# liuyuan-pal/Gen6D

Hardware: NVIDIA B200
Metric: poses/sec end-to-end (128^2 crop, 64 refs, 3 refine iters) (higher is better)
Workload: dtype f32

## Files before the change

gen6d_b200/_lib.py:

```python
import ctypes as C
import os
import re

HERE = os.path.dirname(os.path.abspath(__file__))
LIB_PATH = os.path.join(HERE, 'libgen6d_b200.so')
HEADER_PATH = os.path.join(os.path.dirname(HERE), 'include', 'gen6d_b200.h')

G6D_DET_MAX_SCALES = 8
PRO_NONE, PRO_AFFINE, PRO_AFFINE_RELU, PRO_CORR = 0, 1, 2, 3
ACT_NONE, ACT_RELU, ACT_LEAKY01 = 0, 1, 2
TC_TF32, TC_F16 = 0, 1


class ConvDesc(C.Structure):
    _fields_ = [(n, C.c_int) for n in ('B', 'D', 'H', 'W', 'Cin', 'in_cstride', 'in_coff', 'Cout', 'kd', 'kh', 'kw',
                                       'stride', 'pd', 'ph', 'pw', 'Do', 'Ho', 'Wo', 'out_cstride', 'out_coff',
                                       'prologue')] + [('group_rows', C.c_longlong), ('act', C.c_int), ('max_chain_k', C.c_int)]


class DetMaps(C.Structure):
    _fields_ = [('n_scales', C.c_int), ('rfn', C.c_int), ('hs', C.c_int), ('ws', C.c_int),
                ('map', (C.c_void_p * 3) * G6D_DET_MAX_SCALES),
                ('H', (C.c_int * 3) * G6D_DET_MAX_SCALES), ('W', (C.c_int * 3) * G6D_DET_MAX_SCALES),
                ('mu', C.c_float * 3), ('inv_sigma', C.c_float * 3), ('clip', C.c_float)]


class GlueCamera(C.Structure):
    _fields_ = [('K', C.c_double * 9), ('Kinv', C.c_double * 9), ('f', C.c_double), ('f_sq', C.c_double)]


class GlueRefs(C.Structure):
    _fields_ = [('poses', C.c_void_p), ('cen', C.c_void_p), ('f', C.c_void_p), ('dist', C.c_void_p), ('center', C.c_double * 3)]


class GlueViews(C.Structure):
    _fields_ = [('poses', C.c_void_p), ('R_look', C.c_void_p), ('RlookR', C.c_void_p), ('f', C.c_void_p), ('Kinv', C.c_void_p),
                ('src', C.c_void_p), ('rows', C.c_void_p), ('cols', C.c_void_p), ('even_idx', C.c_void_p), ('even_dirs', C.c_void_p),
                ('n_views', C.c_int), ('n_even', C.c_int), ('ref_num', C.c_int), ('size', C.c_int),
                ('norm_scale', C.c_double), ('norm_offset', C.c_float * 3), ('size_scale', C.c_float)]


P, I, L, F = C.c_void_p, C.c_int, C.c_longlong, C.c_float
_SIGNATURES = {
    'g6d_preprocess_u8': [P, P, L, I, I, P],
    'g6d_imagenet_norm': [P, P, L, I, I, P],
    'g6d_warp_perspective_u8': [P, I, P, I, I, P],
    'g6d_warp_affine_u8': [P, I, P, I, I, P],
    'g6d_glue_detection_jobs': [P, P, I, I, I, I, P, P],
    'g6d_glue_detection_jobs_host': [P, P, I, I, I, I, P],
    'g6d_glue_initial_poses': [P, P, P, C.POINTER(GlueRefs), P, I, P, P],
    'g6d_glue_initial_poses_host': [P, P, P, C.POINTER(GlueRefs), P, I, P],
    'g6d_glue_refine_problems': [C.POINTER(GlueViews), P, P, I, I, P, I, I, P, P, P, P, P, P, P, P],
    'g6d_glue_refine_problems_host': [C.POINTER(GlueViews), P, P, I, I, P, I, I, P, P, P, P, P, P, P],
    'g6d_glue_apply_refinements': [C.POINTER(GlueViews), P, P, P, P, I, P, P],
    'g6d_glue_apply_refinements_host': [C.POINTER(GlueViews), P, P, P, P, I, P],
    'g6d_track_smooth': [P, P, P, P, P, I, I, P, P, P, P, P, P],
    'g6d_track_smooth_host': [P, P, P, P, P, I, I, P, P, P, P, P],
    'g6d_nchw_to_nhwc': [P, P, I, I, I, I, I, P],
    'g6d_nhwc_to_nchw': [P, P, I, I, I, I, I, P],
    'g6d_resize_bilinear': [P, P, I, I, I, I, I, I, I, I, P],
    'g6d_resize_nearest': [P, P, I, I, I, I, I, I, P],
    'g6d_maxpool2x2': [P, P, I, I, I, I, P],
    'g6d_l2norm_channels': [P, P, L, I, F, P],
    'g6d_affine_act': [P, P, L, I, L, P, P, I, I, I, I, I, P],
    'g6d_avgpool_affine': [P, P, L, I, I, L, P, P, I, P],
    'g6d_add': [P, P, P, L, P],
    'g6d_instnorm_stats': [P, L, I, I, I, L, F, P, P, P, P],
    'g6d_instnorm_partial': [P, L, I, I, I, L, P, P],
    'g6d_instnorm_finalize': [P, L, I, L, F, P, P, P],
    'g6d_conv': [C.POINTER(ConvDesc), P, P, P, P, P, P, P, P],
    'g6d_conv_workspace_bytes': [C.POINTER(ConvDesc)],
    'g6d_vgg_first_block': [P, P, P, P, I, I, I, P],
    'g6d_pack_conv_weight': [P, P, I, I, I, I, P, P],
    'g6d_conv_tc_supported': [C.POINTER(ConvDesc), I],
    'g6d_conv_tc_debug': [C.POINTER(C.c_int)],
    'g6d_debug_umma_shift': [P, I, I, P],
    'g6d_conv_tc_workspace_bytes': [C.POINTER(ConvDesc), I],
    'g6d_conv_tc': [C.POINTER(ConvDesc), P, P, P, I, I, P, P, P, P, P, P, L, P],
    'g6d_conv_tc_stats_supported': [C.POINTER(ConvDesc), I, L],
    'g6d_pack_conv_weight_tc': [P, P, P, I, I, I, I, I, P, I, P],
    'g6d_split_operand': [P, P, P, L, I, P],
    'g6d_transpose2d': [P, P, I, I, P],
    'g6d_linear_smallm': [P, P, P, P, I, I, I, I, P],
    'g6d_det_score_fuse': [C.POINTER(DetMaps), I, P, P, P, P, P, P],
    'g6d_det_parse': [P, P, P, I, I, I, I, P, P, P],
    'g6d_det_corr_rowsum': [P, P, I, I, I, I, I, P],
    'g6d_sel_ref_sums': [P, I, I, I, P, P, P],
    'g6d_sel_corr_prologue': [P, P, P, I, I, I, F, P, P, P],
    'g6d_sel_corr_score': [P, P, I, I, I, P, P],
    'g6d_sel_corr_score3': [P, P, P, P, P, P, I, I, I, I, I, P, P, P, P],
    'g6d_sel_corr_score3_workspace_bytes': [I, I, I, I],
    'g6d_sel_vp_norm': [P, I, I, F, P, I, I, P],
    'g6d_sel_max_angle_add': [P, P, P, I, I, I, P],
    'g6d_attention': [P, P, P, P, I, I, I, P],
    'g6d_attention_headmajor': [P, P, P, P, I, I, I, P],
    'g6d_layernorm': [P, P, P, P, I, I, F, P],
    'g6d_sel_parse': [P, P, I, I, P, P, P],
    'g6d_ref_volume_fill': [P, P, P, P, P, P, I, I, I, I, I, I, I, I, P, P, P],
    'g6d_ref_pose_heads': [P, P, P, P, I, I, P],
    'g6d_pose_errors_workspace_bytes': [I, I],
    'g6d_pose_errors': [P, I, P, P, P, I, I, P, P, P],
}
_RESTYPE = {'g6d_pose_errors_workspace_bytes': L, 'g6d_sel_corr_score3_workspace_bytes': L, 'g6d_conv_workspace_bytes': L, 'g6d_conv_tc_workspace_bytes': L, 'g6d_launch_count': L, 'g6d_last_error': C.c_char_p}

_lib = None


class Gen6DLibraryError(RuntimeError):
    pass


def header_symbols():
    text = open(HEADER_PATH).read()
    text = re.sub(r'/\*.*?\*/', '', text, flags=re.S)
    return sorted(set(re.findall(r'\b(g6d_[a-z0-9_]+)\s*\(', text)))


def lib():
    global _lib
    if _lib is not None:
        return _lib
    if not os.path.exists(LIB_PATH):
        raise Gen6DLibraryError(
            f'{LIB_PATH} not found: build it with `python -m gen6d_b200.build` '
            '(there is no CPU or PyTorch fallback for the Gen6D hot path)')
    l = C.CDLL(LIB_PATH)
    for name, args in _SIGNATURES.items():
        fn = getattr(l, name)
        fn.argtypes = args
        fn.restype = _RESTYPE.get(name, I)
    l.g6d_last_error.restype = C.c_char_p
    l.g6d_last_error.argtypes = []
    l.g6d_version.restype = I
    l.g6d_launch_count.restype = L
    _lib = l
    return l


def check(rc, name):
    if rc != 0:
        msg = lib().g6d_last_error().decode(errors='replace')
        raise Gen6DLibraryError(f'{name} failed ({rc}): {msg}')


def launch_count():
    return int(lib().g6d_launch_count())
```

gen6d_b200/csrc/common.cuh:

```cuda
#pragma once
#include <cuda_runtime.h>
#include <stdint.h>
#include <stdio.h>
#include <stdarg.h>

#include "../../include/gen6d_b200.h"

namespace g6d {

void set_error(const char* fmt, ...);
void count_launch(int n = 1);

inline cudaStream_t as_stream(g6d_stream_t s) { return reinterpret_cast<cudaStream_t>(s); }

#define G6D_CHECK_LAUNCH(name)                                                        \
    do {                                                                              \
        cudaError_t e__ = cudaGetLastError();                                         \
        if (e__ != cudaSuccess) {                                                     \
            g6d::set_error("%s: launch failed: %s", name, cudaGetErrorString(e__));   \
            return G6D_ECUDA;                                                         \
        }                                                                             \
        g6d::count_launch();                                                          \
    } while (0)

#define G6D_REQUIRE(cond, ...)            \
    do {                                  \
        if (!(cond)) {                    \
            g6d::set_error(__VA_ARGS__);  \
            return G6D_EINVAL;            \
        }                                 \
    } while (0)

constexpr int kNumSMs = 148;

__device__ __forceinline__ float warp_sum(float v) {
#pragma unroll
    for (int o = 16; o > 0; o >>= 1) v += __shfl_xor_sync(0xffffffffu, v, o);
    return v;
}
__device__ __forceinline__ double warp_sum(double v) {
#pragma unroll
    for (int o = 16; o > 0; o >>= 1) v += __shfl_xor_sync(0xffffffffu, v, o);
    return v;
}
__device__ __forceinline__ float warp_max(float v) {
#pragma unroll
    for (int o = 16; o > 0; o >>= 1) v = fmaxf(v, __shfl_xor_sync(0xffffffffu, v, o));
    return v;
}

__device__ __forceinline__ float4 ldg_stream(const float4* p) {
    float4 r;
    asm volatile("ld.global.nc.L1::no_allocate.v4.f32 {%0,%1,%2,%3}, [%4];"
                 : "=f"(r.x), "=f"(r.y), "=f"(r.z), "=f"(r.w)
                 : "l"(p));
    return r;
}

inline int ceil_div(long long a, long long b) { return (int)((a + b - 1) / b); }

}
```

gen6d_b200/csrc/conv_ffma.cu:

```cuda
#include "common.cuh"

namespace g6d {

struct ConvP {
    const float* x; const float* w; const float* bias; const float* ps; const float* pb;
    float* y; float* ws;
    int B, D, H, W, Cin, ics, ico, Cout, ldw, kd, kh, kw, stride, pd, ph, pw, Do, Ho, Wo, ocs, oco, pro, act;
    long long group_rows;
    int M, K, ktiles, splits, kt_per_split;
};

constexpr int BM = 128, BK = 16, NT = 256;

__device__ __forceinline__ float act_apply(float v, int act) {
    if (act == G6D_ACT_RELU) return fmaxf(v, 0.f);
    if (act == G6D_ACT_LEAKY01) return v > 0.f ? v : 0.1f * v;
    return v;
}

template <int TN>
__global__ void __launch_bounds__(NT, 2) conv_ffma_kernel(const ConvP p) {
    constexpr int BN = 16 * TN;
    constexpr int HN = BN / 2;
    constexpr int B_F4 = (BK * BN / 4);
    constexpr int B_PER_T = (B_F4 + NT - 1) / NT;
    __shared__ __align__(16) float As[2][BK][BM + 4];
    __shared__ __align__(16) float Bs[2][BK][BN];

    const int t = threadIdx.x;
    const int tx = t & 15, ty = t >> 4;
    const int m_base = blockIdx.x * BM;
    const int n_base = blockIdx.y * BN;
    const int split = blockIdx.z;
    const int kt_begin = split * p.kt_per_split;
    const int kt_end = min(p.ktiles, kt_begin + p.kt_per_split);

    const int kq = t & 3;
    int rb[2], rz[2], ry[2], rx[2];
    bool rvalid[2];
#pragma unroll
    for (int i = 0; i < 2; ++i) {
        int m = m_base + (t >> 2) + 64 * i;
        rvalid[i] = m < p.M;
        int mm = rvalid[i] ? m : 0;
        int xo = mm % p.Wo; mm /= p.Wo;
        int yo = mm % p.Ho; mm /= p.Ho;
        int zo = mm % p.Do; mm /= p.Do;
        rb[i] = mm;
        rz[i] = zo * p.stride - p.pd;
        ry[i] = yo * p.stride - p.ph;
        rx[i] = xo * p.stride - p.pw;
    }

    float4 a_reg[2];
    float4 b_reg[B_PER_T];

    auto load_tile = [&](int kt) {
        const int k = kt * BK + kq * 4;
        const bool kvalid = k < p.K;
        int tap = 0, c = k;
        if (p.K != p.Cin) { tap = k / p.Cin; c = k - tap * p.Cin; }
        const int kx = tap % p.kw;
        const int tq = tap / p.kw;
        const int ky = tq % p.kh;
        const int kz = tq / p.kh;
#pragma unroll
        for (int i = 0; i < 2; ++i) {
            float4 v = make_float4(0.f, 0.f, 0.f, 0.f);
            const int zi = rz[i] + kz, yi = ry[i] + ky, xi = rx[i] + kx;
            const bool inb = rvalid[i] && kvalid && (unsigned)zi < (unsigned)p.D && (unsigned)yi < (unsigned)p.H &&
                             (unsigned)xi < (unsigned)p.W;
            if (inb) {
                const long long pos = ((long long)(rb[i] * p.D + zi) * p.H + yi) * p.W + xi;
                v = __ldg(reinterpret_cast<const float4*>(p.x + pos * p.ics + p.ico + c));
                if (p.pro != G6D_PRO_NONE) {
                    float4 s, b;
                    if (p.pro == G6D_PRO_CORR) {
                        const long long sp = ((long long)zi * p.H + yi) * p.W + xi;
                        s = __ldg(reinterpret_cast<const float4*>(p.ps + sp * p.Cin + c));
                        b = __ldg(reinterpret_cast<const float4*>(p.pb + c));
                    } else {
                        const long long g = rb[i] / p.group_rows;
                        s = __ldg(reinterpret_cast<const float4*>(p.ps + g * p.Cin + c));
                        b = __ldg(reinterpret_cast<const float4*>(p.pb + g * p.Cin + c));
                    }
                    v.x = fmaf(v.x, s.x, b.x); v.y = fmaf(v.y, s.y, b.y);
                    v.z = fmaf(v.z, s.z, b.z); v.w = fmaf(v.w, s.w, b.w);
                    if (p.pro == G6D_PRO_AFFINE_RELU) {
                        v.x = fmaxf(v.x, 0.f); v.y = fmaxf(v.y, 0.f); v.z = fmaxf(v.z, 0.f); v.w = fmaxf(v.w, 0.f);
                    }
                }
            }
            a_reg[i] = v;
        }
#pragma unroll
        for (int j = 0; j < B_PER_T; ++j) {
            const int f = t + j * NT;
            float4 v = make_float4(0.f, 0.f, 0.f, 0.f);
            if (f < B_F4) {
                const int kr = f / (BN / 4), nq = f % (BN / 4);
                const int kk = kt * BK + kr, n = n_base + nq * 4;
                if (kk < p.K && n < p.ldw) v = __ldg(reinterpret_cast<const float4*>(p.w + (long long)kk * p.ldw + n));
            }
            b_reg[j] = v;
        }
    };
    auto store_tile = [&](int buf) {
#pragma unroll
        for (int i = 0; i < 2; ++i) {
            const int r = (t >> 2) + 64 * i;
            As[buf][kq * 4 + 0][r] = a_reg[i].x;
            As[buf][kq * 4 + 1][r] = a_reg[i].y;
            As[buf][kq * 4 + 2][r] = a_reg[i].z;
            As[buf][kq * 4 + 3][r] = a_reg[i].w;
        }
#pragma unroll
        for (int j = 0; j < B_PER_T; ++j) {
            const int f = t + j * NT;
            if (f < B_F4) {
                const int kr = f / (BN / 4), nq = f % (BN / 4);
                *reinterpret_cast<float4*>(&Bs[buf][kr][nq * 4]) = b_reg[j];
            }
        }
    };

    float acc[8][TN];
#pragma unroll
    for (int i = 0; i < 8; ++i)
#pragma unroll
        for (int j = 0; j < TN; ++j) acc[i][j] = 0.f;

    if (kt_begin < kt_end) {
        load_tile(kt_begin);
        store_tile(0);
    }
    __syncthreads();
    int cur = 0;
// ... 131 lines not shown
            const int xi = 2 * xp - 1 + dx;
            float4 v = make_float4(0.f, 0.f, 0.f, 0.f);
            if ((unsigned)yi < (unsigned)H && (unsigned)xi < (unsigned)W)
                v = __ldg(reinterpret_cast<const float4*>(x + ((b * H + yi) * W + xi) * 4));
            win[dy][dx] = make_float3(v.x, v.y, v.z);
        }
    }
    float acc[4][16];
#pragma unroll
    for (int o = 0; o < 16; ++o) { const float bv = bs[q * 16 + o]; acc[0][o] = bv; acc[1][o] = bv; acc[2][o] = bv; acc[3][o] = bv; }
#pragma unroll
    for (int ky = 0; ky < 3; ++ky) {
#pragma unroll
        for (int kx = 0; kx < 3; ++kx) {
            const float* wr = ws + (ky * 3 + kx) * 4 * 64 + q * 16;
#pragma unroll
            for (int o4 = 0; o4 < 4; ++o4) {
                const float4 w0 = *reinterpret_cast<const float4*>(wr + o4 * 4);
                const float4 w1 = *reinterpret_cast<const float4*>(wr + 64 + o4 * 4);
                const float4 w2 = *reinterpret_cast<const float4*>(wr + 128 + o4 * 4);
#pragma unroll
                for (int px = 0; px < 4; ++px) {
                    const float3 v = win[(px >> 1) + ky][(px & 1) + kx];
                    float* a = acc[px] + o4 * 4;
                    a[0] = fmaf(v.x, w0.x, fmaf(v.y, w1.x, fmaf(v.z, w2.x, a[0])));
                    a[1] = fmaf(v.x, w0.y, fmaf(v.y, w1.y, fmaf(v.z, w2.y, a[1])));
                    a[2] = fmaf(v.x, w0.z, fmaf(v.y, w1.z, fmaf(v.z, w2.z, a[2])));
                    a[3] = fmaf(v.x, w0.w, fmaf(v.y, w1.w, fmaf(v.z, w2.w, a[3])));
                }
            }
        }
    }
    float4* yr = reinterpret_cast<float4*>(y + pp * 64 + q * 16);
#pragma unroll
    for (int o4 = 0; o4 < 4; ++o4) {
        float r[4];
#pragma unroll
        for (int e = 0; e < 4; ++e) {
            const int o = o4 * 4 + e;
            r[e] = fmaxf(fmaxf(fmaxf(acc[0][o], acc[1][o]), fmaxf(acc[2][o], acc[3][o])), 0.f);
        }
        __stcs(yr + o4, make_float4(r[0], r[1], r[2], r[3]));
    }
}

static int fill_params(const g6d_conv_desc* d, ConvP& p) {
    G6D_REQUIRE(d != nullptr, "g6d_conv: null desc");
    G6D_REQUIRE(d->B > 0 && d->D > 0 && d->H > 0 && d->W > 0 && d->Cin > 0 && d->Cout > 0, "g6d_conv: bad dims");
    G6D_REQUIRE(d->kd > 0 && d->kh > 0 && d->kw > 0 && d->stride > 0, "g6d_conv: bad kernel/stride");
    G6D_REQUIRE((d->Cin & 3) == 0 && (d->in_cstride & 3) == 0 && (d->in_coff & 3) == 0,
                "g6d_conv: Cin (%d), in_cstride (%d), in_coff (%d) must be multiples of 4", d->Cin, d->in_cstride,
                d->in_coff);
    G6D_REQUIRE(d->in_coff + d->Cin <= d->in_cstride, "g6d_conv: input channel slice out of row");
    G6D_REQUIRE(d->out_coff + d->Cout <= d->out_cstride, "g6d_conv: output channel slice out of row");
    const int Do = (d->D + 2 * d->pd - d->kd) / d->stride + 1;
    const int Ho = (d->H + 2 * d->ph - d->kh) / d->stride + 1;
    const int Wo = (d->W + 2 * d->pw - d->kw) / d->stride + 1;
    G6D_REQUIRE(Do == d->Do && Ho == d->Ho && Wo == d->Wo, "g6d_conv: output dims mismatch (%d,%d,%d) vs (%d,%d,%d)",
                d->Do, d->Ho, d->Wo, Do, Ho, Wo);
    G6D_REQUIRE(d->prologue >= 0 && d->prologue <= 3 && d->act >= 0 && d->act <= 2, "g6d_conv: bad prologue/act");
    if (d->prologue == G6D_PRO_AFFINE || d->prologue == G6D_PRO_AFFINE_RELU)
        G6D_REQUIRE(d->group_rows > 0, "g6d_conv: group_rows must be > 0 for affine prologue");
    const long long M = (long long)d->B * Do * Ho * Wo;
    const long long K = (long long)d->kd * d->kh * d->kw * d->Cin;
    G6D_REQUIRE(M < (1ll << 31) && K < (1ll << 31), "g6d_conv: problem too large");
    p.B = d->B; p.D = d->D; p.H = d->H; p.W = d->W; p.Cin = d->Cin; p.ics = d->in_cstride; p.ico = d->in_coff;
    p.Cout = d->Cout; p.ldw = (d->Cout + 3) & ~3; p.kd = d->kd; p.kh = d->kh; p.kw = d->kw; p.stride = d->stride;
    p.pd = d->pd; p.ph = d->ph; p.pw = d->pw; p.Do = Do; p.Ho = Ho; p.Wo = Wo; p.ocs = d->out_cstride;
    p.oco = d->out_coff; p.pro = d->prologue; p.act = d->act; p.group_rows = d->group_rows > 0 ? d->group_rows : 1;
    p.M = (int)M; p.K = (int)K; p.ktiles = (int)((K + BK - 1) / BK);
    const int bn = d->Cout > 64 ? 128 : (d->Cout > 32 ? 64 : 32);
    const long long ctas = (long long)ceil_div(M, BM) * ceil_div(d->Cout, bn);
    int splits = 1;
    if (ctas < kNumSMs && p.ktiles >= 16) {
        splits = (int)((2 * kNumSMs + ctas - 1) / ctas);
        splits = splits > p.ktiles / 8 ? p.ktiles / 8 : splits;
        splits = splits > 64 ? 64 : splits;
        splits = splits < 1 ? 1 : splits;
    }
    p.kt_per_split = (p.ktiles + splits - 1) / splits;
    p.splits = (p.ktiles + p.kt_per_split - 1) / p.kt_per_split;
    return G6D_OK;
}

}

using namespace g6d;

extern "C" long long g6d_conv_workspace_bytes(const g6d_conv_desc* desc) {
    ConvP p{};
    if (fill_params(desc, p) != G6D_OK) return -1;
    return p.splits > 1 ? (long long)p.splits * p.M * p.Cout * (long long)sizeof(float) : 0;
}

extern "C" int g6d_conv(const g6d_conv_desc* desc, const float* x, const float* w, const float* bias,
                        const float* pro_scale, const float* pro_shift, float* y, void* ws, g6d_stream_t stream) {
    ConvP p{};
    int rc = fill_params(desc, p);
    if (rc != G6D_OK) return rc;
    G6D_REQUIRE(x && w && y, "g6d_conv: null tensor pointer");
    if (p.pro != G6D_PRO_NONE) G6D_REQUIRE(pro_scale && pro_shift, "g6d_conv: prologue operands missing");
    if (p.splits > 1) G6D_REQUIRE(ws != nullptr, "g6d_conv: split-K workspace required (%d splits)", p.splits);
    p.x = x; p.w = w; p.bias = bias; p.ps = pro_scale; p.pb = pro_shift; p.y = y; p.ws = (float*)ws;
    cudaStream_t st = as_stream(stream);
    if (p.Cin == 4 && p.ics == 4 && p.ico == 0 && p.Cout == 64 && p.ocs == 64 && p.oco == 0 && p.kd == 1 && p.kh == 3 &&
        p.kw == 3 && p.stride == 1 && p.pd == 0 && p.ph == 1 && p.pw == 1 && p.D == 1 && p.pro == G6D_PRO_NONE) {
        conv3x3_c4_o64_kernel<<<ceil_div(p.M, 128), 128, 0, st>>>(x, w, bias, y, p.B, p.H, p.W, p.act);
        G6D_CHECK_LAUNCH("g6d_conv(first layer)");
        return G6D_OK;
    }
    const int bn = p.Cout > 64 ? 128 : (p.Cout > 32 ? 64 : 32);
    dim3 grid(ceil_div(p.M, BM), ceil_div(p.Cout, bn), p.splits);
    if (bn == 128) conv_ffma_kernel<8><<<grid, NT, 0, st>>>(p);
    else if (bn == 64) conv_ffma_kernel<4><<<grid, NT, 0, st>>>(p);
    else conv_ffma_kernel<2><<<grid, NT, 0, st>>>(p);
    G6D_CHECK_LAUNCH("g6d_conv");
    if (p.splits > 1) {
        const long long n = (long long)p.M * p.Cout;
        conv_splitk_reduce_kernel<<<ceil_div(n, 256), 256, 0, st>>>(p.ws, bias, y, p.M, p.Cout, p.splits, p.ocs, p.oco,
                                                                     p.act);
        G6D_CHECK_LAUNCH("g6d_conv(splitk reduce)");
    }
    return G6D_OK;
}

extern "C" int g6d_vgg_first_block(const float* x, const float* w, const float* bias, float* y, int B, int H, int W,
                                   g6d_stream_t stream) {
    G6D_REQUIRE(x && w && y && B > 0 && H >= 2 && W >= 2 && (H & 1) == 0 && (W & 1) == 0, "g6d_vgg_first_block: bad args (H, W even)");
    const long long threads = (long long)B * (H / 2) * (W / 2) * 4;
    conv3x3_c4_o64_relu_pool_kernel<<<ceil_div(threads, 128), 128, 0, as_stream(stream)>>>(x, w, bias, y, B, H, W);
    G6D_CHECK_LAUNCH("g6d_vgg_first_block");
    return G6D_OK;
}

__global__ void pack_conv_weight_kernel(const float* __restrict__ w, float* __restrict__ out, int Cout, int Cin,
                                        int Cin_pad, int taps, int ldw, const float* __restrict__ scale) {
    const long long i = (long long)blockIdx.x * blockDim.x + threadIdx.x;
    const long long total = (long long)taps * Cin_pad * ldw;
    if (i >= total) return;
    const int o = (int)(i % ldw);
    const long long k = i / ldw;
    const int c = (int)(k % Cin_pad);
    const int tap = (int)(k / Cin_pad);
    float v = 0.f;
    if (o < Cout && c < Cin) {
        v = w[((long long)o * Cin + c) * taps + tap];
        if (scale) v *= scale[o];
    }
    out[i] = v;
}

extern "C" int g6d_pack_conv_weight(const float* w, float* out, int Cout, int Cin, int Cin_pad, int taps,
                                    const float* cout_scale, g6d_stream_t stream) {
    G6D_REQUIRE(w && out && Cout > 0 && Cin > 0 && Cin_pad >= Cin && taps > 0, "g6d_pack_conv_weight: bad args");
    const int ldw = (Cout + 3) & ~3;
    const long long total = (long long)taps * Cin_pad * ldw;
    pack_conv_weight_kernel<<<ceil_div(total, 256), 256, 0, as_stream(stream)>>>(w, out, Cout, Cin, Cin_pad, taps, ldw,
                                                                                 cout_scale);
    G6D_CHECK_LAUNCH("g6d_pack_conv_weight");
// ... 68 lines not shown
```

gen6d_b200/csrc/conv_tc.cu:

```cuda
#include <stdlib.h>
#include <string.h>

#include <cuda_fp16.h>

#include "tc_common.cuh"

namespace g6d {

constexpr int TC_BM = 128;
constexpr int TC_PRODUCER_WARPS = 8;
constexpr int TC_THREADS = (TC_PRODUCER_WARPS + 2) * 32;
constexpr int TC_MAX_K_PER_CHAIN = 2048;

template <int KIND> struct KindCfg;
template <> struct KindCfg<G6D_TC_TF32> {
    static constexpr int BK = 32;
    static constexpr int NV = 1;
    static constexpr int RING = 3;
    static constexpr float CROSS = 1.f;
};
template <> struct KindCfg<G6D_TC_F16> {
    static constexpr int BK = 64;
    static constexpr int NV = 2;
    static constexpr int RING = 2;
    static constexpr float CROSS = 1.f / 2048.f;
};
constexpr float F16_LO_SCALE = 2048.f;
__host__ __device__ __forceinline__ int f16_k_source(int p) {
    const int c = p >> 3, i = p & 7;
    return i < 4 ? 4 * c + i : 32 + 4 * c + (i - 4);
}

struct ConvTcP {
    const float* x; const float* bias; const float* ps; const float* pb;
    float* y; float* ws;
    int B, D, H, W, Cin, ics, ico, Cout, kd, kh, kw, stride, pd, ph, pw, Do, Ho, Wo, ocs, oco, pro, act;
    long long group_rows;
    int M, K, kblocks, splits, kb_per_split;
    double* stats; long long stats_rows;
};

__device__ __forceinline__ uint32_t cvt_f16x2_sat(float e0, float e1) {
    uint32_t r;
    asm("cvt.rn.satfinite.f16x2.f32 %0, %1, %2;" : "=r"(r) : "f"(e1), "f"(e0));
    return r;
}
__device__ __forceinline__ void split_f16x2(float e0, float e1, uint32_t& hi, uint32_t& lo) {
    hi = cvt_f16x2_sat(e0, e1);
    const float2 hf = __half22float2(*reinterpret_cast<const __half2*>(&hi));
    lo = cvt_f16x2_sat((e0 - hf.x) * F16_LO_SCALE, (e1 - hf.y) * F16_LO_SCALE);
}
__device__ __forceinline__ void split_tf32x4(const float4 v, float4& hi, float4& lo) {
    hi.x = __uint_as_float((__float_as_uint(v.x) + 0x1000u) & 0xFFFFE000u);
    hi.y = __uint_as_float((__float_as_uint(v.y) + 0x1000u) & 0xFFFFE000u);
    hi.z = __uint_as_float((__float_as_uint(v.z) + 0x1000u) & 0xFFFFE000u);
    hi.w = __uint_as_float((__float_as_uint(v.w) + 0x1000u) & 0xFFFFE000u);
    lo.x = v.x - hi.x; lo.y = v.y - hi.y; lo.z = v.z - hi.z; lo.w = v.w - hi.w;
}
__device__ __forceinline__ void st_shared_v4(uint32_t addr, uint32_t a, uint32_t b, uint32_t c, uint32_t d) {
    asm volatile("st.shared.v4.b32 [%0], {%1,%2,%3,%4};" ::"r"(addr), "r"(a), "r"(b), "r"(c), "r"(d) : "memory");
}
template <int KIND>
__device__ __forceinline__ void split_store(uint32_t hi_addr, uint32_t lo_addr, const float4 (&v)[KindCfg<KIND>::NV]) {
    if constexpr (KIND == G6D_TC_TF32) {
        float4 hi, lo;
        split_tf32x4(v[0], hi, lo);
        st_shared_v4(hi_addr, __float_as_uint(hi.x), __float_as_uint(hi.y), __float_as_uint(hi.z), __float_as_uint(hi.w));
        st_shared_v4(lo_addr, __float_as_uint(lo.x), __float_as_uint(lo.y), __float_as_uint(lo.z), __float_as_uint(lo.w));
    } else {
        uint32_t h[4], l[4];
        split_f16x2(v[0].x, v[0].y, h[0], l[0]);
        split_f16x2(v[0].z, v[0].w, h[1], l[1]);
        split_f16x2(v[1].x, v[1].y, h[2], l[2]);
        split_f16x2(v[1].z, v[1].w, h[3], l[3]);
        st_shared_v4(hi_addr, h[0], h[1], h[2], h[3]);
        st_shared_v4(lo_addr, l[0], l[1], l[2], l[3]);
    }
}
__device__ __forceinline__ float4 affine4(float4 x, const float4 sc, const float4 sh, bool relu) {
    x.x = fmaf(x.x, sc.x, sh.x); x.y = fmaf(x.y, sc.y, sh.y); x.z = fmaf(x.z, sc.z, sh.z); x.w = fmaf(x.w, sc.w, sh.w);
    if (relu) { x.x = fmaxf(x.x, 0.f); x.y = fmaxf(x.y, 0.f); x.z = fmaxf(x.z, 0.f); x.w = fmaxf(x.w, 0.f); }
    return x;
}

template <int KIND>
__device__ __forceinline__ uint32_t umma_idesc(int M, int N) {
    constexpr uint32_t fmt = KIND == G6D_TC_TF32 ? 2u : 0u;
    return (1u << 4) | (fmt << 7) | (fmt << 10) | ((uint32_t)(N >> 3) << 17) | ((uint32_t)(M >> 4) << 24);
}
template <int KIND>
// ... 78 lines not shown
    const uint32_t base = (smem_u32(smem_raw) + 1023u) & ~1023u;
    uint8_t* base_ptr = smem_raw + (base - smem_u32(smem_raw));
    const uint32_t bar_base = base + STAGES * Cfg::STAGE_BYTES;
    auto a_hi = [&](int s) { return base + s * Cfg::STAGE_BYTES; };
    auto a_lo = [&](int s) { return base + s * Cfg::STAGE_BYTES + Cfg::A_BYTES; };
    auto b_hi = [&](int s) { return base + s * Cfg::STAGE_BYTES + 2 * Cfg::A_BYTES; };
    auto b_lo = [&](int s) { return base + s * Cfg::STAGE_BYTES + 2 * Cfg::A_BYTES + Cfg::B_BYTES; };
    auto full_a = [&](int s) { return bar_base + 8 * s; };
    auto full_b = [&](int s) { return bar_base + 8 * (STAGES + s); };
    auto empty = [&](int s) { return bar_base + 8 * (2 * STAGES + s); };
    auto tmem_full = [&](int b) { return bar_base + 8 * (3 * STAGES + b); };
    auto tmem_empty = [&](int b) { return bar_base + 8 * (3 * STAGES + 2 + b); };
    volatile uint32_t* tmem_slot = reinterpret_cast<volatile uint32_t*>(base_ptr + STAGES * Cfg::STAGE_BYTES + 8 * (3 * STAGES + 4));

    const int warp = threadIdx.x >> 5, lane = threadIdx.x & 31;
    if (warp == W_TMA && lane == 0) {
        for (int s = 0; s < STAGES; ++s) {
            mbar_init(full_a(s), NPW);
            mbar_init(full_b(s), 1);
            mbar_init(empty(s), 1);
        }
        for (int b = 0; b < 2; ++b) { mbar_init(tmem_full(b), 1); mbar_init(tmem_empty(b), 4); }
        fence_barrier_init();
        asm volatile("prefetch.tensormap [%0];" ::"l"(&map_hi) : "memory");
        asm volatile("prefetch.tensormap [%0];" ::"l"(&map_lo) : "memory");
    }
    if (warp == W_MMA) {
        asm volatile("tcgen05.alloc.cta_group::1.sync.aligned.shared::cta.b32 [%0], %1;"
                     ::"r"(smem_u32((const void*)tmem_slot)), "n"(Cfg::TMEM_COLS) : "memory");
        asm volatile("tcgen05.relinquish_alloc_permit.cta_group::1.sync.aligned;" ::: "memory");
    }
    tc_fence_before();
    __syncthreads();
    tc_fence_after();
    const uint32_t tmem_acc = *tmem_slot;

    auto decode = [&](int w, int& mt, int& nt, int& sp) {
        nt = w % wk.n_tiles; w /= wk.n_tiles;
        mt = w % wk.m_tiles;
        sp = w / wk.m_tiles;
    };

    if (warp < NPW) {
        const int chunk = threadIdx.x & 7;
        const int cofs = chunk * 4;
        const int r0 = threadIdx.x >> 3;
        int git = 0;
        for (int w = blockIdx.x; w < wk.total; w += gridDim.x) {
            int mt, nt, sp;
            decode(w, mt, nt, sp);
            const int m_base = mt * TC_BM;
            const int kb_begin = sp * p.kb_per_split;
            const int nkb = min(p.kblocks, kb_begin + p.kb_per_split) - kb_begin;
            int rb[ROWS], rsp[ROWS], rc[ROWS];
            unsigned rvmask = 0;
            const long long plane_sz = (long long)p.D * p.H * p.W;
#pragma unroll
            for (int j = 0; j < ROWS; ++j) {
                int m = m_base + r0 + RSTEP * j;
                const bool v = m < p.M;
                if (!v) m = 0;
                const int xo = m % p.Wo; m /= p.Wo;
                const int yo = m % p.Ho; m /= p.Ho;
                const int zo = m % p.Do; m /= p.Do;
                rb[j] = m;
                const int z = zo * p.stride - p.pd, y = yo * p.stride - p.ph, x = xo * p.stride - p.pw;
                rsp[j] = (z * p.H + y) * p.W + x;
                rc[j] = ((z + 8) << 24) | ((y + 8) << 12) | (x + 8);
                if (v) rvmask |= 1u << j;
            }
            int c0, kx, ky, kz;
            {
                const int k = kb_begin * BK;
                int tap = 0; c0 = k;
                if (p.K != p.Cin) { tap = k / p.Cin; c0 = k - tap * p.Cin; }
                kx = tap % p.kw; const int tq = tap / p.kw; ky = tq % p.kh; kz = tq / p.kh;
            }
            float4 v[RING][ROWS][NV];
            unsigned okm[RING]; int kc[RING]; int ksp[RING];
            auto issue_loads = [&](int q) {
                const int tap_sp = (kz * p.H + ky) * p.W + kx;
                okm[q] = 0; kc[q] = c0 + cofs; ksp[q] = tap_sp;
                const float* xb = p.x + p.ico + cofs + c0;
#pragma unroll
                for (int j = 0; j < ROWS; ++j) {
                    const int z = ((rc[j] >> 24) & 0xff) - 8 + kz, y = ((rc[j] >> 12) & 0xfff) - 8 + ky, x = (rc[j] & 0xfff) - 8 + kx;
                    const bool inb = ((rvmask >> j) & 1u) && (unsigned)z < (unsigned)p.D && (unsigned)y < (unsigned)p.H &&
                                     (unsigned)x < (unsigned)p.W;
#pragma unroll
                    for (int e = 0; e < NV; ++e) v[q][j][e] = make_float4(0.f, 0.f, 0.f, 0.f);
                    if (inb) {
                        const float4* src = reinterpret_cast<const float4*>(xb + ((long long)rb[j] * plane_sz + rsp[j] + tap_sp) * p.ics);
#pragma unroll
                        for (int e = 0; e < NV; ++e) v[q][j][e] = __ldg(src + e * 8);
                        okm[q] |= 1u << j;
                    }
                }
                c0 += BK;
                if (c0 == p.Cin) { c0 = 0; if (++kx == p.kw) { kx = 0; if (++ky == p.kh) { ky = 0; ++kz; } } }
            };
            auto process = [&](int q, int it) {
                const int g_it = git + it;
                const int s = g_it % STAGES;
                const uint32_t n_use = g_it / STAGES;
                if (p.pro != G6D_PRO_NONE) {
                    const bool relu = p.pro == G6D_PRO_AFFINE_RELU;
#pragma unroll
                    for (int j = 0; j < ROWS; ++j) {
                        if (okm[q] & (1u << j)) {
                            const float4* scp; const float4* shp;
                            if (p.pro == G6D_PRO_CORR) {
                                scp = reinterpret_cast<const float4*>(p.ps + (long long)(rsp[j] + ksp[q]) * p.Cin + kc[q]);
                                shp = reinterpret_cast<const float4*>(p.pb + kc[q]);
                            } else {
                                const long long g = rb[j] / (int)p.group_rows;
                                scp = reinterpret_cast<const float4*>(p.ps + g * p.Cin + kc[q]);
                                shp = reinterpret_cast<const float4*>(p.pb + g * p.Cin + kc[q]);
                            }
#pragma unroll
                            for (int e = 0; e < NV; ++e) v[q][j][e] = affine4(v[q][j][e], __ldg(scp + e * 8), __ldg(shp + e * 8), relu);
                        }
                    }
                }
                mbar_wait(empty(s), (n_use & 1) ^ 1, 1, g_it);
#pragma unroll
                for (int j = 0; j < ROWS; ++j) {
                    const int r = r0 + RSTEP * j;
                    const uint32_t so = r * 128 + ((chunk ^ (r & 7)) << 4);
                    split_store<KIND>(a_hi(s) + so, a_lo(s) + so, v[q][j]);
                }
                fence_proxy_async();
                __syncwarp();
                if (lane == 0) mbar_arrive(full_a(s));
            };
#pragma unroll
            for (int q = 0; q < RING - 1; ++q)
                if (q < nkb) issue_loads(q);
            for (int it = 0; it < nkb; it += RING) {
#pragma unroll
                for (int q = 0; q < RING; ++q) {
                    if (it + q < nkb) {
                        if (it + q + RING - 1 < nkb) issue_loads((q + RING - 1) % RING);
                        process(q, it + q);
                    }
                }
            }
            git += nkb;
        }
    } else if (warp == W_TMA) {
        if (lane == 0) {
            int git = 0;
            for (int w = blockIdx.x; w < wk.total; w += gridDim.x) {
                int mt, nt, sp;
                decode(w, mt, nt, sp);
                const int kb_begin = sp * p.kb_per_split;
                const int nkb = min(p.kblocks, kb_begin + p.kb_per_split) - kb_begin;
                for (int it = 0; it < min(nkb, PF); ++it) {
                    tma_prefetch_2d(&map_hi, (kb_begin + it) * BK, nt * BN);
                    tma_prefetch_2d(&map_lo, (kb_begin + it) * BK, nt * BN);
                }
                for (int it = 0; it < nkb; ++it, ++git) {
                    const int s = git % STAGES;
                    if (it + PF < nkb) {
                        tma_prefetch_2d(&map_hi, (kb_begin + it + PF) * BK, nt * BN);
                        tma_prefetch_2d(&map_lo, (kb_begin + it + PF) * BK, nt * BN);
                    }
                    mbar_wait(empty(s), ((git / STAGES) & 1) ^ 1, 3, git);
                    mbar_expect_tx(full_b(s), 2 * Cfg::B_BYTES);
                    const int k = (kb_begin + it) * BK;
                    tma_load_2d(b_hi(s), &map_hi, full_b(s), k, nt * BN);
                    tma_load_2d(b_lo(s), &map_lo, full_b(s), k, nt * BN);
// ... 177 lines not shown
}

static void launch_reduce(const float* ws, const float* bias, float* y, int M, int Cout, int splits, int ocs, int oco, int act,
                          double* stats, long long stats_rows, cudaStream_t st) {
    if (stats) {
        dim3 grid(ceil_div(M, 32), ceil_div(Cout, 64));
        conv_tc_reduce_stats_kernel<<<grid, 256, 0, st>>>(ws, bias, y, M, Cout, splits, ocs, oco, act, stats, stats_rows);
    } else {
        const long long n = (long long)M * Cout;
        conv_tc_reduce_kernel<<<ceil_div(n, 256), 256, 0, st>>>(ws, bias, y, M, Cout, splits, ocs, oco, act);
    }
}

typedef CUresult (*EncodeTiledFn)(CUtensorMap*, CUtensorMapDataType, cuuint32_t, void*, const cuuint64_t*,
                                  const cuuint64_t*, const cuuint32_t*, const cuuint32_t*, CUtensorMapInterleave,
                                  CUtensorMapSwizzle, CUtensorMapL2promotion, CUtensorMapFloatOOBfill);

static EncodeTiledFn get_encode_fn() {
    static EncodeTiledFn fn = nullptr;
    static bool tried = false;
    if (!tried) {
        tried = true;
        void* sym = nullptr;
        cudaDriverEntryPointQueryResult qres;
        if (cudaGetDriverEntryPoint("cuTensorMapEncodeTiled", &sym, cudaEnableDefault, &qres) == cudaSuccess &&
            qres == cudaDriverEntryPointSuccess)
            fn = reinterpret_cast<EncodeTiledFn>(sym);
    }
    return fn;
}

static int kind_bk(int kind) { return kind == G6D_TC_F16 ? 64 : 32; }
static int kind_esize(int kind) { return kind == G6D_TC_F16 ? 2 : 4; }

static int make_weight_map(CUtensorMap* map, const void* w, int rows, int K, int bn, int kind) {
    EncodeTiledFn enc = get_encode_fn();
    if (!enc) { set_error("g6d_conv_tc: cuTensorMapEncodeTiled unavailable"); return G6D_ECUDA; }
    cuuint64_t dims[2] = {(cuuint64_t)K, (cuuint64_t)rows};
    cuuint64_t strides[1] = {(cuuint64_t)K * kind_esize(kind)};
    cuuint32_t box[2] = {(cuuint32_t)kind_bk(kind), (cuuint32_t)bn};
    cuuint32_t estr[2] = {1, 1};
    CUresult r = enc(map, kind == G6D_TC_F16 ? CU_TENSOR_MAP_DATA_TYPE_FLOAT16 : CU_TENSOR_MAP_DATA_TYPE_FLOAT32, 2,
                     const_cast<void*>(w), dims, strides, box, estr,
                     CU_TENSOR_MAP_INTERLEAVE_NONE, CU_TENSOR_MAP_SWIZZLE_128B, CU_TENSOR_MAP_L2_PROMOTION_L2_256B,
                     CU_TENSOR_MAP_FLOAT_OOB_FILL_NONE);
    if (r != CUDA_SUCCESS) { set_error("g6d_conv_tc: cuTensorMapEncodeTiled failed (%d)", (int)r); return G6D_ECUDA; }
    return G6D_OK;
}

static int tc_block_n(int Cout) { return Cout > 64 ? 128 : (Cout > 32 ? 64 : 32); }

static bool tc2_dims_ok(const g6d_conv_desc* d) {
    return d->D + d->pd + 8 < 256 && d->H + d->ph + 8 < 4096 && d->W + d->pw + 8 < 4096 &&
           (long long)d->D * d->H * d->W < (1ll << 30) && d->group_rows < (1ll << 31);
}

static int fill_tc_params(const g6d_conv_desc* d, int kind, ConvTcP& p) {
    G6D_REQUIRE(d != nullptr, "g6d_conv_tc: null desc");
    G6D_REQUIRE(kind == G6D_TC_TF32 || kind == G6D_TC_F16, "g6d_conv_tc: bad operand kind %d", kind);
    G6D_REQUIRE(d->B > 0 && d->D > 0 && d->H > 0 && d->W > 0 && d->Cin > 0 && d->Cout > 0, "g6d_conv_tc: bad dims");
    G6D_REQUIRE(d->kd > 0 && d->kh > 0 && d->kw > 0 && d->stride > 0, "g6d_conv_tc: bad kernel/stride");
    const int bk = kind_bk(kind);
    G6D_REQUIRE((d->Cin % bk) == 0, "g6d_conv_tc: Cin (%d) must be a multiple of %d", d->Cin, bk);
    G6D_REQUIRE((d->in_cstride & 3) == 0 && (d->in_coff & 3) == 0, "g6d_conv_tc: in_cstride/in_coff must be multiples of 4");
    G6D_REQUIRE(d->in_coff + d->Cin <= d->in_cstride, "g6d_conv_tc: input channel slice out of row");
    G6D_REQUIRE(d->out_coff + d->Cout <= d->out_cstride, "g6d_conv_tc: output channel slice out of row");
    G6D_REQUIRE(tc2_dims_ok(d), "g6d_conv_tc: spatial extent too large for the tensor-core kernel");
    const int Do = (d->D + 2 * d->pd - d->kd) / d->stride + 1;
    const int Ho = (d->H + 2 * d->ph - d->kh) / d->stride + 1;
    const int Wo = (d->W + 2 * d->pw - d->kw) / d->stride + 1;
    G6D_REQUIRE(Do == d->Do && Ho == d->Ho && Wo == d->Wo, "g6d_conv_tc: output dims mismatch");
    G6D_REQUIRE(d->prologue >= 0 && d->prologue <= 3 && d->act >= 0 && d->act <= 2, "g6d_conv_tc: bad prologue/act");
    const long long M = (long long)d->B * Do * Ho * Wo;
    const long long K = (long long)d->kd * d->kh * d->kw * d->Cin;
    G6D_REQUIRE(M < (1ll << 31) && K < (1ll << 31), "g6d_conv_tc: problem too large");
    p.B = d->B; p.D = d->D; p.H = d->H; p.W = d->W; p.Cin = d->Cin; p.ics = d->in_cstride; p.ico = d->in_coff;
    p.Cout = d->Cout; p.kd = d->kd; p.kh = d->kh; p.kw = d->kw; p.stride = d->stride; p.pd = d->pd; p.ph = d->ph;
    p.pw = d->pw; p.Do = Do; p.Ho = Ho; p.Wo = Wo; p.ocs = d->out_cstride; p.oco = d->out_coff; p.pro = d->prologue;
    p.act = d->act; p.group_rows = d->group_rows > 0 ? d->group_rows : 1;
    p.M = (int)M; p.K = (int)K; p.kblocks = (int)(K / bk);
    const int bn = tc_block_n(d->Cout);
    const long long ctas = (long long)ceil_div(M, TC_BM) * ceil_div(d->Cout, bn);
    const int min_kb = 256 / bk;
    int splits = 1;
    if (ctas < kNumSMs && p.kblocks >= 2 * min_kb) {
        splits = (int)(kNumSMs / ctas);
        splits = splits > p.kblocks / min_kb ? p.kblocks / min_kb : splits;
        splits = splits < 1 ? 1 : splits;
    }
    const int nmain = bn == 32 ? Tc2Cfg<32>::NMAIN : (bn == 64 ? Tc2Cfg<64>::NMAIN : Tc2Cfg<128>::NMAIN);
    const int chain = d->max_chain_k > 0 ? d->max_chain_k * nmain : (K > 8192 ? TC_MAX_K_PER_CHAIN : 0);
    const int max_kb = chain > bk ? chain / bk : 1;
    const int min_splits = chain > 0 ? (p.kblocks + max_kb - 1) / max_kb : 1;
    splits = splits < min_splits ? min_splits : splits;
    splits = splits > 64 ? 64 : splits;
    p.kb_per_split = (p.kblocks + splits - 1) / splits;
    p.splits = (p.kblocks + p.kb_per_split - 1) / p.kb_per_split;
    return G6D_OK;
}

template <int BN, int KIND, int NPW = 8>
static int launch_tc2(const ConvTcP& p, const CUtensorMap& mh, const CUtensorMap& ml, cudaStream_t st) {
    using Cfg = Tc2Cfg<BN>;
    static bool configured = false;
    if (!configured) {
        cudaError_t e = cudaFuncSetAttribute(conv_tc2_kernel<BN, KIND, NPW>, cudaFuncAttributeMaxDynamicSharedMemorySize, Cfg::SMEM_BYTES);
        if (e != cudaSuccess) { set_error("g6d_conv_tc: cannot opt in to %d B of shared memory: %s", Cfg::SMEM_BYTES, cudaGetErrorString(e)); return G6D_ECUDA; }
        configured = true;
    }
    Tc2Work wk;
    wk.m_tiles = ceil_div(p.M, TC_BM); wk.n_tiles = ceil_div(p.Cout, BN);
    const long long total = (long long)wk.m_tiles * wk.n_tiles * p.splits;
    wk.total = (int)total;
    const int grid = total < kNumSMs ? (int)total : kNumSMs;
    conv_tc2_kernel<BN, KIND, NPW><<<grid, tc2_threads(NPW), Cfg::SMEM_BYTES, st>>>(p, wk, mh, ml);
    G6D_CHECK_LAUNCH("g6d_conv_tc");
    return G6D_OK;
}

__global__ void split_tf32_kernel(const float* __restrict__ in, float* __restrict__ hi, float* __restrict__ lo, long long n) {
    const long long i = (long long)blockIdx.x * blockDim.x + threadIdx.x;
    if (i >= n) return;
    const float v = in[i];
    const float h = to_tf32(v);
    hi[i] = h;
    lo[i] = to_tf32(v - h);
}
__device__ __forceinline__ void split_f16_scalar(float v, __half& h, __half& l) {
    uint32_t hh, ll;
    split_f16x2(v, 0.f, hh, ll);
    h = __ushort_as_half((unsigned short)(hh & 0xffffu));
    l = __ushort_as_half((unsigned short)(ll & 0xffffu));
}
__global__ void split_f16_kernel(const float* __restrict__ in, __half* __restrict__ hi, __half* __restrict__ lo, long long n) {
    const long long i = (long long)blockIdx.x * blockDim.x + threadIdx.x;
    if (i >= n) return;
    split_f16_scalar(in[(i & ~63ll) + f16_k_source((int)(i & 63))], hi[i], lo[i]);
}

template <int KIND>
__global__ void pack_conv_weight_tc_kernel(const float* __restrict__ w, void* __restrict__ hi, void* __restrict__ lo,
                                           int Cout, int Cin, int Cin_pad, int taps, int rows_pad,
                                           const float* __restrict__ scale) {
    const long long i = (long long)blockIdx.x * blockDim.x + threadIdx.x;
    const long long K = (long long)taps * Cin_pad;
    if (i >= K * rows_pad) return;
    const int o = (int)(i / K);
    const long long k = i % K;
    const int tap = (int)(k / Cin_pad);
    int c = (int)(k % Cin_pad);
    if constexpr (KIND == G6D_TC_F16) c = (c & ~63) + f16_k_source(c & 63);
    float v = 0.f;
    if (o < Cout && c < Cin) {
        v = w[((long long)o * Cin + c) * taps + tap];
        if (scale) v *= scale[o];
    }
    if constexpr (KIND == G6D_TC_TF32) {
        const float h = to_tf32(v);
        static_cast<float*>(hi)[i] = h;
        static_cast<float*>(lo)[i] = to_tf32(v - h);
    } else {
        split_f16_scalar(v, static_cast<__half*>(hi)[i], static_cast<__half*>(lo)[i]);
    }
}

struct ConvFlatP {
    const float* x; const float* bias; const float* ps; const float* pb; float* y; float* ws;
    int B, D, H, W, Cin, ics, ico, Cout, kd, kh, kw, pd, ph, pw, Do, Ho, Wo, ocs, oco, pro, act;
    long long group_rows;
    int Wp, tiles_per_plane, mode, nseg, taps_per_seg, seg_rows, rows_pad, ntab, cblocks;
    int a_stages, b_stages, splits, cb_per_split, M;
    double* stats; long long stats_rows;
};

template <int BN> struct FlatCfg {
    static constexpr int NMAIN = BN == 32 ? 7 : (BN == 256 ? 1 : 3);
    static constexpr int TMEM_COLS = (NMAIN + 1) * BN;
};

template <int BN, int KIND>
__global__ void __launch_bounds__(TC_THREADS, 1)
conv_tcflat_kernel(const ConvFlatP p, const __grid_constant__ CUtensorMap map_hi, const __grid_constant__ CUtensorMap map_lo) {
    using KC = KindCfg<KIND>;
    constexpr int NMAIN = FlatCfg<BN>::NMAIN;
    constexpr int TMEM_COLS = FlatCfg<BN>::TMEM_COLS;
    constexpr int B_BYTES = BN * 128;
    constexpr int BK = KC::BK, NV = KC::NV;
    extern __shared__ uint8_t smem_raw[];
    const uint32_t base = (smem_u32(smem_raw) + 1023u) & ~1023u;
    uint8_t* base_ptr = smem_raw + (base - smem_u32(smem_raw));
    const int A_TILE = p.rows_pad * 128;
    const uint32_t a_base = base;
    const uint32_t b_base = base + p.a_stages * 2 * A_TILE;
    const uint32_t bar_base = b_base + p.b_stages * 2 * B_BYTES;
    auto a_hi = [&](int s) { return a_base + s * 2 * A_TILE; };
    auto a_lo = [&](int s) { return a_base + s * 2 * A_TILE + A_TILE; };
    auto b_hi = [&](int s) { return b_base + s * 2 * B_BYTES; };
    auto b_lo = [&](int s) { return b_base + s * 2 * B_BYTES + B_BYTES; };
    auto a_full = [&](int s) { return bar_base + 8 * s; };
    auto a_empty = [&](int s) { return bar_base + 8 * (4 + s); };
    auto b_full = [&](int s) { return bar_base + 8 * (8 + s); };
    auto b_empty = [&](int s) { return bar_base + 8 * (12 + s); };
    const uint32_t tmem_full = bar_base + 8 * 16;
    const uint32_t bar_off = (bar_base - base);
    volatile uint32_t* tmem_slot = reinterpret_cast<volatile uint32_t*>(base_ptr + bar_off + 8 * 17);
    int* rowtab = reinterpret_cast<int*>(base_ptr + bar_off + 256);

    const int warp = threadIdx.x >> 5, lane = threadIdx.x & 31;
    int tile = blockIdx.x;
    const int t_in_plane = tile % p.tiles_per_plane; tile /= p.tiles_per_plane;
    const int zo = tile % p.Do;
    const int b = tile / p.Do;
    const int f0 = t_in_plane * TC_BM;
    const int n_base = blockIdx.y * BN;
    const int split = blockIdx.z;
    const int cb_begin = split * p.cb_per_split;
    const int cb_end = min(p.cblocks, cb_begin + p.cb_per_split);
    const int nunits = (cb_end - cb_begin) * p.nseg;

    for (int e = threadIdx.x; e < p.ntab * p.seg_rows; e += blockDim.x) {
        const int tb = e / p.seg_rows, i = e % p.seg_rows;
        const int g = f0 + (p.mode == 1 ? tb * p.Wp : 0) + i;
        const int yy = g / p.Wp - p.ph, xx = g % p.Wp - p.pw;
        rowtab[e] = ((unsigned)yy < (unsigned)p.H && (unsigned)xx < (unsigned)p.W) ? yy * p.W + xx : -1;
    }
    if (warp == TC_PRODUCER_WARPS && lane == 0) {
        for (int s = 0; s < 4; ++s) {
            mbar_init(a_full(s), TC_PRODUCER_WARPS);
            mbar_init(a_empty(s), 1);
            mbar_init(b_full(s), 1);
            mbar_init(b_empty(s), 1);
        }
        mbar_init(tmem_full, 1);
        fence_barrier_init();
        asm volatile("prefetch.tensormap [%0];" ::"l"(&map_hi) : "memory");
        asm volatile("prefetch.tensormap [%0];" ::"l"(&map_lo) : "memory");
    }
    if (warp == TC_PRODUCER_WARPS + 1) {
        asm volatile("tcgen05.alloc.cta_group::1.sync.aligned.shared::cta.b32 [%0], %1;"
                     ::"r"(smem_u32((const void*)tmem_slot)), "n"(TMEM_COLS) : "memory");
        asm volatile("tcgen05.relinquish_alloc_permit.cta_group::1.sync.aligned;" ::: "memory");
    }
    tc_fence_before();
    __syncthreads();
    tc_fence_after();
    const uint32_t tmem_acc = *tmem_slot;

    if (warp < TC_PRODUCER_WARPS) {
        const int chunk = threadIdx.x & 7;
        const int cofs = chunk * 4;
        const int r0 = threadIdx.x >> 3;
        const long long plane = (long long)p.H * p.W;
        const long long gi = (long long)b / p.group_rows;
        const bool relu = p.pro == G6D_PRO_AFFINE_RELU;
        constexpr int NB = 3;
        const int trips = (p.seg_rows + 127) / 128;
        const int total = nunits * trips;
        float4 v[NB][4][NV]; int off[NB][4];
        auto unit_of = [&](int tt, int& u, int& rbase, int& cb, int& kz, int& tb) {
            u = tt / trips; rbase = (tt - u * trips) * 128;
            cb = cb_begin + u / p.nseg;
            const int seg = u % p.nseg;
            kz = p.mode == 1 ? seg / p.kh : seg;
            tb = p.mode == 1 ? seg % p.kh : 0;
        };
        auto issue = [&](int tt, int q) {
            int u, rbase, cb, kz, tb;
            unit_of(tt, u, rbase, cb, kz, tb);
            const int zz = zo + kz - p.pd;
            const bool zok = (unsigned)zz < (unsigned)p.D;
            const float* xplane = p.x + ((long long)b * p.D + (zok ? zz : 0)) * plane * p.ics + p.ico + cb * BK + cofs;
            const int* tab = rowtab + tb * p.seg_rows;
#pragma unroll
            for (int j = 0; j < 4; ++j) {
                const int r = rbase + r0 + 32 * j;
                off[q][j] = (r < p.seg_rows && zok) ? tab[r] : -1;
#pragma unroll
                for (int e = 0; e < NV; ++e) v[q][j][e] = make_float4(0.f, 0.f, 0.f, 0.f);
                if (off[q][j] >= 0) {
                    const float4* src = reinterpret_cast<const float4*>(xplane + (long long)off[q][j] * p.ics);
#pragma unroll
                    for (int e = 0; e < NV; ++e) v[q][j][e] = __ldg(src + e * 8);
                }
            }
        };
        auto store = [&](int tt, int q) {
            int u, rbase, cb, kz, tb;
            unit_of(tt, u, rbase, cb, kz, tb);
            const int s = u % p.a_stages;
            const int zz = zo + kz - p.pd;
            const int c = cb * BK + cofs;
            if (rbase == 0) mbar_wait(a_empty(s), ((u / p.a_stages) & 1) ^ 1, 1, u);
#pragma unroll
            for (int j = 0; j < 4; ++j) {
                const int r = rbase + r0 + 32 * j;
                if (r >= p.rows_pad) continue;
                if (p.pro != G6D_PRO_NONE && off[q][j] >= 0) {
                    const float4* scp; const float4* shp;
                    if (p.pro == G6D_PRO_CORR) {
                        const long long sp = (long long)zz * plane + off[q][j];
                        scp = reinterpret_cast<const float4*>(p.ps + sp * p.Cin + c);
                        shp = reinterpret_cast<const float4*>(p.pb + c);
                    } else {
                        scp = reinterpret_cast<const float4*>(p.ps + gi * p.Cin + c);
                        shp = reinterpret_cast<const float4*>(p.pb + gi * p.Cin + c);
                    }
#pragma unroll
                    for (int e = 0; e < NV; ++e) v[q][j][e] = affine4(v[q][j][e], __ldg(scp + e * 8), __ldg(shp + e * 8), relu);
                }
                const uint32_t so = r * 128 + ((chunk ^ (r & 7)) << 4);
                split_store<KIND>(a_hi(s) + so, a_lo(s) + so, v[q][j]);
            }
            if (rbase + 128 >= p.seg_rows) {
                fence_proxy_async();
                __syncwarp();
                if (lane == 0) mbar_arrive(a_full(s));
            }
        };
#pragma unroll
        for (int q = 0; q < NB - 1; ++q)
            if (q < total) issue(q, q);
        for (int tt = 0; tt < total; tt += NB) {
#pragma unroll
            for (int q = 0; q < NB; ++q) {
                if (tt + q < total) {
                    if (tt + q + NB - 1 < total) issue(tt + q + NB - 1, (q + NB - 1) % NB);
                    store(tt + q, q);
                }
            }
        }

        mbar_wait(tmem_full, 0, 2, nunits);
        tc_fence_after();
        const int quad = warp & 3;
        const int row = quad * 32 + lane;
        const int f = f0 + row;
        const int yo = f / p.Wp, xo = f % p.Wp;
        const bool valid = yo < p.Ho && xo < p.Wo;
        const long long m = (((long long)b * p.Do + zo) * p.Ho + yo) * p.Wo + xo;
        constexpr int HALF = BN / 2;
        const int col0 = (warp >> 2) * HALF;
        const bool partial = p.splits > 1;
        const bool vec_ok = partial ? (p.Cout & 3) == 0
                                    : ((p.ocs & 3) == 0 && (p.oco & 3) == 0 && (reinterpret_cast<uintptr_t>(p.y) & 15) == 0 &&
                                       (!p.bias || (reinterpret_cast<uintptr_t>(p.bias) & 15) == 0));
        const int total_mm = nunits * p.taps_per_seg;
        const int n_acc = total_mm < NMAIN ? total_mm : NMAIN;
#pragma unroll
        for (int cc = 0; cc < HALF; cc += 16) {
            float accv[16];
            const uint32_t taddr = tmem_acc + ((uint32_t)(quad * 32) << 16) + (uint32_t)(col0 + cc);
            {
                uint32_t r[16];
                G6D_TMEM_LD16(r, taddr + (uint32_t)(NMAIN * BN));
                asm volatile("tcgen05.wait::ld.sync.aligned;" ::: "memory");
// ... 59 lines not shown
                    const int k = (seg * p.taps_per_seg + t) * p.Cin + cb * BK;
                    tma_load_2d(b_hi(s), &map_hi, b_full(s), k, n_base);
                    tma_load_2d(b_lo(s), &map_lo, b_full(s), k, n_base);
                }
            }
        }
    } else {
        if (elect_one_sync()) {
            const uint32_t idesc = umma_idesc<KIND>(TC_BM, BN);
            int bi = 0;
            for (int u = 0; u < nunits; ++u) {
                const int sa = u % p.a_stages;
                mbar_wait(a_full(sa), (u / p.a_stages) & 1, 4, u);
                tc_fence_after();
                for (int t = 0; t < p.taps_per_seg; ++t, ++bi) {
                    const int sb = bi % p.b_stages;
                    mbar_wait(b_full(sb), (bi / p.b_stages) & 1, 5, bi);
                    tc_fence_after();
                    const int shift = p.mode == 1 ? t : (t / p.kw) * p.Wp + (t % p.kw);
                    const uint64_t dah = umma_desc_sw128(a_hi(sa) + shift * 128), dal = umma_desc_sw128(a_lo(sa) + shift * 128);
                    const uint64_t dbh = umma_desc_sw128(b_hi(sb)), dbl = umma_desc_sw128(b_lo(sb));
                    const uint32_t main_acc = tmem_acc + (uint32_t)((bi % NMAIN) * BN);
                    const uint32_t cross_acc = tmem_acc + (uint32_t)(NMAIN * BN);
#pragma unroll
                    for (int ks = 0; ks < 4; ++ks) {
                        const uint64_t adv = (uint64_t)((ks * 32) >> 4);
                        umma<KIND>(cross_acc, dal + adv, dbh + adv, idesc, (bi > 0 || ks > 0) ? 1u : 0u);
                        umma<KIND>(cross_acc, dah + adv, dbl + adv, idesc, 1u);
                        umma<KIND>(main_acc, dah + adv, dbh + adv, idesc, (bi >= NMAIN || ks > 0) ? 1u : 0u);
                    }
                    umma_commit(b_empty(sb));
                }
                umma_commit(a_empty(sa));
            }
            umma_commit(tmem_full);
        }
    }
    __syncthreads();
    if (warp == TC_PRODUCER_WARPS + 1) {
        tc_fence_after();
        asm volatile("tcgen05.dealloc.cta_group::1.sync.aligned.b32 %0, %1;" ::"r"(tmem_acc), "n"(TMEM_COLS) : "memory");
    }
}

static int flat_level() {
    static int v = -1;
    if (v < 0) { const char* e = getenv("G6D_CONV_FLAT"); v = (e && e[0] >= '0' && e[0] <= '2') ? e[0] - '0' : 1; }
    return v;
}
static bool flat_disabled() { return flat_level() == 0; }

static int fill_flat_params(const g6d_conv_desc* d, int kind, ConvFlatP& p, int* smem_bytes) {
    const int bk = kind_bk(kind);
    if (!d || d->stride != 1 || (d->Cin % bk) != 0 || d->Cout < 16 || (d->in_cstride & 3) || (d->in_coff & 3)) return -1;
    const int Do = d->D + 2 * d->pd - d->kd + 1, Ho = d->H + 2 * d->ph - d->kh + 1, Wo = d->W + 2 * d->pw - d->kw + 1;
    if (Do != d->Do || Ho != d->Ho || Wo != d->Wo || Do < 1 || Ho < 1 || Wo < 1) return -1;
    if (d->kd * d->kh * d->kw == 1) return -1;
    const int bn = tc_block_n(d->Cout);
    const int Wp = d->W + 2 * d->pw;
    const int flat_rows = TC_BM + (d->kh - 1) * Wp + d->kw - 1;
    const int row_rows = TC_BM + d->kw - 1;
    const int budget = 220 * 1024;
    const int b_stage = 2 * bn * 128;
    {
        const long long tiles = ((long long)Ho * Wp + TC_BM - 1) / TC_BM;
        if ((long long)Ho * Wo * 100 < tiles * TC_BM * 60) return -1;
    }
    auto a_stage = [](int rows) { return 2 * ((rows + 7) / 8 * 8) * 128; };
    int mode, rows, ntab;
    if (2 * a_stage(flat_rows) + 3 * b_stage + 4 * flat_rows + 2048 <= budget) { mode = 0; rows = flat_rows; ntab = 1; }
    else if (d->kw > 1 && flat_level() >= 2) { mode = 1; rows = row_rows; ntab = d->kh; }
    else return -1;
    p.B = d->B; p.D = d->D; p.H = d->H; p.W = d->W; p.Cin = d->Cin; p.ics = d->in_cstride; p.ico = d->in_coff;
    p.Cout = d->Cout; p.kd = d->kd; p.kh = d->kh; p.kw = d->kw; p.pd = d->pd; p.ph = d->ph; p.pw = d->pw;
    p.Do = Do; p.Ho = Ho; p.Wo = Wo; p.ocs = d->out_cstride; p.oco = d->out_coff; p.pro = d->prologue; p.act = d->act;
    p.group_rows = d->group_rows > 0 ? d->group_rows : 1;
    p.Wp = Wp; p.tiles_per_plane = (Ho * Wp + TC_BM - 1) / TC_BM; p.mode = mode;
    p.nseg = mode == 0 ? d->kd : d->kd * d->kh; p.taps_per_seg = mode == 0 ? d->kh * d->kw : d->kw;
    p.seg_rows = rows; p.rows_pad = (rows + 7) / 8 * 8; p.ntab = ntab; p.cblocks = d->Cin / bk;
    const long long M = (long long)d->B * Do * Ho * Wo;
    if (M >= (1ll << 31)) return -1;
    p.M = (int)M;
    const int tab_bytes = 4 * ntab * rows;
    int a_st = 2, b_st = 3;
    int used = a_st * a_stage(rows) + b_st * b_stage + tab_bytes + 2048;
    while (b_st < 4 && used + b_stage <= budget) { ++b_st; used += b_stage; }
    while (a_st < 4 && used + a_stage(rows) <= budget) { ++a_st; used += a_stage(rows); }
    if (used > budget) return -1;
    p.a_stages = a_st; p.b_stages = b_st;
    *smem_bytes = a_st * a_stage(rows) + b_st * b_stage + 256 + tab_bytes + 1024 + 64;
    const long long ctas = (long long)d->B * Do * p.tiles_per_plane * ((d->Cout + bn - 1) / bn);
    const long long K = (long long)d->Cin * d->kd * d->kh * d->kw;
    int splits = 1;
    if (ctas < kNumSMs && p.cblocks >= 2) splits = (int)((kNumSMs + ctas - 1) / ctas);
    const int nmain = bn == 32 ? FlatCfg<32>::NMAIN : (bn == 64 ? FlatCfg<64>::NMAIN : FlatCfg<128>::NMAIN);
    const long long chain = d->max_chain_k > 0 ? (long long)d->max_chain_k * nmain : (K > 8192 ? TC_MAX_K_PER_CHAIN : 0);
    if (chain > 0) { const int ms = (int)((K + chain - 1) / chain); splits = splits < ms ? ms : splits; }
    splits = splits > p.cblocks ? p.cblocks : splits;
    splits = splits < 1 ? 1 : splits;
    p.cb_per_split = (p.cblocks + splits - 1) / splits;
    p.splits = (p.cblocks + p.cb_per_split - 1) / p.cb_per_split;
    return 0;
}

template <int BN, int KIND>
static int launch_flat(const ConvFlatP& p, int smem, const CUtensorMap& mh, const CUtensorMap& ml, cudaStream_t st) {
    static bool configured = false;
    if (!configured) {
        cudaError_t e = cudaFuncSetAttribute(conv_tcflat_kernel<BN, KIND>, cudaFuncAttributeMaxDynamicSharedMemorySize, 227 * 1024);
        if (e != cudaSuccess) { set_error("g6d_conv_tc(flat): cannot opt in to shared memory: %s", cudaGetErrorString(e)); return G6D_ECUDA; }
        configured = true;
    }
    dim3 grid((unsigned)((long long)p.B * p.Do * p.tiles_per_plane), ceil_div(p.Cout, BN), p.splits);
    conv_tcflat_kernel<BN, KIND><<<grid, TC_THREADS, smem, st>>>(p, mh, ml);
    G6D_CHECK_LAUNCH("g6d_conv_tc(flat)");
    return G6D_OK;
}

template <int KIND>
static int dispatch_flat(int bn, const ConvFlatP& p, int smem, const CUtensorMap& mh, const CUtensorMap& ml, cudaStream_t st) {
    if (bn == 128) return launch_flat<128, KIND>(p, smem, mh, ml, st);
    if (bn == 64) return launch_flat<64, KIND>(p, smem, mh, ml, st);
    return launch_flat<32, KIND>(p, smem, mh, ml, st);
}
template <int KIND>
static int dispatch_tc2(int bn, const ConvTcP& p, const CUtensorMap& mh, const CUtensorMap& ml, cudaStream_t st) {
    if (bn == 128) return launch_tc2<128, KIND>(p, mh, ml, st);
    if (bn == 64) return launch_tc2<64, KIND>(p, mh, ml, st);
    return launch_tc2<32, KIND>(p, mh, ml, st);
}

}

using namespace g6d;

extern "C" int g6d_conv_tc_debug(int* host_out8) {
    G6D_REQUIRE(host_out8 != nullptr, "g6d_conv_tc_debug: null");
    cudaError_t e = cudaDeviceSynchronize();
    if (e != cudaSuccess) { set_error("g6d_conv_tc_debug: sync: %s", cudaGetErrorString(e)); return G6D_ECUDA; }
    e = cudaMemcpyFromSymbol(host_out8, g_tc_timeout, sizeof(int) * 8);
    if (e != cudaSuccess) { set_error("g6d_conv_tc_debug: %s", cudaGetErrorString(e)); return G6D_ECUDA; }
    int zeros[8] = {0, 0, 0, 0, 0, 0, 0, 0};
    cudaMemcpyToSymbol(g_tc_timeout, zeros, sizeof(zeros));
    return G6D_OK;
}

extern "C" int g6d_conv_tc_supported(const g6d_conv_desc* d, int kind) {
    if (!d || (kind != G6D_TC_TF32 && kind != G6D_TC_F16)) return 0;
    return (d->Cin % kind_bk(kind)) == 0 && d->Cout >= 16 && (d->in_cstride & 3) == 0 && (d->in_coff & 3) == 0 &&
           tc2_dims_ok(d) ? 1 : 0;
}

extern "C" long long g6d_conv_tc_workspace_bytes(const g6d_conv_desc* desc, int kind) {
    {
        ConvFlatP fp{}; int smem = 0;
        if (!flat_disabled() && (kind == G6D_TC_TF32 || kind == G6D_TC_F16) && fill_flat_params(desc, kind, fp, &smem) == 0)
            return fp.splits > 1 ? (long long)fp.splits * fp.M * fp.Cout * (long long)sizeof(float) : 0;
    }
    ConvTcP p{};
    if (fill_tc_params(desc, kind, p) != G6D_OK) return -1;
    return p.splits > 1 ? (long long)p.splits * p.M * p.Cout * (long long)sizeof(float) : 0;
}

static bool stats_ok_tc2(long long stats_rows, long long M) { return stats_rows > 0 && stats_rows % 32 == 0 && M % stats_rows == 0; }
static bool stats_ok_flat(const ConvFlatP& fp, long long stats_rows) {
    return stats_rows > 0 && stats_rows % 32 == 0 && stats_rows % ((long long)fp.Ho * fp.Wo) == 0 && (long long)fp.M % stats_rows == 0;
}

extern "C" int g6d_conv_tc_stats_supported(const g6d_conv_desc* desc, int kind, long long stats_rows) {
    if (!g6d_conv_tc_supported(desc, kind)) return 0;
    ConvFlatP fp{}; int smem = 0;
    if (!flat_disabled() && fill_flat_params(desc, kind, fp, &smem) == 0) return stats_ok_flat(fp, stats_rows) ? 1 : 0;
    const long long M = (long long)desc->B * desc->Do * desc->Ho * desc->Wo;
    return stats_ok_tc2(stats_rows, M) ? 1 : 0;
}

extern "C" int g6d_conv_tc(const g6d_conv_desc* desc, const float* x, const void* w_hi, const void* w_lo, int w_rows,
                           int kind, const float* bias, const float* pro_scale, const float* pro_shift, float* y,
                           void* ws, double* stats, long long stats_rows, g6d_stream_t stream) {
    G6D_REQUIRE(kind == G6D_TC_TF32 || kind == G6D_TC_F16, "g6d_conv_tc: bad operand kind %d", kind);
    if (stats) {
        G6D_REQUIRE(g6d_conv_tc_stats_supported(desc, kind, stats_rows), "g6d_conv_tc: fused statistics need groups of whole 32-row slices / planes (stats_rows %lld)", stats_rows);
        const long long M = (long long)desc->B * desc->Do * desc->Ho * desc->Wo;
        cudaError_t e = cudaMemsetAsync(stats, 0, sizeof(double) * 2 * (M / stats_rows) * desc->Cout, as_stream(stream));
        if (e != cudaSuccess) { set_error("g6d_conv_tc: memset: %s", cudaGetErrorString(e)); return G6D_ECUDA; }
    }
    {
        ConvFlatP fp{}; int smem = 0;
        if (!flat_disabled() && fill_flat_params(desc, kind, fp, &smem) == 0) {
            G6D_REQUIRE(x && w_hi && w_lo && y, "g6d_conv_tc: null tensor pointer");
            G6D_REQUIRE(w_rows >= fp.Cout, "g6d_conv_tc: weight rows (%d) < Cout (%d)", w_rows, fp.Cout);
            if (fp.pro != G6D_PRO_NONE) G6D_REQUIRE(pro_scale && pro_shift, "g6d_conv_tc: prologue operands missing");
            if (fp.splits > 1) G6D_REQUIRE(ws != nullptr, "g6d_conv_tc: split workspace required (%d splits)", fp.splits);
            fp.x = x; fp.bias = bias; fp.ps = pro_scale; fp.pb = pro_shift; fp.y = y; fp.ws = (float*)ws;
            fp.stats = stats; fp.stats_rows = stats ? stats_rows : 1;
            const int bn = tc_block_n(fp.Cout);
            const int K = fp.kd * fp.kh * fp.kw * fp.Cin;
            CUtensorMap mh, ml;
            int rc2;
            if ((rc2 = make_weight_map(&mh, w_hi, w_rows, K, bn, kind)) != G6D_OK) return rc2;
            if ((rc2 = make_weight_map(&ml, w_lo, w_rows, K, bn, kind)) != G6D_OK) return rc2;
            cudaStream_t st = as_stream(stream);
// ... 126 lines not shown
```

gen6d_b200/csrc/selector.cu:

```cuda
#include <stdlib.h>

#include "common.cuh"

namespace g6d {

template <int C>
__global__ void __launch_bounds__(256) sel_corr_score_kernel(const float* __restrict__ ref,
                                                             const float* __restrict__ q, int S, int P,
                                                             float* __restrict__ score) {
    constexpr int V = C / 128;
    extern __shared__ float t_sh[];
    const int warp = threadIdx.x >> 5, lane = threadIdx.x & 31;
    const int nwarp = blockDim.x >> 5;
    __shared__ float s_red[8];
    for (int s = blockIdx.x; s < S; s += gridDim.x) {
        const float4* rs = reinterpret_cast<const float4*>(ref + (long long)s * P * C);
        float mx = -INFINITY;
        for (int p = warp; p < P; p += nwarp) {
            const float4* rp = rs + (long long)p * (C / 4);
            const float4* qp = reinterpret_cast<const float4*>(q + (long long)p * C);
            float4 rv[V];
#pragma unroll
            for (int i = 0; i < V; ++i) rv[i] = ldg_stream(rp + lane + 32 * i);
            float t = 0.f;
#pragma unroll
            for (int i = 0; i < V; ++i) {
                const float4 qv = __ldg(qp + lane + 32 * i);
                t = fmaf(rv[i].x, qv.x, fmaf(rv[i].y, qv.y, fmaf(rv[i].z, qv.z, fmaf(rv[i].w, qv.w, t))));
            }
            t = warp_sum(t);
            if (lane == 0) t_sh[p] = t;
            mx = fmaxf(mx, t);
        }
        if (lane == 0) s_red[warp] = mx;
        __syncthreads();
        float m = s_red[0];
        for (int w = 1; w < nwarp; ++w) m = fmaxf(m, s_red[w]);
        __syncthreads();
        float acc = 0.f;
        for (int p = threadIdx.x; p < P; p += blockDim.x) { const float t = t_sh[p]; acc += t * (t / m); }
        acc = warp_sum(acc);
        if (lane == 0) s_red[warp] = acc;
        __syncthreads();
        if (threadIdx.x == 0) {
            float a = 0.f;
            for (int w = 0; w < nwarp; ++w) a += s_red[w];
            score[s] = a;
        }
        __syncthreads();
    }
}

struct ScoreLevels {
    const float* ref[3];
    const float* q[3];
    int P[3];
    int S;
    long long row_end[3];
};

template <int C>
__device__ __forceinline__ float row_dot(const float4* __restrict__ rp, const float4* __restrict__ qp, int lane) {
    constexpr int V = C / 128;
    float4 rv[V];
#pragma unroll
    for (int i = 0; i < V; ++i) rv[i] = ldg_stream(rp + lane + 32 * i);
    float t = 0.f;
#pragma unroll
    for (int i = 0; i < V; ++i) {
        const float4 qv = __ldg(qp + lane + 32 * i);
        t = fmaf(rv[i].x, qv.x, fmaf(rv[i].y, qv.y, fmaf(rv[i].z, qv.z, fmaf(rv[i].w, qv.w, t))));
    }
    return t;
}

template <int C, bool FUSED>
__global__ void __launch_bounds__(256, 6) sel_corr_dots_kernel(const ScoreLevels L, float* __restrict__ t_out,
                                                            int* __restrict__ done, float* __restrict__ score,
                                                            long long chunk) {
    const int lane = threadIdx.x & 31, wib = threadIdx.x >> 5;
    const long long rows = L.row_end[2];
    auto locate = [&](long long row, const float4*& rp, const float4*& qp, int& item, int& P, long long& first) {
        const bool l0 = row < L.row_end[0], l1 = row < L.row_end[1];
        const long long lbase = l0 ? 0 : (l1 ? L.row_end[0] : L.row_end[1]);
        const long long local = row - lbase;
        P = l0 ? L.P[0] : (l1 ? L.P[1] : L.P[2]);
        const float* ref = l0 ? L.ref[0] : (l1 ? L.ref[1] : L.ref[2]);
        const float* q = l0 ? L.q[0] : (l1 ? L.q[1] : L.q[2]);
        const int sl = (int)(local / P);
        const int p = (int)(local - (long long)sl * P);
        item = (l0 ? 0 : (l1 ? 1 : 2)) * L.S + sl;
        first = lbase + (long long)sl * P;
        rp = reinterpret_cast<const float4*>(ref + local * C);
        qp = reinterpret_cast<const float4*>(q + (long long)p * C);
    };
    long long begin, end, stride;
    if (FUSED) {
        begin = (long long)blockIdx.x * chunk;
        end = min(rows, begin + chunk);
        stride = 16;
    } else {
        begin = 0; end = rows;
        stride = (((long long)gridDim.x * blockDim.x) >> 5) * 2;
    }
    const long long w0 = FUSED ? wib : (((long long)blockIdx.x * blockDim.x + threadIdx.x) >> 5);
    for (long long row = begin + w0 * 2; row < end; row += stride) {
        const float4 *r0, *q0, *r1, *q1;
        int item, P;
        long long first;
        locate(row, r0, q0, item, P, first);
        const bool two = row + 1 < end;
        locate(two ? row + 1 : row, r1, q1, item, P, first);
        float t0 = row_dot<C>(r0, q0, lane);
        float t1 = row_dot<C>(r1, q1, lane);
        t0 = warp_sum(t0);
        t1 = warp_sum(t1);
        if (lane == 0) {
            t_out[row] = t0;
            if (two) t_out[row + 1] = t1;
        }
    }
    if (!FUSED) return;
    if (lane == 0) __threadfence();
    __syncthreads();
    int n = 0;
    for (long long r = begin; r < end; ++n) {
        const float4 *rp, *qp;
        int item, P;
        long long first;
        locate(r, rp, qp, item, P, first);
        const long long next = min(end, first + P);
        if ((n & 7) == wib) {
            int last = 0;
            if (lane == 0) last = atomicAdd(done + item, (int)(next - r)) + (int)(next - r) == P;
            last = __shfl_sync(0xffffffffu, last, 0);
            if (last) {
                if (lane == 0) done[item] = 0;
                __threadfence();
                const float* tp = t_out + first;
                float m = -INFINITY;
                for (int p = lane; p < P; p += 32) m = fmaxf(m, __ldcg(tp + p));
                m = warp_max(m);
                float acc = 0.f;
                for (int p = lane; p < P; p += 32) { const float v = __ldcg(tp + p); acc += v * (v / m); }
                acc = warp_sum(acc);
                if (lane == 0) score[item] = acc;
            }
        }
        r = next;
    }
}

__global__ void sel_corr_finish_kernel(const ScoreLevels L, const float* __restrict__ t, float* __restrict__ score) {
    const int lane = threadIdx.x & 31;
    const int item = (int)(((long long)blockIdx.x * blockDim.x + threadIdx.x) >> 5);
    if (item >= 3 * L.S) return;
    const int l = item / L.S, s = item % L.S;
    const int P = l == 0 ? L.P[0] : (l == 1 ? L.P[1] : L.P[2]);
    const float* tp = t + (l == 0 ? 0 : (l == 1 ? L.row_end[0] : L.row_end[1])) + (long long)s * P;
    float m = -INFINITY;
    for (int p = lane; p < P; p += 32) m = fmaxf(m, tp[p]);
    m = warp_max(m);
    float acc = 0.f;
    for (int p = lane; p < P; p += 32) { const float v = tp[p]; acc += v * (v / m); }
    acc = warp_sum(acc);
    if (lane == 0) score[item] = acc;
}

__global__ void sel_ref_sums_kernel(const float* __restrict__ ref, int S, long long PC, int s_chunk,
                                    double* __restrict__ sum1, double* __restrict__ sum2) {
    const long long i = (long long)blockIdx.x * blockDim.x + threadIdx.x;
    if (i >= PC) return;
    const int s0 = blockIdx.y * s_chunk, s1 = min(S, s0 + s_chunk);
    double a = 0.0, b = 0.0;
    for (int s = s0; s < s1; ++s) {
        const double v = (double)ref[(long long)s * PC + i];
        a += v; b += v * v;
    }
    atomicAdd(sum1 + i, a);
    atomicAdd(sum2 + i, b);
}

__global__ void sel_corr_prologue_kernel(const float* __restrict__ q, const double* __restrict__ sum1,
                                         const double* __restrict__ sum2, int S, int P, int C, float eps,
                                         float* __restrict__ scale, float* __restrict__ shift) {
    const int c = blockIdx.x * 32 + (threadIdx.x & 31);
    const int row = threadIdx.x >> 5, nrow = blockDim.x >> 5;
    __shared__ double sm[8][32], sv[8][32];
    __shared__ float s_rstd[32];
    double m = 0.0, e2 = 0.0;
    if (c < C) {
        for (int p = row; p < P; p += nrow) {
            const double qv = (double)q[(long long)p * C + c];
            m += qv * sum1[(long long)p * C + c];
            e2 += qv * qv * sum2[(long long)p * C + c];
        }
    }
    sm[row][threadIdx.x & 31] = m; sv[row][threadIdx.x & 31] = e2;
    __syncthreads();
    if (row == 0 && c < C) {
        for (int r = 1; r < nrow; ++r) { m += sm[r][threadIdx.x]; e2 += sv[r][threadIdx.x]; }
        const double n = (double)S * (double)P;
        const double mean = m / n;
        double var = e2 / n - mean * mean;
        var = var < 0.0 ? 0.0 : var;
        const double rstd = 1.0 / sqrt(var + (double)eps);
        s_rstd[threadIdx.x] = (float)rstd;
        shift[c] = (float)(-mean * rstd);
    }
    __syncthreads();
    if (c < C) {
        const float r = s_rstd[threadIdx.x & 31];
        for (int p = row; p < P; p += nrow) scale[(long long)p * C + c] = q[(long long)p * C + c] * r;
    }
}

__global__ void sel_vp_norm_kernel(const float* __restrict__ score, int n, float eps, float* __restrict__ feats,
                                   int cstride, int coff) {
    const int l = blockIdx.x;
    const float* s = score + (long long)l * n;
    __shared__ double r1[32], r2[32];
    double a = 0.0, b = 0.0;
    for (int i = threadIdx.x; i < n; i += blockDim.x) { const double v = s[i]; a += v; b += v * v; }
    a = warp_sum(a); b = warp_sum(b);
    if ((threadIdx.x & 31) == 0) { r1[threadIdx.x >> 5] = a; r2[threadIdx.x >> 5] = b; }
    __syncthreads();
    a = 0.0; b = 0.0;
    for (int w = 0; w < (int)(blockDim.x >> 5); ++w) { a += r1[w]; b += r2[w]; }
    const double mean = a / n;
    double var = b / n - mean * mean;
    var = var < 0.0 ? 0.0 : var;
    const float rstd = (float)(1.0 / sqrt(var + (double)eps));
    const float fm = (float)mean;
    for (int i = threadIdx.x; i < n; i += blockDim.x) feats[(long long)i * cstride + coff + l] = (s[i] - fm) * rstd;
    if (l == 0)
        for (int c = coff + (int)gridDim.x; c < cstride; ++c)
            for (int i = threadIdx.x; i < n; i += blockDim.x) feats[(long long)i * cstride + c] = 0.f;
}

__global__ void sel_max_angle_add_kernel(const float* __restrict__ x, const float* __restrict__ embed,
                                         float* __restrict__ out, int rfn, int an, int C) {
    const long long i = (long long)blockIdx.x * blockDim.x + threadIdx.x;
    if (i >= (long long)rfn * C) return;
    const int c = (int)(i % C);
    const int r = (int)(i / C);
    float m = -INFINITY;
    for (int a = 0; a < an; ++a) m = fmaxf(m, x[((long long)r * an + a) * C + c]);
    out[i] = m + embed[i];
}

__global__ void attention_kernel(const float* __restrict__ q, const float* __restrict__ k, const float* __restrict__ v,
                                 float* __restrict__ out, int n, int C, int heads) {
    extern __shared__ float sh[];
    const int i = blockIdx.x, h = blockIdx.y;
    const int D = C / heads;
    float* prob = sh;
    float* qv = sh + n;
    for (int d = threadIdx.x; d < D; d += blockDim.x) qv[d] = q[(long long)i * C + d * heads + h];
    __syncthreads();
    const float inv = rsqrtf((float)D);
    for (int j = threadIdx.x; j < n; j += blockDim.x) {
        float s = 0.f;
        for (int d = 0; d < D; ++d) s = fmaf(qv[d], k[(long long)j * C + d * heads + h], s);
        prob[j] = s * inv;
    }
    __syncthreads();
    __shared__ float red[32];
    float m = -INFINITY;
    for (int j = threadIdx.x; j < n; j += blockDim.x) m = fmaxf(m, prob[j]);
    m = warp_max(m);
    if ((threadIdx.x & 31) == 0) red[threadIdx.x >> 5] = m;
    __syncthreads();
    m = red[0];
    for (int w = 1; w < (int)(blockDim.x >> 5); ++w) m = fmaxf(m, red[w]);
    __syncthreads();
    float sum = 0.f;
    for (int j = threadIdx.x; j < n; j += blockDim.x) { const float e = expf(prob[j] - m); prob[j] = e; sum += e; }
    sum = warp_sum(sum);
    if ((threadIdx.x & 31) == 0) red[threadIdx.x >> 5] = sum;
    __syncthreads();
    sum = 0.f;
    for (int w = 0; w < (int)(blockDim.x >> 5); ++w) sum += red[w];
    for (int d = threadIdx.x; d < D; d += blockDim.x) {
        float acc = 0.f;
        for (int j = 0; j < n; ++j) acc = fmaf(prob[j], v[(long long)j * C + d * heads + h], acc);
        out[(long long)i * C + d * heads + h] = acc / sum;
    }
}

constexpr int ATT_TQ = 8, ATT_TK = 32, ATT_D = 64;
__global__ void __launch_bounds__(128) attention_hm_kernel(const float* __restrict__ q, const float* __restrict__ k,
                                                           const float* __restrict__ v, float* __restrict__ out, int n, int C) {
    extern __shared__ float sh[];
    const int npad = (n + 31) & ~31;
    float* qs = sh;
    float* kt = qs + ATT_TQ * ATT_D;
    float* sc = kt + ATT_TK * (ATT_D + 1);
    __shared__ float s_sum[ATT_TQ];
    const int t = threadIdx.x, lane = t & 31, warp = t >> 5;
    const int i0 = blockIdx.x * ATT_TQ, h = blockIdx.y;
    const float inv = rsqrtf((float)ATT_D);
    for (int e = t; e < ATT_TQ * ATT_D; e += 128) {
        const int qi = e / ATT_D, d = e % ATT_D;
        qs[e] = i0 + qi < n ? q[(long long)(i0 + qi) * C + h * ATT_D + d] : 0.f;
    }
    for (int j0 = 0; j0 < n; j0 += ATT_TK) {
        __syncthreads();
        for (int e = t; e < ATT_TK * ATT_D / 4; e += 128) {
            const int jj = e >> 4, d4 = e & 15;
            float4 kv = make_float4(0.f, 0.f, 0.f, 0.f);
            if (j0 + jj < n) kv = __ldg(reinterpret_cast<const float4*>(k + (long long)(j0 + jj) * C + h * ATT_D) + d4);
            float* dst = kt + jj * (ATT_D + 1) + d4 * 4;
            dst[0] = kv.x; dst[1] = kv.y; dst[2] = kv.z; dst[3] = kv.w;
        }
        __syncthreads();
#pragma unroll
        for (int r = 0; r < 2; ++r) {
            const int qi = warp + 4 * r;
            const float* qr = qs + qi * ATT_D;
            const float* kr = kt + lane * (ATT_D + 1);
            float a = 0.f;
#pragma unroll 16
            for (int d = 0; d < ATT_D; ++d) a = fmaf(qr[d], kr[d], a);
            sc[qi * npad + j0 + lane] = a * inv;
        }
    }
    __syncthreads();
#pragma unroll
    for (int r = 0; r < 2; ++r) {
        const int qi = warp + 4 * r;
        float* row = sc + qi * npad;
        float m = -INFINITY;
        for (int j = lane; j < n; j += 32) m = fmaxf(m, row[j]);
        m = warp_max(m);
        float sum = 0.f;
        for (int j = lane; j < n; j += 32) { const float e = expf(row[j] - m); row[j] = e; sum += e; }
        sum = warp_sum(sum);
        if (lane == 0) s_sum[qi] = sum;
    }
    const int d = t & 63, qh = t >> 6;
    float acc[4] = {0.f, 0.f, 0.f, 0.f};
    for (int j0 = 0; j0 < n; j0 += ATT_TK) {
        __syncthreads();
        for (int e = t; e < ATT_TK * ATT_D / 4; e += 128) {
            const int jj = e >> 4, d4 = e & 15;
            float4 vv = make_float4(0.f, 0.f, 0.f, 0.f);
            if (j0 + jj < n) vv = __ldg(reinterpret_cast<const float4*>(v + (long long)(j0 + jj) * C + h * ATT_D) + d4);
            float* dst = kt + jj * (ATT_D + 1) + d4 * 4;
            dst[0] = vv.x; dst[1] = vv.y; dst[2] = vv.z; dst[3] = vv.w;
        }
        __syncthreads();
        const int jn = min(ATT_TK, n - j0);
        for (int jj = 0; jj < jn; ++jj) {
// ... 7 lines not shown
        const int qi = qh + 2 * r;
        if (i0 + qi < n) out[(long long)(i0 + qi) * C + h * ATT_D + d] = acc[r] / s_sum[qi];
    }
}

__global__ void layernorm_kernel(const float* __restrict__ x, const float* __restrict__ gamma,
                                 const float* __restrict__ beta, float* __restrict__ out, int rows, int C, float eps) {
    const int row = blockIdx.x * (blockDim.x >> 5) + (threadIdx.x >> 5);
    if (row >= rows) return;
    const int lane = threadIdx.x & 31;
    const float* xr = x + (long long)row * C;
    float s = 0.f;
    for (int c = lane; c < C; c += 32) s += xr[c];
    const float mean = warp_sum(s) / (float)C;
    float v = 0.f;
    for (int c = lane; c < C; c += 32) { const float d = xr[c] - mean; v = fmaf(d, d, v); }
    const float rstd = rsqrtf(warp_sum(v) / (float)C + eps);
    for (int c = lane; c < C; c += 32) out[(long long)row * C + c] = (xr[c] - mean) * rstd * gamma[c] + beta[c];
}

__global__ void sel_parse_kernel(const float* __restrict__ logits, const float* __restrict__ angles, int rfn,
                                 long long* __restrict__ out_idx, float* __restrict__ out) {
    const int qi = blockIdx.x;
    if (threadIdx.x != 0) return;
    const float* l = logits + (long long)qi * rfn;
    int best = 0;
    float bv = l[0];
    for (int r = 1; r < rfn; ++r)
        if (l[r] > bv || (l[r] != l[r] && bv == bv)) { bv = l[r]; best = r; }
    out_idx[qi] = best;
    out[qi * 2 + 0] = angles[(long long)qi * rfn + best];
    out[qi * 2 + 1] = bv;
}

}

using namespace g6d;

extern "C" int g6d_sel_corr_score(const float* ref, const float* q, int S, int P, int C, float* score,
                                  g6d_stream_t stream) {
    G6D_REQUIRE(ref && q && score && S > 0 && P > 0, "g6d_sel_corr_score: bad args");
    G6D_REQUIRE(C == 512 || C == 256 || C == 128, "g6d_sel_corr_score: C must be 128, 256 or 512 (got %d)", C);
    G6D_REQUIRE(P <= 8192, "g6d_sel_corr_score: P too large");
    const int grid = S < 8 * kNumSMs ? S : 8 * kNumSMs;
    const size_t smem = sizeof(float) * P;
    cudaStream_t st = as_stream(stream);
    if (C == 512) sel_corr_score_kernel<512><<<grid, 256, smem, st>>>(ref, q, S, P, score);
    else if (C == 256) sel_corr_score_kernel<256><<<grid, 256, smem, st>>>(ref, q, S, P, score);
    else sel_corr_score_kernel<128><<<grid, 256, smem, st>>>(ref, q, S, P, score);
    G6D_CHECK_LAUNCH("g6d_sel_corr_score");
    return G6D_OK;
}

extern "C" long long g6d_sel_corr_score3_workspace_bytes(int S, int P0, int P1, int P2) {
    if (S <= 0 || P0 <= 0 || P1 <= 0 || P2 <= 0) { set_error("g6d_sel_corr_score3_workspace_bytes: bad args"); return -1; }
    const long long rows = (long long)S * ((long long)P0 + P1 + P2);
    return ((rows + 3) / 4) * 4 * (long long)sizeof(float);
}

extern "C" int g6d_sel_corr_score3(const float* ref0, const float* ref1, const float* ref2, const float* q0,
                                   const float* q1, const float* q2, int S, int P0, int P1, int P2, int C, float* score,
                                   float* ws, int* counters, g6d_stream_t stream) {
    G6D_REQUIRE(ref0 && ref1 && ref2 && q0 && q1 && q2 && score && ws && S > 0 && P0 > 0 && P1 > 0 && P2 > 0,
                "g6d_sel_corr_score3: bad args");
    G6D_REQUIRE(C == 512, "g6d_sel_corr_score3: C must be 512 (got %d)", C);
    ScoreLevels L;
    L.ref[0] = ref0; L.ref[1] = ref1; L.ref[2] = ref2; L.q[0] = q0; L.q[1] = q1; L.q[2] = q2;
    L.P[0] = P0; L.P[1] = P1; L.P[2] = P2; L.S = S;
    L.row_end[0] = (long long)S * P0; L.row_end[1] = L.row_end[0] + (long long)S * P1;
    L.row_end[2] = L.row_end[1] + (long long)S * P2;
    cudaStream_t st = as_stream(stream);
    static int fused = -1;
    if (fused < 0) { const char* e = getenv("G6D_S2_FUSED"); fused = (e && e[0] == '0') ? 0 : 1; }
    static int occ[2] = {0, 0};
    if (occ[fused] == 0) {
        int n = 0;
        cudaError_t e = fused ? cudaOccupancyMaxActiveBlocksPerMultiprocessor(&n, sel_corr_dots_kernel<512, true>, 256, 0)
                              : cudaOccupancyMaxActiveBlocksPerMultiprocessor(&n, sel_corr_dots_kernel<512, false>, 256, 0);
        occ[fused] = (e == cudaSuccess && n > 0) ? n : 4;
    }
    const long long pairs = (L.row_end[2] + 1) / 2;
    long long grid = (pairs + 7) / 8;
    const long long full = (long long)occ[fused] * kNumSMs;
    if (grid > full) grid = full;
    if (fused && counters) {
        int* done = counters;
        long long chunk = (L.row_end[2] + grid - 1) / grid;
        chunk += chunk & 1;
        grid = (L.row_end[2] + chunk - 1) / chunk;
        sel_corr_dots_kernel<512, true><<<(unsigned)grid, 256, 0, st>>>(L, ws, done, score, chunk);
        G6D_CHECK_LAUNCH("g6d_sel_corr_score3");
        return G6D_OK;
    }
    sel_corr_dots_kernel<512, false><<<(unsigned)grid, 256, 0, st>>>(L, ws, nullptr, nullptr, 0);
    G6D_CHECK_LAUNCH("g6d_sel_corr_score3(dots)");
    sel_corr_finish_kernel<<<ceil_div(3ll * S * 32, 256), 256, 0, st>>>(L, ws, score);
    G6D_CHECK_LAUNCH("g6d_sel_corr_score3(finish)");
    return G6D_OK;
}

extern "C" int g6d_sel_ref_sums(const float* ref, int S, int P, int C, double* sum1, double* sum2,
                                g6d_stream_t stream) {
    G6D_REQUIRE(ref && sum1 && sum2 && S > 0 && P > 0 && C > 0, "g6d_sel_ref_sums: bad args");
    const long long PC = (long long)P * C;
    cudaStream_t st = as_stream(stream);
    cudaError_t e = cudaMemsetAsync(sum1, 0, sizeof(double) * PC, st);
    if (e == cudaSuccess) e = cudaMemsetAsync(sum2, 0, sizeof(double) * PC, st);
    if (e != cudaSuccess) { set_error("g6d_sel_ref_sums: memset failed: %s", cudaGetErrorString(e)); return G6D_ECUDA; }
    const int s_chunk = 16;
    dim3 grid(ceil_div(PC, 256), ceil_div(S, s_chunk));
    sel_ref_sums_kernel<<<grid, 256, 0, st>>>(ref, S, PC, s_chunk, sum1, sum2);
    G6D_CHECK_LAUNCH("g6d_sel_ref_sums");
    return G6D_OK;
}

extern "C" int g6d_sel_corr_prologue(const float* q, const double* sum1, const double* sum2, int S, int P, int C,
                                     float eps, float* scale, float* shift, g6d_stream_t stream) {
    G6D_REQUIRE(q && sum1 && sum2 && scale && shift && S > 0 && P > 0 && C > 0, "g6d_sel_corr_prologue: bad args");
    sel_corr_prologue_kernel<<<ceil_div(C, 32), 256, 0, as_stream(stream)>>>(q, sum1, sum2, S, P, C, eps, scale, shift);
    G6D_CHECK_LAUNCH("g6d_sel_corr_prologue");
    return G6D_OK;
}

extern "C" int g6d_sel_vp_norm(const float* score, int L, int n, float eps, float* feats, int cstride, int coff,
                               g6d_stream_t stream) {
    G6D_REQUIRE(score && feats && L > 0 && n > 0 && coff + L <= cstride, "g6d_sel_vp_norm: bad args");
    sel_vp_norm_kernel<<<L, 256, 0, as_stream(stream)>>>(score, n, eps, feats, cstride, coff);
    G6D_CHECK_LAUNCH("g6d_sel_vp_norm");
    return G6D_OK;
}

extern "C" int g6d_sel_max_angle_add(const float* x, const float* embed, float* out, int rfn, int an, int C,
                                     g6d_stream_t stream) {
    G6D_REQUIRE(x && embed && out && rfn > 0 && an > 0 && C > 0, "g6d_sel_max_angle_add: bad args");
    sel_max_angle_add_kernel<<<ceil_div((long long)rfn * C, 256), 256, 0, as_stream(stream)>>>(x, embed, out, rfn, an, C);
    G6D_CHECK_LAUNCH("g6d_sel_max_angle_add");
    return G6D_OK;
}

extern "C" int g6d_attention(const float* q, const float* k, const float* v, float* out, int n, int C, int heads,
                             g6d_stream_t stream) {
    G6D_REQUIRE(q && k && v && out && n > 0 && n <= 8192 && heads > 0 && C % heads == 0, "g6d_attention: bad args");
    const size_t smem = sizeof(float) * (n + C / heads);
    attention_kernel<<<dim3(n, heads), 64, smem, as_stream(stream)>>>(q, k, v, out, n, C, heads);
    G6D_CHECK_LAUNCH("g6d_attention");
    return G6D_OK;
}

extern "C" int g6d_attention_headmajor(const float* q, const float* k, const float* v, float* out, int n, int C, int heads,
                                       g6d_stream_t stream) {
    G6D_REQUIRE(q && k && v && out && n > 0 && n <= 2048 && heads > 0 && C == heads * ATT_D && (C & 3) == 0,
                "g6d_attention_headmajor: bad args (n <= 2048, C = heads * 64)");
    const int npad = (n + 31) & ~31;
    const size_t smem = sizeof(float) * (ATT_TQ * ATT_D + ATT_TK * (ATT_D + 1) + (size_t)ATT_TQ * npad);
    static bool configured = false;
    if (!configured) {
        cudaError_t e = cudaFuncSetAttribute(attention_hm_kernel, cudaFuncAttributeMaxDynamicSharedMemorySize, 96 * 1024);
        if (e != cudaSuccess) { set_error("g6d_attention_headmajor: %s", cudaGetErrorString(e)); return G6D_ECUDA; }
        configured = true;
    }
    attention_hm_kernel<<<dim3(ceil_div(n, ATT_TQ), heads), 128, smem, as_stream(stream)>>>(q, k, v, out, n, C);
    G6D_CHECK_LAUNCH("g6d_attention_headmajor");
    return G6D_OK;
}

extern "C" int g6d_layernorm(const float* x, const float* gamma, const float* beta, float* out, int rows, int C,
                             float eps, g6d_stream_t stream) {
    G6D_REQUIRE(x && gamma && beta && out && rows > 0 && C > 0, "g6d_layernorm: bad args");
    layernorm_kernel<<<ceil_div(rows, 4), 128, 0, as_stream(stream)>>>(x, gamma, beta, out, rows, C, eps);
    G6D_CHECK_LAUNCH("g6d_layernorm");
    return G6D_OK;
}

extern "C" int g6d_sel_parse(const float* logits, const float* angles, int qn, int rfn, long long* out_idx, float* out,
                             g6d_stream_t stream) {
    G6D_REQUIRE(logits && angles && out_idx && out && qn > 0 && rfn > 0, "g6d_sel_parse: bad args");
    sel_parse_kernel<<<qn, 32, 0, as_stream(stream)>>>(logits, angles, rfn, out_idx, out);
    G6D_CHECK_LAUNCH("g6d_sel_parse");
    return G6D_OK;
}
```

gen6d_b200/network/selector.py:

```python
import numpy as np
import torch

from .. import ops
from .backbone import pack_vgg, vgg_v1
from .base import Branches, PackedModule, linear_as_conv
from .params import SEL_TOWER_POST, SEL_TOWERS, VGG11BNParams, selector_modules

IN_EPS = 1e-5


class LocalComm:
    rank, world, capturable = 0, 1, True

    def all_reduce_sum(self, t):
        return t

    def all_gather_cat(self, t, dim=0):
        return t

    def shard_range(self, n):
        return 0, n


FEAT_PAD = 516
# ... 42 lines not shown
        p['score_predict'] = [linear_as_conv(self.score_predict[i].weight, self.score_predict[i].bias) for i in (0, 2)]
        w0 = self.angle_predict[0].weight.reshape(512, 515, an)
        w0p = torch.zeros(512, an, FEAT_PAD, device=w0.device, dtype=torch.float32)
        w0p[:, :, :515] = w0.permute(0, 2, 1)
        p['angle_predict'] = [linear_as_conv(w0p.reshape(512, an * FEAT_PAD, 1), self.angle_predict[0].bias)] + \
                             [linear_as_conv(self.angle_predict[i].weight, self.angle_predict[i].bias) for i in (2, 4)]
        p['vpe'] = [linear_as_conv(self.view_point_encoder[i].weight, self.view_point_encoder[i].bias) for i in (0, 2, 4)]
        return p

    def _feats(self, imgs_norm4):
        return [ops.l2norm_channels(f) for f in vgg_v1(self.packed()['vgg'], imgs_norm4)]

    @staticmethod
    def viewpoints(ref_poses, object_center, object_vert):
        ref_poses = torch.as_tensor(ref_poses, dtype=torch.float32).cpu()
        center = torch.as_tensor(object_center, dtype=torch.float32).cpu()
        vert = torch.as_tensor(object_vert, dtype=torch.float32).cpu()
        cam = (-ref_poses[:, :3, :3].permute(0, 2, 1) @ ref_poses[:, :3, 3:])[..., 0] - center[None]
        fwd = cam[0]
        y = torch.linalg.cross(vert, fwd)
        x = torch.linalg.cross(y, vert)
        nrm = lambda v: v / torch.clamp(torch.linalg.norm(v), min=1e-12)
        R = torch.stack([nrm(x), nrm(y), nrm(vert)], 0)
        cam = cam @ R.T
        return cam / torch.clamp(torch.linalg.norm(cam, dim=1, keepdim=True), min=1e-12)

    def _load_nhwc(self, ref_norm4, rfn, an, ref_poses, object_center, object_vert, chunk=64):
        p = self.packed()
        self.rfn_total = rfn
        r0, r1 = self.comm.shard_range(rfn)
        assert ref_norm4.shape[0] == (r1 - r0) * an
        vp_all = self.viewpoints(ref_poses, object_center, object_vert)
        rfn = r1 - r0
        S = rfn * an
        levels = [[], [], []]
        for s0 in range(0, S, chunk):
            for l, f in enumerate(self._feats(ref_norm4[s0:s0 + chunk])):
                levels[l].append(f)
        self.ref_feats_cache = [torch.cat(lv, 0) if len(lv) > 1 else lv[0] for lv in levels]
        sums = [ops.sel_ref_sums(f.reshape(S, -1, f.shape[-1])) for f in self.ref_feats_cache]
        self.ref_sums = [(self.comm.all_reduce_sum(a), self.comm.all_reduce_sum(b)) for a, b in sums]
        self.ref_shape = (rfn, an)
        vp = torch.zeros(rfn, 4, dtype=torch.float32)
        vp[:, :3] = vp_all[r0:r1]
        x = vp.to(self.device).reshape(rfn, 1, 1, 4)
        for i, pc in enumerate(p['vpe']):
            x = ops.conv(x, pc, act=ops.ACT_RELU if i < 2 else ops.ACT_NONE)
        self.ref_pose_embed = x.reshape(rfn, 512)
        self.bump_generation()

    def comm_stats(self):
        return dict(getattr(self.comm, 'calls', {}))

    def _s2_counters(self):
        n = 3 * self.ref_shape[0] * self.ref_shape[1]
        c = self.__dict__.get('_s2_done')
        if c is None or c.numel() != n or c.device != self.device:
            c = torch.zeros(n, device=self.device, dtype=torch.int32)
            self.__dict__['_s2_done'] = c
        return c

    def _finalize(self, ws, rows_total):
        return ops.instnorm_finalize(self.comm.all_reduce_sum(ws), rows_total, IN_EPS)

    def _tower(self, level, ref, scale, shift, cat_buf, S):
        convs = self.packed()['towers'][level]
        x, pro, ps, pb = ref, ops.PRO_CORR, scale, shift
        for i, (pc, post) in enumerate(convs):
            last = i + 1 == len(convs)
            if last:
                ops.conv(x, pc, prologue=pro, pro_scale=ps, pro_shift=pb, group_rows=S, out=cat_buf, out_coff=256 * level)
                break
            rows = x.shape[0] * x.shape[1] * x.shape[2]
            y, ws = ops.conv(x, pc, prologue=pro, pro_scale=ps, pro_shift=pb, group_rows=S, stats_rows=rows)
            ps, pb = self._finalize(ws, rows // self.ref_shape[0] * self.rfn_total)
            pro = ops.PRO_AFFINE_RELU if 'r' in post else ops.PRO_AFFINE
            x = ops.maxpool2x2(y) if 'p' in post else y

    def _towers_sharded(self, q_feats, cat_buf, S, S_total):
        towers = self.packed()['towers']
        nbr = 3 if self.comm.capturable else 1
        state, keep = [], []
        for l, (q, ref, (s1, s2)) in enumerate(zip(q_feats, self.ref_feats_cache, self.ref_sums)):
            h, w, c = q.shape
            scale, shift = ops.sel_corr_prologue(q.reshape(h * w, c), s1, s2, S_total, IN_EPS)
            state.append({'x': ref, 'pro': ops.PRO_CORR, 'ps': scale, 'pb': shift, 'i': 0})
        for _ in range(max(len(t) for t in towers)):
            br = Branches(nbr)
            pend = []
            for l, st in enumerate(state):
                convs = towers[l]
                if st['i'] >= len(convs):
                    continue
                pc, post = convs[st['i']]
                last = st['i'] + 1 == len(convs)

                def step(l=l, st=st, pc=pc, last=last):
                    if last:
                        ops.conv(st['x'], pc, prologue=st['pro'], pro_scale=st['ps'], pro_shift=st['pb'], group_rows=S,
                                 out=cat_buf, out_coff=256 * l)
                        return None
                    rows = st['x'].shape[0] * st['x'].shape[1] * st['x'].shape[2]
                    return ops.conv(st['x'], pc, prologue=st['pro'], pro_scale=st['ps'], pro_shift=st['pb'], group_rows=S,
                                    stats_rows=rows) + (rows,)
                res = br.run(l, step)
                st['i'] += 1
                if res is not None:
                    pend.append((st, post, res))
            br.join()
            if not pend:
                continue
            flat = torch.cat([ws.reshape(-1) for _, _, (_, ws, _) in pend]) if len(pend) > 1 else pend[0][2][1].reshape(-1)
            flat = self.comm.all_reduce_sum(flat)
            o = 0
            for st, post, (y, ws, rows) in pend:
                n = ws.numel()
                ps, pb = ops.instnorm_finalize(flat[o:o + n].reshape(ws.shape), rows // self.ref_shape[0] * self.rfn_total, IN_EPS)
                o += n
                keep.append((y, ws))
                st['ps'], st['pb'] = ps, pb
                st['pro'] = ops.PRO_AFFINE_RELU if 'r' in post else ops.PRO_AFFINE
                st['x'] = ops.maxpool2x2(y) if 'p' in post else y

    def _select_one(self, q_feats):
        p = self.packed()
        rfn, an = self.ref_shape
        S = rfn * an
        S_total = self.rfn_total * an
        dev = self.device
        cat_buf = torch.empty(S, 4, 4, 768, device=dev, dtype=torch.float32)
        feats = torch.empty(S, FEAT_PAD, device=dev, dtype=torch.float32)
        scores = ops.sel_corr_score3([r.reshape(S, -1, r.shape[-1]) for r in self.ref_feats_cache],
                                     [q.reshape(-1, q.shape[-1]) for q in q_feats], counters=self._s2_counters())
        if self.comm.world == 1:
            br = Branches(3)
            keep = []

            def one_level(l, q, ref, s1, s2):
                h, w, c = q.shape
                scale, shift = ops.sel_corr_prologue(q.reshape(h * w, c), s1, s2, S_total, IN_EPS)
                keep.append((scale, shift))
                self._tower(l, ref, scale, shift, cat_buf, S)

            for l, (q, ref, (s1, s2)) in enumerate(zip(q_feats, self.ref_feats_cache, self.ref_sums)):
                br.run(l, lambda l=l, q=q, ref=ref, s1=s1, s2=s2: one_level(l, q, ref, s1, s2))
            br.join()
        else:
            self._towers_sharded(q_feats, cat_buf, S, S_total)
        y, ws = ops.conv(cat_buf, p['cf0'], stats_rows=S * 16)
        ps, pb = self._finalize(ws, S_total * 16)
        y = ops.avgpool_affine(y.reshape(S * 16, 512), 16, ps, pb, rows_per_group=S * 16, act=ops.ACT_RELU)
        ops.conv(y.reshape(S, 1, 1, 512), p['cf3'], out=feats.reshape(S, 1, 1, FEAT_PAD), out_coff=0)
        if self.comm.world == 1:
            ops.sel_vp_norm(scores, feats, 512, IN_EPS)
        else:
            all_scores = self.comm.all_gather_cat(scores, dim=1).contiguous()
            tmp = torch.empty(S_total, 4, device=dev, dtype=torch.float32)
            ops.sel_vp_norm(all_scores, tmp, 0, IN_EPS)
            r0, _ = self.comm.shard_range(self.rfn_total)
            feats[:, 512:516] = tmp[r0 * an:r0 * an + S]
        x = ops.conv(feats.reshape(S, 1, 1, FEAT_PAD), p['sp0'], act=ops.ACT_RELU)
        x = ops.conv(x, p['sp2']).reshape(rfn, an, 512)
        sf = ops.sel_max_angle_add(x, self.ref_pose_embed)
        sf = self.comm.all_gather_cat(sf, dim=0).contiguous()
        rfn_local, rfn = rfn, self.rfn_total
        for att, (m0, m3) in zip(p['atts'], p['mlps']):
            x4 = sf.reshape(rfn, 1, 1, 512)
            qv = ops.conv(x4, att['conv_query']).reshape(rfn, 512)
            kv = ops.conv(x4, att['conv_key']).reshape(rfn, 512)
            vv = ops.conv(x4, att['conv_feats']).reshape(rfn, 512)
            msg = ops.attention(qv, kv, vv, heads=8, head_major=True)
            msg = ops.conv(msg.reshape(rfn, 1, 1, 512), att['conv_merge']).reshape(rfn, 512)
            msg = ops.layernorm(msg, att['ln_w'], att['ln_b'], 1e-5)
            y = ops.conv(torch.cat([sf, msg], 1).reshape(rfn, 1, 1, 1024), m0)
            ps, pb = ops.instnorm_stats(y, rows_per_group=rfn, eps=IN_EPS)
            y = ops.conv(y, m3, prologue=ops.PRO_AFFINE_RELU, pro_scale=ps, pro_shift=pb, group_rows=rfn)
            ps, pb = ops.instnorm_stats(y, rows_per_group=rfn, eps=IN_EPS)
            y = ops.affine_act(y.reshape(rfn, 512), ps, pb, rows_per_group=rfn, act=ops.ACT_RELU)
            sf = ops.add(y, sf)
        x = ops.conv(sf.reshape(rfn, 1, 1, 512), p['score_predict'][0], act=ops.ACT_RELU)
        logits = ops.conv(x, p['score_predict'][1]).reshape(rfn)
        x = feats.reshape(rfn_local, 1, 1, an * FEAT_PAD)
        for i, pc in enumerate(p['angle_predict']):
            x = ops.conv(x, pc, act=ops.ACT_RELU if i < 2 else ops.ACT_NONE)
        angles = self.comm.all_gather_cat(x.reshape(rfn_local), dim=0)
        return logits, angles, scores

    def _select_nhwc(self, que_norm4):
        if self.ref_feats_cache is None:
            raise RuntimeError('ViewpointSelector: load_ref_imgs / extract_ref_feats must be called first')
        feats = self._feats(que_norm4)
        logits, angles, taps = [], [], []
        for qi in range(que_norm4.shape[0]):
            lg, ang, sc = self._select_one([f[qi] for f in feats])
            logits.append(lg)
            angles.append(ang)
            taps.append(sc)
        return torch.stack(logits, 0), torch.stack(angles, 0), torch.stack(taps, 0)

    def _select_u8(self, u8):
        logits, angles, _ = self._select_nhwc(ops.preprocess_u8(u8, out_c=4, imagenet_norm=True))
        idx, out = ops.sel_parse(logits, angles)
        return idx, out, logits

    def extract_ref_feats(self, ref_imgs, ref_poses, object_center, object_vert, is_train=False):
        if is_train:
            raise NotImplementedError('inference-only build: random forward-view selection is a training feature')
        with torch.no_grad():
            an, rfn, _, h, w = ref_imgs.shape
            r0, r1 = self.comm.shard_range(rfn)
            x = ref_imgs[:, r0:r1].permute(1, 0, 2, 3, 4).reshape((r1 - r0) * an, 3, h, w).float().contiguous()
            x = ops.imagenet_norm(ops.nchw_to_nhwc(x), out_c=4)
            self._load_nhwc(x, rfn, an, ref_poses, object_center, object_vert)

    def compute_view_point_feats(self, que_imgs):
        with torch.no_grad():
            x = ops.imagenet_norm(ops.nchw_to_nhwc(que_imgs.float().contiguous()), out_c=4)
            logits, angles, _ = self._select_nhwc(x)
        return logits, angles

    def forward(self, data):
        self.extract_ref_feats(data['ref_imgs'], data['ref_imgs_info']['poses'], data['object_center'],
                               data['object_vert'], 'eval' not in data)
        logits, angles = self.compute_view_point_feats(data['que_imgs_info']['imgs'])
        return {'ref_vp_logits': logits, 'angles_pr': angles}

    def load_ref_imgs(self, ref_imgs, ref_poses, object_center, object_vert):
        with torch.no_grad():
            an, rfn, h, w, _ = ref_imgs.shape
            r0, r1 = self.comm.shard_range(rfn)
            u8 = torch.from_numpy(np.ascontiguousarray(ref_imgs[:, r0:r1].transpose(1, 0, 2, 3, 4))).to(self.device)
            u8 = u8.reshape((r1 - r0) * an, h, w, 3)
            x = ops.preprocess_u8(u8, out_c=4, imagenet_norm=True)
            self._load_nhwc(x, rfn, an, ref_poses.astype(np.float32), object_center.astype(np.float32),
                            object_vert.astype(np.float32))

    def _select_warped(self, size):
        def fn(jobs):
            crop = ops.warp_affine_u8(jobs, jobs.numel() // ops.WARP_JOB_BYTES, size, size)
            return (crop,) + tuple(self._select_u8(crop))
        return fn

    def select_from_frame(self, frame_dev, M, size):
        from .. import geometry as G
        fn = self._select_warped(size)
        with torch.no_grad():
            jobs = self._to_dev(G.pack_warp_jobs([frame_dev], [G.affine_dst_to_src(M)]))
            if self.comm.capturable:
                crop, idx, out, logits = self.stages.run(f'select_warp{size}', fn, [jobs])
            else:
                crop, idx, out, logits = fn(jobs)
# ... 25 lines not shown
```

gen6d_b200/ops.py:

```python
import ctypes as C
import os
from dataclasses import dataclass
from typing import Optional

import torch

from . import _lib
from ._lib import ACT_LEAKY01, ACT_NONE, ACT_RELU, PRO_AFFINE, PRO_AFFINE_RELU, PRO_CORR, PRO_NONE


WARP_JOB_BYTES = 88


def _stream():
    return C.c_void_p(torch.cuda.current_stream().cuda_stream)


def _p(t, dtype=torch.float32):
    if t is None:
        return None
    if not (t.is_cuda and t.dtype == dtype and t.is_contiguous()):
        raise ValueError(f'expected a contiguous CUDA {dtype} tensor, got {t.dtype} {t.device} '
                         f'contiguous={t.is_contiguous()} shape={tuple(t.shape)}')
    return C.c_void_p(t.data_ptr())
# ... 245 lines not shown


def _tc_dtype(kind):
    return torch.float16 if kind == _lib.TC_F16 else torch.float32


def pack_conv(weight, bias=None, stride=1, pad=None, cin_pad=None, cout_scale=None, bias_override=None):
    cout, cin = weight.shape[:2]
    ks = tuple(weight.shape[2:])
    k3 = (1,) * (3 - len(ks)) + ks
    if pad is None:
        pad = tuple(kk // 2 for kk in k3)
    elif isinstance(pad, int):
        pad = tuple(pad if kk > 1 else 0 for kk in k3)
    else:
        pad = (0,) * (3 - len(pad)) + tuple(pad)
    cin_pad = cin_pad or ((cin + 3) // 4 * 4)
    taps = k3[0] * k3[1] * k3[2]
    ldw = (cout + 3) // 4 * 4
    w = weight.detach().to(torch.float32).contiguous()
    out = torch.empty(taps * cin_pad, ldw, device=w.device, dtype=torch.float32)
    _call('g6d_pack_conv_weight', _p(w), _p(out), cout, cin, cin_pad, taps,
          _p(cout_scale.contiguous()) if cout_scale is not None else None, _stream())
    b = bias_override if bias_override is not None else bias
    b = b.detach().to(torch.float32).contiguous() if b is not None else None
    pc = PackedConv(out, b, cin_pad, cout, k3, stride, pad)
    kind = tc_kind_for(cin_pad)
    if kind is not None and cout >= 16:
        rows = (cout + 7) // 8 * 8
        pc.kind = kind
        pc.w_hi = torch.empty(rows, taps * cin_pad, device=w.device, dtype=_tc_dtype(kind))
        pc.w_lo = torch.empty_like(pc.w_hi)
        _call('g6d_pack_conv_weight_tc', _p(w), _p(pc.w_hi, pc.w_hi.dtype), _p(pc.w_lo, pc.w_lo.dtype), cout, cin, cin_pad,
              taps, rows, _p(cout_scale.contiguous()) if cout_scale is not None else None, kind, _stream())
    return pc


def split_operand(x, kind=None):
    kind = tc_kind_for(x.shape[-1]) if kind is None else kind
    hi = torch.empty(x.shape, device=x.device, dtype=_tc_dtype(kind))
    lo = torch.empty_like(hi)
    _call('g6d_split_operand', _p(x), _p(hi, hi.dtype), _p(lo, lo.dtype), x.numel(), kind, _stream())
    return hi, lo, kind


def transpose_to_packed(x2d):
    rows, cols = x2d.shape
    out = torch.empty(cols, (rows + 3) // 4 * 4, device=x2d.device, dtype=torch.float32)
    _call('g6d_transpose2d', _p(x2d), _p(out), rows, cols, _stream())
    return out


def conv(x, pc, prologue=PRO_NONE, pro_scale=None, pro_shift=None, group_rows=1, act=ACT_NONE,
         in_coff=0, out=None, out_coff=0, stats_rows=None):
    four = x.dim() == 4
    if four:
        B, H, W, cs = x.shape
        D = 1
    else:
        B, D, H, W, cs = x.shape
    kd, kh, kw = pc.k
    pd, ph, pw = pc.pad
    s = pc.stride
    Do, Ho, Wo = (D + 2 * pd - kd) // s + 1, (H + 2 * ph - kh) // s + 1, (W + 2 * pw - kw) // s + 1
    if out is None:
        shape = (B, Ho, Wo, pc.cout) if four else (B, Do, Ho, Wo, pc.cout)
        out = torch.empty(shape, device=x.device, dtype=torch.float32)
    d = _lib.ConvDesc(B=B, D=D, H=H, W=W, Cin=pc.cin, in_cstride=cs, in_coff=in_coff, Cout=pc.cout, kd=kd, kh=kh,
                      kw=kw, stride=s, pd=pd, ph=ph, pw=pw, Do=Do, Ho=Ho, Wo=Wo, out_cstride=out.shape[-1],
                      out_coff=out_coff, prologue=prologue, group_rows=group_rows, act=act, max_chain_k=pc.max_chain_k)
    work = 2.0 * B * Do * Ho * Wo * pc.cout * kd * kh * kw * pc.cin
    M = B * Do * Ho * Wo
    stats = None
    if pc.w_hi is not None and conv_path() == 'tc' and _lib.lib().g6d_conv_tc_supported(C.byref(d), pc.kind):
        nbytes = _lib.lib().g6d_conv_tc_workspace_bytes(C.byref(d), pc.kind)
        if nbytes < 0:
            _lib.check(-1, 'g6d_conv_tc_workspace_bytes')
        ws = torch.empty(nbytes // 4, device=x.device, dtype=torch.float32) if nbytes > 0 else None
        fuse = (stats_rows is not None and fused_stats_enabled() and
                _lib.lib().g6d_conv_tc_stats_supported(C.byref(d), pc.kind, stats_rows))
        if fuse:
            stats = torch.empty(M // stats_rows, pc.cout, 2, device=x.device, dtype=torch.float64)
        _call('g6d_conv_tc', C.byref(d), _p(x), _p(pc.w_hi, pc.w_hi.dtype), _p(pc.w_lo, pc.w_lo.dtype), pc.w_hi.shape[0],
              pc.kind, _p(pc.bias), _p(pro_scale), _p(pro_shift), _p(out), _p(ws), _p(stats, torch.float64), stats_rows or 0,
              _stream(), work=work,
              tag=f'M={M} N={pc.cout} K={kd * kh * kw * pc.cin} k={kd}x{kh}x{kw} s={s} pro={prologue}')
    else:
        if pc.w is None:
            raise _lib.Gen6DLibraryError('this operand was packed for the tensor-core path only and the problem is not supported there')
        nbytes = _lib.lib().g6d_conv_workspace_bytes(C.byref(d))
        if nbytes < 0:
            _lib.check(-1, 'g6d_conv_workspace_bytes')
        ws = torch.empty(nbytes // 4, device=x.device, dtype=torch.float32) if nbytes > 0 else None
        _call('g6d_conv', C.byref(d), _p(x), _p(pc.w), _p(pc.bias), _p(pro_scale), _p(pro_shift), _p(out), _p(ws), _stream(),
              work=work)
    if stats_rows is None:
        return out
    if stats is None:
        stats = instnorm_partial(out, rows_per_group=stats_rows, channels=pc.cout, coff=out_coff)
    return out, stats


def fused_stats_enabled():
    return os.environ.get('G6D_FUSED_STATS', '1') != '0'


def vgg_first_block(x, pc):
    B, H, W, _ = x.shape
    out = torch.empty(B, H // 2, W // 2, 64, device=x.device, dtype=torch.float32)
    _call('g6d_vgg_first_block', _p(x), _p(pc.w), _p(pc.bias), _p(out), B, H, W, _stream())
    return out


def linear_smallm(x, w, bias, act=ACT_NONE):
    M, K = x.shape
    N = w.shape[0]
    out = torch.empty(M, N, device=x.device, dtype=torch.float32)
    _call('g6d_linear_smallm', _p(x), _p(w), _p(bias), _p(out), M, N, K, act, _stream())
    return out


def det_score_fuse(maps, sizes, rfn, hs, ws, stats, clip, w1, b1, w2, b2, qn):
    m = _lib.DetMaps()
    m.n_scales, m.rfn, m.hs, m.ws = len(maps), rfn, hs, ws
    for s, lv in enumerate(maps):
        for l, t in enumerate(lv):
            m.map[s][l] = _p(t).value
            m.H[s][l], m.W[s][l] = sizes[s][l]
    for l in range(3):
        m.mu[l] = float(stats[l][0])
        m.inv_sigma[l] = 1.0 / float(stats[l][1])
    m.clip = float(clip)
    out = torch.empty(qn, hs, ws, 64, device=w1.device, dtype=torch.float32)
    _call('g6d_det_score_fuse', C.byref(m), qn, _p(w1), _p(b1), _p(w2), _p(b2), _p(out), _stream())
    return out


def det_corr_rowsum(partial, k, rfn):
    qn, Hp, W, _ = partial.shape
    H = Hp - (k - 1)
    out = torch.empty(qn, H, W, rfn, device=partial.device, dtype=torch.float32)
    _call('g6d_det_corr_rowsum', _p(partial), _p(out), qn, H, W, k, rfn, _stream())
    return out


def det_parse(scores, scales, offsets, pool_ratio=8):
    qn, hs, ws, _ = scores.shape
    out = torch.empty(qn, 4, device=scores.device, dtype=torch.float32)
    idx = torch.empty(qn, device=scores.device, dtype=torch.int64)
    _call('g6d_det_parse', _p(scores), _p(scales), _p(offsets), qn, hs, ws, pool_ratio, _p(out),
          _p(idx, torch.int64), _stream())
    return out, idx


def sel_ref_sums(ref):
    S, Pn, Cc = ref.shape
    s1 = torch.empty(Pn, Cc, device=ref.device, dtype=torch.float64)
    s2 = torch.empty_like(s1)
    _call('g6d_sel_ref_sums', _p(ref), S, Pn, Cc, _p(s1, torch.float64), _p(s2, torch.float64), _stream())
    return s1, s2


def sel_corr_prologue(q, s1, s2, S, eps=1e-5):
    Pn, Cc = q.shape
    scale = torch.empty(Pn, Cc, device=q.device, dtype=torch.float32)
    shift = torch.empty(Cc, device=q.device, dtype=torch.float32)
    _call('g6d_sel_corr_prologue', _p(q), _p(s1, torch.float64), _p(s2, torch.float64), S, Pn, Cc, eps, _p(scale),
          _p(shift), _stream())
    return scale, shift


def sel_corr_score(ref, q, out=None):
    S, Pn, Cc = ref.shape
    if out is None:
        out = torch.empty(S, device=ref.device, dtype=torch.float32)
    _call('g6d_sel_corr_score', _p(ref), _p(q), S, Pn, Cc, _p(out), _stream(),
          work=4.0 * (S * Pn * Cc + Pn * Cc + S))
    return out


def sel_corr_score3(refs, qs, counters=None):
    S, Cc = refs[0].shape[0], refs[0].shape[2]
    Ps = [r.shape[1] for r in refs]
    out = torch.empty(3, S, device=refs[0].device, dtype=torch.float32)
    ws = torch.empty(_lib.lib().g6d_sel_corr_score3_workspace_bytes(S, *Ps) // 4, device=refs[0].device, dtype=torch.float32)
    _call('g6d_sel_corr_score3', _p(refs[0]), _p(refs[1]), _p(refs[2]), _p(qs[0]), _p(qs[1]), _p(qs[2]), S, Ps[0], Ps[1],
          Ps[2], Cc, _p(out), _p(ws), _p(counters, torch.int32), _stream(), work=4.0 * (S * sum(Ps) * Cc + sum(Ps) * Cc + 3 * S))
    return out


def sel_vp_norm(score, feats, coff, eps=1e-5):
    Ln, n = score.shape
    _call('g6d_sel_vp_norm', _p(score), Ln, n, eps, _p(feats), feats.shape[-1], coff, _stream())


def sel_max_angle_add(x, embed):
    rfn, an, Cc = x.shape
    out = torch.empty(rfn, Cc, device=x.device, dtype=torch.float32)
    _call('g6d_sel_max_angle_add', _p(x), _p(embed), _p(out), rfn, an, Cc, _stream())
    return out


def attention(q, k, v, heads, head_major=False):
    n, Cc = q.shape
    out = torch.empty_like(q)
    _call('g6d_attention_headmajor' if head_major else 'g6d_attention', _p(q), _p(k), _p(v), _p(out), n, Cc, heads, _stream())
    return out


def layernorm(x, gamma, beta, eps=1e-5):
    rows, Cc = x.shape
    out = torch.empty_like(x)
    _call('g6d_layernorm', _p(x), _p(gamma), _p(beta), _p(out), rows, Cc, eps, _stream())
    return out


def sel_parse(logits, angles):
    qn, rfn = logits.shape
    idx = torch.empty(qn, device=logits.device, dtype=torch.int64)
    out = torch.empty(qn, 2, device=logits.device, dtype=torch.float32)
    _call('g6d_sel_parse', _p(logits), _p(angles), qn, rfn, _p(idx, torch.int64), _p(out), _stream())
    return idx, out


def ref_volume_fill(ref_feats, que_feats, ref_Ks, ref_poses, que_Ks, que_poses, sn, img_h, img_w):
    Q, R, fh, fw, Cc = ref_feats.shape
    mean_in = torch.empty(Q, sn, sn, sn, 2 * Cc, device=ref_feats.device, dtype=torch.float32)
    stdv = torch.empty(Q, sn, sn, sn, Cc, device=ref_feats.device, dtype=torch.float32)
    _call('g6d_ref_volume_fill', _p(ref_feats), _p(que_feats), _p(ref_Ks), _p(ref_poses), _p(que_Ks), _p(que_poses),
          Q, R, fh, fw, Cc, sn, img_h, img_w, _p(mean_in), _p(stdv), _stream(),
          work=4.0 * Q * ((R + 1) * fh * fw * Cc + 3 * Cc * sn ** 3))
    return mean_in, stdv


def ref_pose_heads(x, w, b):
    M, K = x.shape
    out = torch.empty(M, 7, device=x.device, dtype=torch.float32)
    _call('g6d_ref_pose_heads', _p(x), _p(w), _p(b), _p(out), M, K, _stream())
    return out
```

include/gen6d_b200.h:

```cpp
#ifndef GEN6D_B200_H
#define GEN6D_B200_H

#include <stdint.h>

#ifdef __cplusplus
extern "C" {
#endif

#define G6D_OK 0
#define G6D_EINVAL (-1)
#define G6D_ECUDA (-2)

typedef void* g6d_stream_t;

const char* g6d_last_error(void);
int g6d_version(void);
long long g6d_launch_count(void);

int g6d_preprocess_u8(const uint8_t* img, float* out, long long n_pixels, int out_c, int imagenet_norm,
                      g6d_stream_t stream);
typedef struct g6d_warp_job {
    const uint8_t* src;
    int rows, cols;
    double M[9];
// ... 37 lines not shown
                           const g6d_glue_camera* cams, int qn, double* poses, g6d_stream_t stream);
int g6d_glue_initial_poses_host(const float* det_out, const long long* sel_idx, const float* sel_out, const g6d_glue_refs* refs,
                                const g6d_glue_camera* cams, int qn, double* poses);
int g6d_glue_refine_problems(const g6d_glue_views* views, const g6d_glue_camera* cams, const uint8_t* frames, int rows, int cols,
                             const double* poses, int poses_are_f32, int qn, g6d_warp_job* jobs, float* que_K, float* que_pose,
                             float* rect, float* ref_Ks, float* ref_poses, int* ref_rows, g6d_stream_t stream);
int g6d_glue_refine_problems_host(const g6d_glue_views* views, const g6d_glue_camera* cams, const uint8_t* frames, int rows,
                                  int cols, const double* poses, int poses_are_f32, int qn, g6d_warp_job* jobs, float* que_K,
                                  float* que_pose, float* rect, float* ref_Ks, float* ref_poses, int* ref_rows);
int g6d_glue_apply_refinements(const g6d_glue_views* views, const float* que_pose, const float* que_K, const float* rect,
                               const float* net_out, int qn, double* poses, g6d_stream_t stream);
int g6d_glue_apply_refinements_host(const g6d_glue_views* views, const float* que_pose, const float* que_K, const float* rect,
                                    const float* net_out, int qn, double* poses);

int g6d_track_smooth(const float* bbox, const double* poses, const g6d_glue_camera* cams, const double* weights, const double* wsum,
                     int lanes, int num, float* hist, int* count, float* corners, double* wpts, double* smoothed, g6d_stream_t stream);
int g6d_track_smooth_host(const float* bbox, const double* poses, const g6d_glue_camera* cams, const double* weights, const double* wsum,
                          int lanes, int num, float* hist, int* count, float* corners, double* wpts, double* smoothed);
int g6d_imagenet_norm(const float* in, float* out, long long n_pixels, int in_c, int out_c, g6d_stream_t stream);
int g6d_nchw_to_nhwc(const float* in, float* out, int N, int C, int H, int W, int out_c, g6d_stream_t stream);
int g6d_nhwc_to_nchw(const float* in, float* out, int N, int C, int H, int W, int in_c, g6d_stream_t stream);
int g6d_resize_bilinear(const float* in, float* out, int N, int Hi, int Wi, int Ho, int Wo, int C,
                        int out_cstride, int out_coff, g6d_stream_t stream);
int g6d_resize_nearest(const float* in, float* out, int N, int Hi, int Wi, int Ho, int Wo, int C, g6d_stream_t stream);
int g6d_maxpool2x2(const float* in, float* out, int N, int H, int W, int C, g6d_stream_t stream);
int g6d_l2norm_channels(const float* in, float* out, long long rows, int C, float eps, g6d_stream_t stream);
int g6d_affine_act(const float* in, float* out, long long rows, int C, long long rows_per_group,
                   const float* scale, const float* shift, int act,
                   int in_cstride, int in_coff, int out_cstride, int out_coff, g6d_stream_t stream);
int g6d_avgpool_affine(const float* in, float* out, long long n_out, int spatial, int C, long long rows_per_group,
                       const float* scale, const float* shift, int act, g6d_stream_t stream);
int g6d_add(const float* a, const float* b, float* out, long long n, g6d_stream_t stream);

int g6d_instnorm_stats(const float* x, long long rows, int C, int cstride, int coff, long long rows_per_group,
                       float eps, float* scale, float* shift, double* ws, g6d_stream_t stream);

int g6d_instnorm_partial(const float* x, long long rows, int C, int cstride, int coff, long long rows_per_group,
                         double* ws, g6d_stream_t stream);
int g6d_instnorm_finalize(const double* ws, long long groups, int C, long long count, float eps, float* scale,
                          float* shift, g6d_stream_t stream);

typedef struct g6d_conv_desc {
    int B, D, H, W, Cin;
    int in_cstride, in_coff;
    int Cout, kd, kh, kw;
    int stride;
    int pd, ph, pw;
    int Do, Ho, Wo;
    int out_cstride, out_coff;
    int prologue;
    long long group_rows;
    int act;
    int max_chain_k;
} g6d_conv_desc;

#define G6D_PRO_NONE 0
#define G6D_PRO_AFFINE 1
#define G6D_PRO_AFFINE_RELU 2
#define G6D_PRO_CORR 3
#define G6D_ACT_NONE 0
#define G6D_ACT_RELU 1
#define G6D_ACT_LEAKY01 2

int g6d_conv(const g6d_conv_desc* desc, const float* x, const float* w, const float* bias,
             const float* pro_scale, const float* pro_shift, float* y, void* ws, g6d_stream_t stream);
long long g6d_conv_workspace_bytes(const g6d_conv_desc* desc);
int g6d_vgg_first_block(const float* x, const float* w, const float* bias, float* y, int B, int H, int W,
                        g6d_stream_t stream);
int g6d_pack_conv_weight(const float* w, float* out, int Cout, int Cin, int Cin_pad, int taps,
                         const float* cout_scale, g6d_stream_t stream);
#define G6D_TC_TF32 0
#define G6D_TC_F16 1
int g6d_conv_tc_supported(const g6d_conv_desc* desc, int kind);
int g6d_debug_umma_shift(float* out, int shift, int mode, g6d_stream_t stream);
int g6d_conv_tc_debug(int* host_out8);
long long g6d_conv_tc_workspace_bytes(const g6d_conv_desc* desc, int kind);
int g6d_conv_tc_stats_supported(const g6d_conv_desc* desc, int kind, long long stats_rows);
int g6d_conv_tc(const g6d_conv_desc* desc, const float* x, const void* w_hi, const void* w_lo, int w_rows, int kind,
                const float* bias, const float* pro_scale, const float* pro_shift, float* y, void* ws,
                double* stats, long long stats_rows, g6d_stream_t stream);
int g6d_pack_conv_weight_tc(const float* w, void* out_hi, void* out_lo, int Cout, int Cin, int Cin_pad, int taps,
                            int rows_pad, const float* cout_scale, int kind, g6d_stream_t stream);
int g6d_split_operand(const float* in, void* hi, void* lo, long long n, int kind, g6d_stream_t stream);
int g6d_transpose2d(const float* in, float* out, int rows, int cols, g6d_stream_t stream);
int g6d_linear_smallm(const float* x, const float* w, const float* bias, float* y, int M, int N, int K, int act,
                      g6d_stream_t stream);

#define G6D_DET_MAX_SCALES 8
typedef struct g6d_det_maps {
    int n_scales;
    int rfn, hs, ws;
    const float* map[G6D_DET_MAX_SCALES][3];
    int H[G6D_DET_MAX_SCALES][3];
    int W[G6D_DET_MAX_SCALES][3];
    float mu[3], inv_sigma[3], clip;
} g6d_det_maps;
int g6d_det_score_fuse(const g6d_det_maps* host_maps, int qn, const float* w1, const float* b1,
                       const float* w2, const float* b2, float* out, g6d_stream_t stream);
int g6d_det_corr_rowsum(const float* partial, float* out, int qn, int H, int W, int k, int rfn, g6d_stream_t stream);
int g6d_det_parse(const float* scores, const float* scales, const float* offsets, int qn, int hs, int ws,
                  int pool_ratio, float* out, long long* out_idx, g6d_stream_t stream);

int g6d_sel_ref_sums(const float* ref, int S, int P, int C, double* sum1, double* sum2, g6d_stream_t stream);
int g6d_sel_corr_prologue(const float* q, const double* sum1, const double* sum2, int S, int P, int C, float eps,
                          float* scale, float* shift, g6d_stream_t stream);
int g6d_sel_corr_score(const float* ref, const float* q, int S, int P, int C, float* score, g6d_stream_t stream);
long long g6d_sel_corr_score3_workspace_bytes(int S, int P0, int P1, int P2);
int g6d_sel_corr_score3(const float* ref0, const float* ref1, const float* ref2, const float* q0, const float* q1,
                        const float* q2, int S, int P0, int P1, int P2, int C, float* score, float* ws, int* counters,
                        g6d_stream_t stream);
int g6d_sel_vp_norm(const float* score, int L, int n, float eps, float* feats, int cstride, int coff,
                    g6d_stream_t stream);
int g6d_sel_max_angle_add(const float* x, const float* embed, float* out, int rfn, int an, int C, g6d_stream_t stream);
int g6d_attention(const float* q, const float* k, const float* v, float* out, int n, int C, int heads,
                  g6d_stream_t stream);
int g6d_attention_headmajor(const float* q, const float* k, const float* v, float* out, int n, int C, int heads,
                            g6d_stream_t stream);
int g6d_layernorm(const float* x, const float* gamma, const float* beta, float* out, int rows, int C, float eps,
                  g6d_stream_t stream);
int g6d_sel_parse(const float* logits, const float* angles, int qn, int rfn, long long* out_idx, float* out,
                  g6d_stream_t stream);

int g6d_ref_volume_fill(const float* ref_feats, const float* que_feats, const float* ref_Ks,
                        const float* ref_poses, const float* que_Ks, const float* que_poses, int Q, int R,
                        int fh, int fw, int C, int sn, int img_h, int img_w, float* mean_in, float* stdv,
                        g6d_stream_t stream);
int g6d_ref_pose_heads(const float* x, const float* w, const float* b, float* out, int M, int K, g6d_stream_t stream);

long long g6d_pose_errors_workspace_bytes(int n_pts, int n_poses);
int g6d_pose_errors(const float* pts, int n_pts, const float* poses_pr, const float* poses_gt, const float* Ks,
                    int n_poses, int symmetric, float* out, void* ws, g6d_stream_t stream);

#ifdef __cplusplus
}
#endif
#endif
```

Before: 170.6.

## Batch viewpoint selection across query images instead of a per-query loop

Replaces the per-query Python loop in viewpoint selection with one batched pass. Convolutions gain an in_items field so a shared input can be broadcast across a larger batch with per-group prologue operands. The correlation, vp-norm, max-angle and attention kernels gain a group dimension. This cuts kernel launches and host overhead per query, at the cost of more index arithmetic and packed group deltas in the tensor-core gather.

```diff
diff --git a/gen6d_b200/_lib.py b/gen6d_b200/_lib.py
--- a/gen6d_b200/_lib.py
+++ b/gen6d_b200/_lib.py
@@ -15,7 +15,8 @@
 class ConvDesc(C.Structure):
     _fields_ = [(n, C.c_int) for n in ('B', 'D', 'H', 'W', 'Cin', 'in_cstride', 'in_coff', 'Cout', 'kd', 'kh', 'kw',
                                        'stride', 'pd', 'ph', 'pw', 'Do', 'Ho', 'Wo', 'out_cstride', 'out_coff',
-                                       'prologue')] + [('group_rows', C.c_longlong), ('act', C.c_int), ('max_chain_k', C.c_int)]
+                                       'prologue')] + [('group_rows', C.c_longlong), ('act', C.c_int), ('max_chain_k', C.c_int),
+                                                           ('in_items', C.c_int)]
 
 
 class DetMaps(C.Structure):
@@ -86,14 +87,14 @@
     'g6d_det_parse': [P, P, P, I, I, I, I, P, P, P],
     'g6d_det_corr_rowsum': [P, P, I, I, I, I, I, P],
     'g6d_sel_ref_sums': [P, I, I, I, P, P, P],
-    'g6d_sel_corr_prologue': [P, P, P, I, I, I, F, P, P, P],
+    'g6d_sel_corr_prologue': [P, P, P, I, I, I, I, F, P, P, P],
     'g6d_sel_corr_score': [P, P, I, I, I, P, P],
-    'g6d_sel_corr_score3': [P, P, P, P, P, P, I, I, I, I, I, P, P, P, P],
-    'g6d_sel_corr_score3_workspace_bytes': [I, I, I, I],
-    'g6d_sel_vp_norm': [P, I, I, F, P, I, I, P],
-    'g6d_sel_max_angle_add': [P, P, P, I, I, I, P],
-    'g6d_attention': [P, P, P, P, I, I, I, P],
-    'g6d_attention_headmajor': [P, P, P, P, I, I, I, P],
+    'g6d_sel_corr_score3': [P, P, P, P, P, P, I, I, I, I, I, I, P, P, P, P],
+    'g6d_sel_corr_score3_workspace_bytes': [I, I, I, I, I],
+    'g6d_sel_vp_norm': [P, I, I, I, F, P, I, I, P],
+    'g6d_sel_max_angle_add': [P, P, P, I, I, I, I, P],
+    'g6d_attention': [P, P, P, P, I, I, I, I, P],
+    'g6d_attention_headmajor': [P, P, P, P, I, I, I, I, P],
     'g6d_layernorm': [P, P, P, P, I, I, F, P],
     'g6d_sel_parse': [P, P, I, I, P, P, P],
     'g6d_ref_volume_fill': [P, P, P, P, P, P, I, I, I, I, I, I, I, I, P, P, P],
diff --git a/gen6d_b200/csrc/common.cuh b/gen6d_b200/csrc/common.cuh
--- a/gen6d_b200/csrc/common.cuh
+++ b/gen6d_b200/csrc/common.cuh
@@ -59,4 +59,13 @@
 
 inline int ceil_div(long long a, long long b) { return (int)((a + b - 1) / b); }
 
+inline bool in_items_ok(const g6d_conv_desc* d) { return d->in_items == 0 || (d->in_items > 0 && d->B % d->in_items == 0); }
+inline bool pro_operands_fit(const g6d_conv_desc* d) {
+    if (d->prologue == G6D_PRO_NONE) return true;
+    const long long gr = d->group_rows > 0 ? d->group_rows : 1;
+    const long long groups = (d->B + gr - 1) / gr;
+    const long long per = d->prologue == G6D_PRO_CORR ? (long long)d->D * d->H * d->W : 1;
+    return groups * per * d->Cin < (1ll << 31);
 }
+
+}
diff --git a/gen6d_b200/csrc/conv_ffma.cu b/gen6d_b200/csrc/conv_ffma.cu
--- a/gen6d_b200/csrc/conv_ffma.cu
+++ b/gen6d_b200/csrc/conv_ffma.cu
@@ -7,6 +7,7 @@
     float* y; float* ws;
     int B, D, H, W, Cin, ics, ico, Cout, ldw, kd, kh, kw, stride, pd, ph, pw, Do, Ho, Wo, ocs, oco, pro, act;
     long long group_rows;
+    int in_items;
     int M, K, ktiles, splits, kt_per_split;
 };
 
@@ -36,7 +37,7 @@
     const int kt_end = min(p.ktiles, kt_begin + p.kt_per_split);
 
     const int kq = t & 3;
-    int rb[2], rz[2], ry[2], rx[2];
+    int rb[2], rg[2], rz[2], ry[2], rx[2];
     bool rvalid[2];
 #pragma unroll
     for (int i = 0; i < 2; ++i) {
@@ -46,7 +47,8 @@
         int xo = mm % p.Wo; mm /= p.Wo;
         int yo = mm % p.Ho; mm /= p.Ho;
         int zo = mm % p.Do; mm /= p.Do;
-        rb[i] = mm;
+        rb[i] = p.in_items == p.B ? mm : mm % p.in_items;
+        rg[i] = p.pro == G6D_PRO_NONE ? 0 : (int)(mm / p.group_rows);
         rz[i] = zo * p.stride - p.pd;
         ry[i] = yo * p.stride - p.ph;
         rx[i] = xo * p.stride - p.pw;
@@ -75,14 +77,13 @@
                 v = __ldg(reinterpret_cast<const float4*>(p.x + pos * p.ics + p.ico + c));
                 if (p.pro != G6D_PRO_NONE) {
                     float4 s, b;
+                    const int gc = rg[i] * p.Cin + c;
                     if (p.pro == G6D_PRO_CORR) {
-                        const long long sp = ((long long)zi * p.H + yi) * p.W + xi;
-                        s = __ldg(reinterpret_cast<const float4*>(p.ps + sp * p.Cin + c));
-                        b = __ldg(reinterpret_cast<const float4*>(p.pb + c));
+                        s = __ldg(reinterpret_cast<const float4*>(p.ps + (((rg[i] * p.D + zi) * p.H + yi) * p.W + xi) * p.Cin + c));
+                        b = __ldg(reinterpret_cast<const float4*>(p.pb + gc));
                     } else {
-                        const long long g = rb[i] / p.group_rows;
-                        s = __ldg(reinterpret_cast<const float4*>(p.ps + g * p.Cin + c));
-                        b = __ldg(reinterpret_cast<const float4*>(p.pb + g * p.Cin + c));
+                        s = __ldg(reinterpret_cast<const float4*>(p.ps + gc));
+                        b = __ldg(reinterpret_cast<const float4*>(p.pb + gc));
                     }
                     v.x = fmaf(v.x, s.x, b.x); v.y = fmaf(v.y, s.y, b.y);
                     v.z = fmaf(v.z, s.z, b.z); v.w = fmaf(v.w, s.w, b.w);
@@ -320,6 +321,8 @@
                 "g6d_conv: Cin (%d), in_cstride (%d), in_coff (%d) must be multiples of 4", d->Cin, d->in_cstride,
                 d->in_coff);
     G6D_REQUIRE(d->in_coff + d->Cin <= d->in_cstride, "g6d_conv: input channel slice out of row");
+    G6D_REQUIRE(in_items_ok(d), "g6d_conv: in_items (%d) must be 0 or divide B (%d)", d->in_items, d->B);
+    G6D_REQUIRE(pro_operands_fit(d), "g6d_conv: prologue operands too large");
     G6D_REQUIRE(d->out_coff + d->Cout <= d->out_cstride, "g6d_conv: output channel slice out of row");
     const int Do = (d->D + 2 * d->pd - d->kd) / d->stride + 1;
     const int Ho = (d->H + 2 * d->ph - d->kh) / d->stride + 1;
@@ -336,6 +339,7 @@
     p.Cout = d->Cout; p.ldw = (d->Cout + 3) & ~3; p.kd = d->kd; p.kh = d->kh; p.kw = d->kw; p.stride = d->stride;
     p.pd = d->pd; p.ph = d->ph; p.pw = d->pw; p.Do = Do; p.Ho = Ho; p.Wo = Wo; p.ocs = d->out_cstride;
     p.oco = d->out_coff; p.pro = d->prologue; p.act = d->act; p.group_rows = d->group_rows > 0 ? d->group_rows : 1;
+    p.in_items = d->in_items > 0 ? d->in_items : d->B;
     p.M = (int)M; p.K = (int)K; p.ktiles = (int)((K + BK - 1) / BK);
     const int bn = d->Cout > 64 ? 128 : (d->Cout > 32 ? 64 : 32);
     const long long ctas = (long long)ceil_div(M, BM) * ceil_div(d->Cout, bn);
@@ -372,7 +376,8 @@
     p.x = x; p.w = w; p.bias = bias; p.ps = pro_scale; p.pb = pro_shift; p.y = y; p.ws = (float*)ws;
     cudaStream_t st = as_stream(stream);
     if (p.Cin == 4 && p.ics == 4 && p.ico == 0 && p.Cout == 64 && p.ocs == 64 && p.oco == 0 && p.kd == 1 && p.kh == 3 &&
-        p.kw == 3 && p.stride == 1 && p.pd == 0 && p.ph == 1 && p.pw == 1 && p.D == 1 && p.pro == G6D_PRO_NONE) {
+        p.kw == 3 && p.stride == 1 && p.pd == 0 && p.ph == 1 && p.pw == 1 && p.D == 1 && p.pro == G6D_PRO_NONE &&
+        p.in_items == p.B) {
         conv3x3_c4_o64_kernel<<<ceil_div(p.M, 128), 128, 0, st>>>(x, w, bias, y, p.B, p.H, p.W, p.act);
         G6D_CHECK_LAUNCH("g6d_conv(first layer)");
         return G6D_OK;
diff --git a/gen6d_b200/csrc/conv_tc.cu b/gen6d_b200/csrc/conv_tc.cu
--- a/gen6d_b200/csrc/conv_tc.cu
+++ b/gen6d_b200/csrc/conv_tc.cu
@@ -36,6 +36,7 @@
     float* y; float* ws;
     int B, D, H, W, Cin, ics, ico, Cout, kd, kh, kw, stride, pd, ph, pw, Do, Ho, Wo, ocs, oco, pro, act;
     long long group_rows;
+    int in_items;
     int M, K, kblocks, splits, kb_per_split;
     double* stats; long long stats_rows;
 };
@@ -220,8 +221,9 @@
             const int m_base = mt * TC_BM;
             const int kb_begin = sp * p.kb_per_split;
             const int nkb = min(p.kblocks, kb_begin + p.kb_per_split) - kb_begin;
-            int rb[ROWS], rsp[ROWS], rc[ROWS];
-            unsigned rvmask = 0;
+            static_assert(ROWS <= 4 && RSTEP * (ROWS - 1) < 128, "group deltas must fit 7 bits each");
+            int rin[ROWS], rc[ROWS];
+            int g0 = 0; unsigned gd = 0;
             const long long plane_sz = (long long)p.D * p.H * p.W;
 #pragma unroll
             for (int j = 0; j < ROWS; ++j) {
@@ -231,11 +233,13 @@
                 const int xo = m % p.Wo; m /= p.Wo;
                 const int yo = m % p.Ho; m /= p.Ho;
                 const int zo = m % p.Do; m /= p.Do;
-                rb[j] = m;
+                const int item = p.in_items == p.B ? m : m % p.in_items;
+                const int g = m / (int)p.group_rows;
+                if (j == 0) g0 = g;
+                if (v) gd |= ((unsigned)(g - g0) | 0x80u) << (8 * j);
                 const int z = zo * p.stride - p.pd, y = yo * p.stride - p.ph, x = xo * p.stride - p.pw;
-                rsp[j] = (z * p.H + y) * p.W + x;
+                rin[j] = item * (int)plane_sz + (z * p.H + y) * p.W + x;
                 rc[j] = ((z + 8) << 24) | ((y + 8) << 12) | (x + 8);
-                if (v) rvmask |= 1u << j;
             }
             int c0, kx, ky, kz;
             {
@@ -253,12 +257,12 @@
 #pragma unroll
                 for (int j = 0; j < ROWS; ++j) {
                     const int z = ((rc[j] >> 24) & 0xff) - 8 + kz, y = ((rc[j] >> 12) & 0xfff) - 8 + ky, x = (rc[j] & 0xfff) - 8 + kx;
-                    const bool inb = ((rvmask >> j) & 1u) && (unsigned)z < (unsigned)p.D && (unsigned)y < (unsigned)p.H &&
+                    const bool inb = ((gd >> (8 * j + 7)) & 1u) && (unsigned)z < (unsigned)p.D && (unsigned)y < (unsigned)p.H &&
                                      (unsigned)x < (unsigned)p.W;
 #pragma unroll
                     for (int e = 0; e < NV; ++e) v[q][j][e] = make_float4(0.f, 0.f, 0.f, 0.f);
                     if (inb) {
-                        const float4* src = reinterpret_cast<const float4*>(xb + ((long long)rb[j] * plane_sz + rsp[j] + tap_sp) * p.ics);
+                        const float4* src = reinterpret_cast<const float4*>(xb + (long long)(rin[j] + tap_sp) * p.ics);
 #pragma unroll
                         for (int e = 0; e < NV; ++e) v[q][j][e] = __ldg(src + e * 8);
                         okm[q] |= 1u << j;
@@ -277,14 +281,15 @@
                     for (int j = 0; j < ROWS; ++j) {
                         if (okm[q] & (1u << j)) {
                             const float4* scp; const float4* shp;
+                            const int gc = (g0 + (int)((gd >> (8 * j)) & 0x7fu)) * p.Cin;
+                            const int sh = gc + kc[q];
                             if (p.pro == G6D_PRO_CORR) {
-                                scp = reinterpret_cast<const float4*>(p.ps + (long long)(rsp[j] + ksp[q]) * p.Cin + kc[q]);
-                                shp = reinterpret_cast<const float4*>(p.pb + kc[q]);
+                                const int rsp = ((((rc[j] >> 24) & 0xff) - 8) * p.H + ((rc[j] >> 12) & 0xfff) - 8) * p.W + (rc[j] & 0xfff) - 8;
+                                scp = reinterpret_cast<const float4*>(p.ps + (gc * (int)plane_sz + (rsp + ksp[q]) * p.Cin + kc[q]));
                             } else {
-                                const long long g = rb[j] / (int)p.group_rows;
-                                scp = reinterpret_cast<const float4*>(p.ps + g * p.Cin + kc[q]);
-                                shp = reinterpret_cast<const float4*>(p.pb + g * p.Cin + kc[q]);
+                                scp = reinterpret_cast<const float4*>(p.ps + sh);
                             }
+                            shp = reinterpret_cast<const float4*>(p.pb + sh);
 #pragma unroll
                             for (int e = 0; e < NV; ++e) v[q][j][e] = affine4(v[q][j][e], __ldg(scp + e * 8), __ldg(shp + e * 8), relu);
                         }
@@ -568,7 +573,8 @@
 
 static bool tc2_dims_ok(const g6d_conv_desc* d) {
     return d->D + d->pd + 8 < 256 && d->H + d->ph + 8 < 4096 && d->W + d->pw + 8 < 4096 &&
-           (long long)d->D * d->H * d->W < (1ll << 30) && d->group_rows < (1ll << 31);
+           (long long)d->D * d->H * d->W < (1ll << 30) && d->group_rows < (1ll << 31) &&
+           (long long)(d->in_items > 0 ? d->in_items : d->B) * d->D * d->H * d->W < (1ll << 31);
 }
 
 static int fill_tc_params(const g6d_conv_desc* d, int kind, ConvTcP& p) {
@@ -581,6 +587,8 @@
     G6D_REQUIRE((d->in_cstride & 3) == 0 && (d->in_coff & 3) == 0, "g6d_conv_tc: in_cstride/in_coff must be multiples of 4");
     G6D_REQUIRE(d->in_coff + d->Cin <= d->in_cstride, "g6d_conv_tc: input channel slice out of row");
     G6D_REQUIRE(d->out_coff + d->Cout <= d->out_cstride, "g6d_conv_tc: output channel slice out of row");
+    G6D_REQUIRE(in_items_ok(d), "g6d_conv_tc: in_items (%d) must be 0 or divide B (%d)", d->in_items, d->B);
+    G6D_REQUIRE(pro_operands_fit(d), "g6d_conv_tc: prologue operands too large");
     G6D_REQUIRE(tc2_dims_ok(d), "g6d_conv_tc: spatial extent too large for the tensor-core kernel");
     const int Do = (d->D + 2 * d->pd - d->kd) / d->stride + 1;
     const int Ho = (d->H + 2 * d->ph - d->kh) / d->stride + 1;
@@ -594,6 +602,7 @@
     p.Cout = d->Cout; p.kd = d->kd; p.kh = d->kh; p.kw = d->kw; p.stride = d->stride; p.pd = d->pd; p.ph = d->ph;
     p.pw = d->pw; p.Do = Do; p.Ho = Ho; p.Wo = Wo; p.ocs = d->out_cstride; p.oco = d->out_coff; p.pro = d->prologue;
     p.act = d->act; p.group_rows = d->group_rows > 0 ? d->group_rows : 1;
+    p.in_items = d->in_items > 0 ? d->in_items : d->B;
     p.M = (int)M; p.K = (int)K; p.kblocks = (int)(K / bk);
     const int bn = tc_block_n(d->Cout);
     const long long ctas = (long long)ceil_div(M, TC_BM) * ceil_div(d->Cout, bn);
@@ -684,6 +693,7 @@
     const float* x; const float* bias; const float* ps; const float* pb; float* y; float* ws;
     int B, D, H, W, Cin, ics, ico, Cout, kd, kh, kw, pd, ph, pw, Do, Ho, Wo, ocs, oco, pro, act;
     long long group_rows;
+    int in_items;
     int Wp, tiles_per_plane, mode, nseg, taps_per_seg, seg_rows, rows_pad, ntab, cblocks;
     int a_stages, b_stages, splits, cb_per_split, M;
     double* stats; long long stats_rows;
@@ -768,6 +778,7 @@
         const int r0 = threadIdx.x >> 3;
         const long long plane = (long long)p.H * p.W;
         const long long gi = (long long)b / p.group_rows;
+        const int b_in = p.in_items == p.B ? b : b % p.in_items;
         const bool relu = p.pro == G6D_PRO_AFFINE_RELU;
         constexpr int NB = 3;
         const int trips = (p.seg_rows + 127) / 128;
@@ -785,7 +796,7 @@
             unit_of(tt, u, rbase, cb, kz, tb);
             const int zz = zo + kz - p.pd;
             const bool zok = (unsigned)zz < (unsigned)p.D;
-            const float* xplane = p.x + ((long long)b * p.D + (zok ? zz : 0)) * plane * p.ics + p.ico + cb * BK + cofs;
+            const float* xplane = p.x + ((long long)b_in * p.D + (zok ? zz : 0)) * plane * p.ics + p.ico + cb * BK + cofs;
             const int* tab = rowtab + tb * p.seg_rows;
 #pragma unroll
             for (int j = 0; j < 4; ++j) {
@@ -814,9 +825,9 @@
                 if (p.pro != G6D_PRO_NONE && off[q][j] >= 0) {
                     const float4* scp; const float4* shp;
                     if (p.pro == G6D_PRO_CORR) {
-                        const long long sp = (long long)zz * plane + off[q][j];
+                        const long long sp = (gi * p.D + zz) * plane + off[q][j];
                         scp = reinterpret_cast<const float4*>(p.ps + sp * p.Cin + c);
-                        shp = reinterpret_cast<const float4*>(p.pb + c);
+                        shp = reinterpret_cast<const float4*>(p.pb + gi * p.Cin + c);
                     } else {
                         scp = reinterpret_cast<const float4*>(p.ps + gi * p.Cin + c);
                         shp = reinterpret_cast<const float4*>(p.pb + gi * p.Cin + c);
@@ -982,7 +993,7 @@
 
 static int fill_flat_params(const g6d_conv_desc* d, int kind, ConvFlatP& p, int* smem_bytes) {
     const int bk = kind_bk(kind);
-    if (!d || d->stride != 1 || (d->Cin % bk) != 0 || d->Cout < 16 || (d->in_cstride & 3) || (d->in_coff & 3)) return -1;
+    if (!d || !in_items_ok(d) || d->stride != 1 || (d->Cin % bk) != 0 || d->Cout < 16 || (d->in_cstride & 3) || (d->in_coff & 3)) return -1;
     const int Do = d->D + 2 * d->pd - d->kd + 1, Ho = d->H + 2 * d->ph - d->kh + 1, Wo = d->W + 2 * d->pw - d->kw + 1;
     if (Do != d->Do || Ho != d->Ho || Wo != d->Wo || Do < 1 || Ho < 1 || Wo < 1) return -1;
     if (d->kd * d->kh * d->kw == 1) return -1;
@@ -1005,6 +1016,7 @@
     p.Cout = d->Cout; p.kd = d->kd; p.kh = d->kh; p.kw = d->kw; p.pd = d->pd; p.ph = d->ph; p.pw = d->pw;
     p.Do = Do; p.Ho = Ho; p.Wo = Wo; p.ocs = d->out_cstride; p.oco = d->out_coff; p.pro = d->prologue; p.act = d->act;
     p.group_rows = d->group_rows > 0 ? d->group_rows : 1;
+    p.in_items = d->in_items > 0 ? d->in_items : d->B;
     p.Wp = Wp; p.tiles_per_plane = (Ho * Wp + TC_BM - 1) / TC_BM; p.mode = mode;
     p.nseg = mode == 0 ? d->kd : d->kd * d->kh; p.taps_per_seg = mode == 0 ? d->kh * d->kw : d->kw;
     p.seg_rows = rows; p.rows_pad = (rows + 7) / 8 * 8; p.ntab = ntab; p.cblocks = d->Cin / bk;
@@ -1077,7 +1089,7 @@
 
 extern "C" int g6d_conv_tc_supported(const g6d_conv_desc* d, int kind) {
     if (!d || (kind != G6D_TC_TF32 && kind != G6D_TC_F16)) return 0;
-    return (d->Cin % kind_bk(kind)) == 0 && d->Cout >= 16 && (d->in_cstride & 3) == 0 && (d->in_coff & 3) == 0 &&
+    return in_items_ok(d) && pro_operands_fit(d) && (d->Cin % kind_bk(kind)) == 0 && d->Cout >= 16 && (d->in_cstride & 3) == 0 && (d->in_coff & 3) == 0 &&
            tc2_dims_ok(d) ? 1 : 0;
 }
 
diff --git a/gen6d_b200/csrc/selector.cu b/gen6d_b200/csrc/selector.cu
--- a/gen6d_b200/csrc/selector.cu
+++ b/gen6d_b200/csrc/selector.cu
@@ -55,19 +55,20 @@
     const float* ref[3];
     const float* q[3];
     int P[3];
-    int S;
+    int S, qn;
     long long row_end[3];
 };
 
 template <int C>
-__device__ __forceinline__ float row_dot(const float4* __restrict__ rp, const float4* __restrict__ qp, int lane) {
-    constexpr int V = C / 128;
-    float4 rv[V];
-#pragma unroll
-    for (int i = 0; i < V; ++i) rv[i] = ldg_stream(rp + lane + 32 * i);
+__device__ __forceinline__ void row_load(const float4* __restrict__ rp, int lane, float4 (&rv)[C / 128]) {
+#pragma unroll
+    for (int i = 0; i < C / 128; ++i) rv[i] = ldg_stream(rp + lane + 32 * i);
+}
+template <int C>
+__device__ __forceinline__ float row_dot(const float4 (&rv)[C / 128], const float4* __restrict__ qp, int lane) {
     float t = 0.f;
 #pragma unroll
-    for (int i = 0; i < V; ++i) {
+    for (int i = 0; i < C / 128; ++i) {
         const float4 qv = __ldg(qp + lane + 32 * i);
         t = fmaf(rv[i].x, qv.x, fmaf(rv[i].y, qv.y, fmaf(rv[i].z, qv.z, fmaf(rv[i].w, qv.w, t))));
     }
@@ -75,7 +76,7 @@
 }
 
 template <int C, bool FUSED>
-__global__ void __launch_bounds__(256, 6) sel_corr_dots_kernel(const ScoreLevels L, float* __restrict__ t_out,
+__global__ void __launch_bounds__(256, 4) sel_corr_dots_kernel(const ScoreLevels L, float* __restrict__ t_out,
                                                             int* __restrict__ done, float* __restrict__ score,
                                                             long long chunk) {
     const int lane = threadIdx.x & 31, wib = threadIdx.x >> 5;
@@ -110,41 +111,49 @@
         long long first;
         locate(row, r0, q0, item, P, first);
         const bool two = row + 1 < end;
+        const int P0 = P;
         locate(two ? row + 1 : row, r1, q1, item, P, first);
-        float t0 = row_dot<C>(r0, q0, lane);
-        float t1 = row_dot<C>(r1, q1, lane);
-        t0 = warp_sum(t0);
-        t1 = warp_sum(t1);
-        if (lane == 0) {
-            t_out[row] = t0;
-            if (two) t_out[row + 1] = t1;
+        float4 v0[C / 128], v1[C / 128];
+        row_load<C>(r0, lane, v0);
+        row_load<C>(r1, lane, v1);
+        for (int g = 0; g < L.qn; ++g) {
+            float t0 = row_dot<C>(v0, q0 + (long long)g * P0 * (C / 4), lane);
+            float t1 = row_dot<C>(v1, q1 + (long long)g * P * (C / 4), lane);
+            t0 = warp_sum(t0);
+            t1 = warp_sum(t1);
+            if (lane == 0) {
+                t_out[g * rows + row] = t0;
+                if (two) t_out[g * rows + row + 1] = t1;
+            }
         }
     }
     if (!FUSED) return;
     if (lane == 0) __threadfence();
     __syncthreads();
     int n = 0;
-    for (long long r = begin; r < end; ++n) {
+    for (long long r = begin; r < end;) {
         const float4 *rp, *qp;
         int item, P;
         long long first;
         locate(r, rp, qp, item, P, first);
         const long long next = min(end, first + P);
-        if ((n & 7) == wib) {
+        for (int g = 0; g < L.qn; ++g, ++n) {
+            if ((n & 7) != wib) continue;
+            const long long gi = (long long)g * 3 * L.S + item;
             int last = 0;
-            if (lane == 0) last = atomicAdd(done + item, (int)(next - r)) + (int)(next - r) == P;
+            if (lane == 0) last = atomicAdd(done + gi, (int)(next - r)) + (int)(next - r) == P;
             last = __shfl_sync(0xffffffffu, last, 0);
             if (last) {
-                if (lane == 0) done[item] = 0;
+                if (lane == 0) done[gi] = 0;
                 __threadfence();
-                const float* tp = t_out + first;
+                const float* tp = t_out + g * rows + first;
                 float m = -INFINITY;
                 for (int p = lane; p < P; p += 32) m = fmaxf(m, __ldcg(tp + p));
                 m = warp_max(m);
                 float acc = 0.f;
                 for (int p = lane; p < P; p += 32) { const float v = __ldcg(tp + p); acc += v * (v / m); }
                 acc = warp_sum(acc);
-                if (lane == 0) score[item] = acc;
+                if (lane == 0) score[gi] = acc;
             }
         }
         r = next;
@@ -154,10 +163,11 @@
 __global__ void sel_corr_finish_kernel(const ScoreLevels L, const float* __restrict__ t, float* __restrict__ score) {
     const int lane = threadIdx.x & 31;
     const int item = (int)(((long long)blockIdx.x * blockDim.x + threadIdx.x) >> 5);
-    if (item >= 3 * L.S) return;
-    const int l = item / L.S, s = item % L.S;
+    if (item >= 3 * L.S * L.qn) return;
+    const int g = item / (3 * L.S), li = item % (3 * L.S);
+    const int l = li / L.S, s = li % L.S;
     const int P = l == 0 ? L.P[0] : (l == 1 ? L.P[1] : L.P[2]);
-    const float* tp = t + (l == 0 ? 0 : (l == 1 ? L.row_end[0] : L.row_end[1])) + (long long)s * P;
+    const float* tp = t + g * L.row_end[2] + (l == 0 ? 0 : (l == 1 ? L.row_end[0] : L.row_end[1])) + (long long)s * P;
     float m = -INFINITY;
     for (int p = lane; p < P; p += 32) m = fmaxf(m, tp[p]);
     m = warp_max(m);
@@ -184,6 +194,9 @@
 __global__ void sel_corr_prologue_kernel(const float* __restrict__ q, const double* __restrict__ sum1,
                                          const double* __restrict__ sum2, int S, int P, int C, float eps,
                                          float* __restrict__ scale, float* __restrict__ shift) {
+    q += (long long)blockIdx.y * P * C;
+    scale += (long long)blockIdx.y * P * C;
+    shift += (long long)blockIdx.y * C;
     const int c = blockIdx.x * 32 + (threadIdx.x & 31);
     const int row = threadIdx.x >> 5, nrow = blockDim.x >> 5;
     __shared__ double sm[8][32], sv[8][32];
@@ -218,7 +231,8 @@
 __global__ void sel_vp_norm_kernel(const float* __restrict__ score, int n, float eps, float* __restrict__ feats,
                                    int cstride, int coff) {
     const int l = blockIdx.x;
-    const float* s = score + (long long)l * n;
+    const float* s = score + ((long long)blockIdx.y * gridDim.x + l) * n;
+    feats += (long long)blockIdx.y * n * cstride;
     __shared__ double r1[32], r2[32];
     double a = 0.0, b = 0.0;
     for (int i = threadIdx.x; i < n; i += blockDim.x) { const double v = s[i]; a += v; b += v * v; }
@@ -239,20 +253,22 @@
 }
 
 __global__ void sel_max_angle_add_kernel(const float* __restrict__ x, const float* __restrict__ embed,
-                                         float* __restrict__ out, int rfn, int an, int C) {
+                                         float* __restrict__ out, int rows, int rfn, int an, int C) {
     const long long i = (long long)blockIdx.x * blockDim.x + threadIdx.x;
-    if (i >= (long long)rfn * C) return;
+    if (i >= (long long)rows * C) return;
     const int c = (int)(i % C);
     const int r = (int)(i / C);
     float m = -INFINITY;
     for (int a = 0; a < an; ++a) m = fmaxf(m, x[((long long)r * an + a) * C + c]);
-    out[i] = m + embed[i];
+    out[i] = m + embed[(long long)(r % rfn) * C + c];
 }
 
 __global__ void attention_kernel(const float* __restrict__ q, const float* __restrict__ k, const float* __restrict__ v,
                                  float* __restrict__ out, int n, int C, int heads) {
     extern __shared__ float sh[];
     const int i = blockIdx.x, h = blockIdx.y;
+    const long long go = (long long)blockIdx.z * n * C;
+    q += go; k += go; v += go; out += go;
     const int D = C / heads;
     float* prob = sh;
     float* qv = sh + n;
@@ -299,6 +315,8 @@
     __shared__ float s_sum[ATT_TQ];
     const int t = threadIdx.x, lane = t & 31, warp = t >> 5;
     const int i0 = blockIdx.x * ATT_TQ, h = blockIdx.y;
+    const long long go = (long long)blockIdx.z * n * C;
+    q += go; k += go; v += go; out += go;
     const float inv = rsqrtf((float)ATT_D);
     for (int e = t; e < ATT_TQ * ATT_D; e += 128) {
         const int qi = e / ATT_D, d = e % ATT_D;
@@ -412,21 +430,22 @@
     return G6D_OK;
 }
 
-extern "C" long long g6d_sel_corr_score3_workspace_bytes(int S, int P0, int P1, int P2) {
-    if (S <= 0 || P0 <= 0 || P1 <= 0 || P2 <= 0) { set_error("g6d_sel_corr_score3_workspace_bytes: bad args"); return -1; }
-    const long long rows = (long long)S * ((long long)P0 + P1 + P2);
+extern "C" long long g6d_sel_corr_score3_workspace_bytes(int S, int P0, int P1, int P2, int qn) {
+    if (S <= 0 || P0 <= 0 || P1 <= 0 || P2 <= 0 || qn <= 0) { set_error("g6d_sel_corr_score3_workspace_bytes: bad args"); return -1; }
+    const long long rows = (long long)qn * S * ((long long)P0 + P1 + P2);
     return ((rows + 3) / 4) * 4 * (long long)sizeof(float);
 }
 
 extern "C" int g6d_sel_corr_score3(const float* ref0, const float* ref1, const float* ref2, const float* q0,
-                                   const float* q1, const float* q2, int S, int P0, int P1, int P2, int C, float* score,
-                                   float* ws, int* counters, g6d_stream_t stream) {
-    G6D_REQUIRE(ref0 && ref1 && ref2 && q0 && q1 && q2 && score && ws && S > 0 && P0 > 0 && P1 > 0 && P2 > 0,
+                                   const float* q1, const float* q2, int S, int P0, int P1, int P2, int C, int qn,
+                                   float* score, float* ws, int* counters, g6d_stream_t stream) {
+    G6D_REQUIRE(ref0 && ref1 && ref2 && q0 && q1 && q2 && score && ws && S > 0 && P0 > 0 && P1 > 0 && P2 > 0 && qn > 0,
                 "g6d_sel_corr_score3: bad args");
     G6D_REQUIRE(C == 512, "g6d_sel_corr_score3: C must be 512 (got %d)", C);
+    G6D_REQUIRE(3ll * S * qn < (1ll << 31), "g6d_sel_corr_score3: too many (query, level, slice) items");
     ScoreLevels L;
     L.ref[0] = ref0; L.ref[1] = ref1; L.ref[2] = ref2; L.q[0] = q0; L.q[1] = q1; L.q[2] = q2;
-    L.P[0] = P0; L.P[1] = P1; L.P[2] = P2; L.S = S;
+    L.P[0] = P0; L.P[1] = P1; L.P[2] = P2; L.S = S; L.qn = qn;
     L.row_end[0] = (long long)S * P0; L.row_end[1] = L.row_end[0] + (long long)S * P1;
     L.row_end[2] = L.row_end[1] + (long long)S * P2;
     cudaStream_t st = as_stream(stream);
@@ -454,7 +473,7 @@
     }
     sel_corr_dots_kernel<512, false><<<(unsigned)grid, 256, 0, st>>>(L, ws, nullptr, nullptr, 0);
     G6D_CHECK_LAUNCH("g6d_sel_corr_score3(dots)");
-    sel_corr_finish_kernel<<<ceil_div(3ll * S * 32, 256), 256, 0, st>>>(L, ws, score);
+    sel_corr_finish_kernel<<<ceil_div(3ll * S * qn * 32, 256), 256, 0, st>>>(L, ws, score);
     G6D_CHECK_LAUNCH("g6d_sel_corr_score3(finish)");
     return G6D_OK;
 }
@@ -474,43 +493,48 @@
     return G6D_OK;
 }
 
-extern "C" int g6d_sel_corr_prologue(const float* q, const double* sum1, const double* sum2, int S, int P, int C,
+extern "C" int g6d_sel_corr_prologue(const float* q, const double* sum1, const double* sum2, int S, int P, int C, int qn,
                                      float eps, float* scale, float* shift, g6d_stream_t stream) {
-    G6D_REQUIRE(q && sum1 && sum2 && scale && shift && S > 0 && P > 0 && C > 0, "g6d_sel_corr_prologue: bad args");
-    sel_corr_prologue_kernel<<<ceil_div(C, 32), 256, 0, as_stream(stream)>>>(q, sum1, sum2, S, P, C, eps, scale, shift);
+    G6D_REQUIRE(q && sum1 && sum2 && scale && shift && S > 0 && P > 0 && C > 0 && qn > 0 && qn <= 65535,
+                "g6d_sel_corr_prologue: bad args");
+    sel_corr_prologue_kernel<<<dim3(ceil_div(C, 32), qn), 256, 0, as_stream(stream)>>>(q, sum1, sum2, S, P, C, eps, scale, shift);
     G6D_CHECK_LAUNCH("g6d_sel_corr_prologue");
     return G6D_OK;
 }
 
-extern "C" int g6d_sel_vp_norm(const float* score, int L, int n, float eps, float* feats, int cstride, int coff,
+extern "C" int g6d_sel_vp_norm(const float* score, int groups, int L, int n, float eps, float* feats, int cstride, int coff,
                                g6d_stream_t stream) {
-    G6D_REQUIRE(score && feats && L > 0 && n > 0 && coff + L <= cstride, "g6d_sel_vp_norm: bad args");
-    sel_vp_norm_kernel<<<L, 256, 0, as_stream(stream)>>>(score, n, eps, feats, cstride, coff);
+    G6D_REQUIRE(score && feats && groups > 0 && groups <= 65535 && L > 0 && n > 0 && coff + L <= cstride,
+                "g6d_sel_vp_norm: bad args");
+    sel_vp_norm_kernel<<<dim3(L, groups), 256, 0, as_stream(stream)>>>(score, n, eps, feats, cstride, coff);
     G6D_CHECK_LAUNCH("g6d_sel_vp_norm");
     return G6D_OK;
 }
 
-extern "C" int g6d_sel_max_angle_add(const float* x, const float* embed, float* out, int rfn, int an, int C,
+extern "C" int g6d_sel_max_angle_add(const float* x, const float* embed, float* out, int groups, int rfn, int an, int C,
                                      g6d_stream_t stream) {
-    G6D_REQUIRE(x && embed && out && rfn > 0 && an > 0 && C > 0, "g6d_sel_max_angle_add: bad args");
-    sel_max_angle_add_kernel<<<ceil_div((long long)rfn * C, 256), 256, 0, as_stream(stream)>>>(x, embed, out, rfn, an, C);
+    G6D_REQUIRE(x && embed && out && groups > 0 && rfn > 0 && an > 0 && C > 0 && (long long)groups * rfn < (1ll << 31),
+                "g6d_sel_max_angle_add: bad args");
+    const int rows = groups * rfn;
+    sel_max_angle_add_kernel<<<ceil_div((long long)rows * C, 256), 256, 0, as_stream(stream)>>>(x, embed, out, rows, rfn, an, C);
     G6D_CHECK_LAUNCH("g6d_sel_max_angle_add");
     return G6D_OK;
 }
 
-extern "C" int g6d_attention(const float* q, const float* k, const float* v, float* out, int n, int C, int heads,
+extern "C" int g6d_attention(const float* q, const float* k, const float* v, float* out, int groups, int n, int C, int heads,
                              g6d_stream_t stream) {
-    G6D_REQUIRE(q && k && v && out && n > 0 && n <= 8192 && heads > 0 && C % heads == 0, "g6d_attention: bad args");
+    G6D_REQUIRE(q && k && v && out && groups > 0 && groups <= 65535 && n > 0 && n <= 8192 && heads > 0 && C % heads == 0,
+                "g6d_attention: bad args");
     const size_t smem = sizeof(float) * (n + C / heads);
-    attention_kernel<<<dim3(n, heads), 64, smem, as_stream(stream)>>>(q, k, v, out, n, C, heads);
+    attention_kernel<<<dim3(n, heads, groups), 64, smem, as_stream(stream)>>>(q, k, v, out, n, C, heads);
     G6D_CHECK_LAUNCH("g6d_attention");
     return G6D_OK;
 }
 
-extern "C" int g6d_attention_headmajor(const float* q, const float* k, const float* v, float* out, int n, int C, int heads,
-                                       g6d_stream_t stream) {
-    G6D_REQUIRE(q && k && v && out && n > 0 && n <= 2048 && heads > 0 && C == heads * ATT_D && (C & 3) == 0,
-                "g6d_attention_headmajor: bad args (n <= 2048, C = heads * 64)");
+extern "C" int g6d_attention_headmajor(const float* q, const float* k, const float* v, float* out, int groups, int n, int C,
+                                       int heads, g6d_stream_t stream) {
+    G6D_REQUIRE(q && k && v && out && groups > 0 && groups <= 65535 && n > 0 && n <= 2048 && heads > 0 &&
+                C == heads * ATT_D && (C & 3) == 0, "g6d_attention_headmajor: bad args (n <= 2048, C = heads * 64)");
     const int npad = (n + 31) & ~31;
     const size_t smem = sizeof(float) * (ATT_TQ * ATT_D + ATT_TK * (ATT_D + 1) + (size_t)ATT_TQ * npad);
     static bool configured = false;
@@ -519,7 +543,7 @@
         if (e != cudaSuccess) { set_error("g6d_attention_headmajor: %s", cudaGetErrorString(e)); return G6D_ECUDA; }
         configured = true;
     }
-    attention_hm_kernel<<<dim3(ceil_div(n, ATT_TQ), heads), 128, smem, as_stream(stream)>>>(q, k, v, out, n, C);
+    attention_hm_kernel<<<dim3(ceil_div(n, ATT_TQ), heads, groups), 128, smem, as_stream(stream)>>>(q, k, v, out, n, C);
     G6D_CHECK_LAUNCH("g6d_attention_headmajor");
     return G6D_OK;
 }
diff --git a/gen6d_b200/network/selector.py b/gen6d_b200/network/selector.py
--- a/gen6d_b200/network/selector.py
+++ b/gen6d_b200/network/selector.py
@@ -118,39 +118,70 @@
     def comm_stats(self):
         return dict(getattr(self.comm, 'calls', {}))
 
-    def _s2_counters(self):
-        n = 3 * self.ref_shape[0] * self.ref_shape[1]
-        c = self.__dict__.get('_s2_done')
-        if c is None or c.numel() != n or c.device != self.device:
-            c = torch.zeros(n, device=self.device, dtype=torch.int32)
-            self.__dict__['_s2_done'] = c
+    def _s2_counters(self, qn):
+        n = 3 * qn * self.ref_shape[0] * self.ref_shape[1]
+        bufs = self.__dict__.setdefault('_s2_done', {})
+        c = bufs.get(n)
+        if c is None or c.device != self.device:
+            c = bufs[n] = torch.zeros(n, device=self.device, dtype=torch.int32)
         return c
 
     def _finalize(self, ws, rows_total):
         return ops.instnorm_finalize(self.comm.all_reduce_sum(ws), rows_total, IN_EPS)
 
-    def _tower(self, level, ref, scale, shift, cat_buf, S):
-        convs = self.packed()['towers'][level]
-        x, pro, ps, pb = ref, ops.PRO_CORR, scale, shift
-        for i, (pc, post) in enumerate(convs):
-            last = i + 1 == len(convs)
-            if last:
-                ops.conv(x, pc, prologue=pro, pro_scale=ps, pro_shift=pb, group_rows=S, out=cat_buf, out_coff=256 * level)
-                break
-            rows = x.shape[0] * x.shape[1] * x.shape[2]
-            y, ws = ops.conv(x, pc, prologue=pro, pro_scale=ps, pro_shift=pb, group_rows=S, stats_rows=rows)
-            ps, pb = self._finalize(ws, rows // self.ref_shape[0] * self.rfn_total)
-            pro = ops.PRO_AFFINE_RELU if 'r' in post else ops.PRO_AFFINE
-            x = ops.maxpool2x2(y) if 'p' in post else y
-
-    def _towers_sharded(self, q_feats, cat_buf, S, S_total):
+
+    def _tower_step(self, st, pc, last, cat_buf, level, S, qn):
+        x = st['x']
+        h, w = x.shape[1], x.shape[2]
+        if last:
+            ops.conv(x, pc, prologue=st['pro'], pro_scale=st['ps'], pro_shift=st['pb'], group_rows=S, out=cat_buf,
+                     out_coff=256 * level, batch=qn * S)
+            return None
+        rows = S * h * w
+        y, ws = ops.conv(x, pc, prologue=st['pro'], pro_scale=st['ps'], pro_shift=st['pb'], group_rows=S, stats_rows=rows,
+                         batch=qn * S)
+        return y, ws, rows
+
+    def _advance(self, st, post, y, ps, pb):
+        st['ps'], st['pb'] = ps, pb
+        st['pro'] = ops.PRO_AFFINE_RELU if 'r' in post else ops.PRO_AFFINE
+        st['x'] = ops.maxpool2x2(y) if 'p' in post else y
+
+    def _tower_states(self, q_feats, S_total):
+        state = []
+        for q, ref, (s1, s2) in zip(q_feats, self.ref_feats_cache, self.ref_sums):
+            qn, h, w, c = q.shape
+            scale, shift = ops.sel_corr_prologue(q.reshape(qn, h * w, c), s1, s2, S_total, IN_EPS)
+            state.append({'x': ref, 'pro': ops.PRO_CORR, 'ps': scale, 'pb': shift})
+        return state
+
+    def _towers(self, q_feats, cat_buf, S, S_total, qn):
+        towers = self.packed()['towers']
+        state = self._tower_states(q_feats, S_total)
+        br = Branches(3)
+        keep = []
+
+        def run(l, st):
+            convs = towers[l]
+            for i, (pc, post) in enumerate(convs):
+                res = self._tower_step(st, pc, i + 1 == len(convs), cat_buf, l, S, qn)
+                if res is None:
+                    break
+                y, ws, rows = res
+                ps, pb = self._finalize(ws, rows // self.ref_shape[0] * self.rfn_total)
+                self._advance(st, post, y, ps, pb)
+                keep.append(st['x'])
+
+        for l, st in enumerate(state):
+            br.run(l, lambda l=l, st=st: run(l, st))
+        br.join()
+
+    def _towers_sharded(self, q_feats, cat_buf, S, S_total, qn):
         towers = self.packed()['towers']
         nbr = 3 if self.comm.capturable else 1
-        state, keep = [], []
-        for l, (q, ref, (s1, s2)) in enumerate(zip(q_feats, self.ref_feats_cache, self.ref_sums)):
-            h, w, c = q.shape
-            scale, shift = ops.sel_corr_prologue(q.reshape(h * w, c), s1, s2, S_total, IN_EPS)
-            state.append({'x': ref, 'pro': ops.PRO_CORR, 'ps': scale, 'pb': shift, 'i': 0})
+        state, keep = self._tower_states(q_feats, S_total), []
+        for st in state:
+            st['i'] = 0
         for _ in range(max(len(t) for t in towers)):
             br = Branches(nbr)
             pend = []
@@ -160,16 +191,7 @@
                     continue
                 pc, post = convs[st['i']]
                 last = st['i'] + 1 == len(convs)
-
-                def step(l=l, st=st, pc=pc, last=last):
-                    if last:
-                        ops.conv(st['x'], pc, prologue=st['pro'], pro_scale=st['ps'], pro_shift=st['pb'], group_rows=S,
-                                 out=cat_buf, out_coff=256 * l)
-                        return None
-                    rows = st['x'].shape[0] * st['x'].shape[1] * st['x'].shape[2]
-                    return ops.conv(st['x'], pc, prologue=st['pro'], pro_scale=st['ps'], pro_shift=st['pb'], group_rows=S,
-                                    stats_rows=rows) + (rows,)
-                res = br.run(l, step)
+                res = br.run(l, lambda l=l, st=st, pc=pc, last=last: self._tower_step(st, pc, last, cat_buf, l, S, qn))
                 st['i'] += 1
                 if res is not None:
                     pend.append((st, post, res))
@@ -184,85 +206,67 @@
                 ps, pb = ops.instnorm_finalize(flat[o:o + n].reshape(ws.shape), rows // self.ref_shape[0] * self.rfn_total, IN_EPS)
                 o += n
                 keep.append((y, ws))
-                st['ps'], st['pb'] = ps, pb
-                st['pro'] = ops.PRO_AFFINE_RELU if 'r' in post else ops.PRO_AFFINE
-                st['x'] = ops.maxpool2x2(y) if 'p' in post else y
-
-    def _select_one(self, q_feats):
+                self._advance(st, post, y, ps, pb)
+
+    def _select_batch(self, q_feats):
         p = self.packed()
         rfn, an = self.ref_shape
         S = rfn * an
         S_total = self.rfn_total * an
+        qn = q_feats[0].shape[0]
         dev = self.device
-        cat_buf = torch.empty(S, 4, 4, 768, device=dev, dtype=torch.float32)
-        feats = torch.empty(S, FEAT_PAD, device=dev, dtype=torch.float32)
+        cat_buf = torch.empty(qn * S, 4, 4, 768, device=dev, dtype=torch.float32)
+        feats = torch.empty(qn * S, FEAT_PAD, device=dev, dtype=torch.float32)
         scores = ops.sel_corr_score3([r.reshape(S, -1, r.shape[-1]) for r in self.ref_feats_cache],
-                                     [q.reshape(-1, q.shape[-1]) for q in q_feats], counters=self._s2_counters())
+                                     [q.reshape(qn, -1, q.shape[-1]) for q in q_feats], counters=self._s2_counters(qn))
         if self.comm.world == 1:
-            br = Branches(3)
-            keep = []
-
-            def one_level(l, q, ref, s1, s2):
-                h, w, c = q.shape
-                scale, shift = ops.sel_corr_prologue(q.reshape(h * w, c), s1, s2, S_total, IN_EPS)
-                keep.append((scale, shift))
-                self._tower(l, ref, scale, shift, cat_buf, S)
-
-            for l, (q, ref, (s1, s2)) in enumerate(zip(q_feats, self.ref_feats_cache, self.ref_sums)):
-                br.run(l, lambda l=l, q=q, ref=ref, s1=s1, s2=s2: one_level(l, q, ref, s1, s2))
-            br.join()
+            self._towers(q_feats, cat_buf, S, S_total, qn)
         else:
-            self._towers_sharded(q_feats, cat_buf, S, S_total)
+            self._towers_sharded(q_feats, cat_buf, S, S_total, qn)
         y, ws = ops.conv(cat_buf, p['cf0'], stats_rows=S * 16)
         ps, pb = self._finalize(ws, S_total * 16)
-        y = ops.avgpool_affine(y.reshape(S * 16, 512), 16, ps, pb, rows_per_group=S * 16, act=ops.ACT_RELU)
-        ops.conv(y.reshape(S, 1, 1, 512), p['cf3'], out=feats.reshape(S, 1, 1, FEAT_PAD), out_coff=0)
+        y = ops.avgpool_affine(y.reshape(qn * S * 16, 512), 16, ps, pb, rows_per_group=S * 16, act=ops.ACT_RELU)
+        ops.conv(y.reshape(qn * S, 1, 1, 512), p['cf3'], out=feats.reshape(qn * S, 1, 1, FEAT_PAD), out_coff=0)
         if self.comm.world == 1:
             ops.sel_vp_norm(scores, feats, 512, IN_EPS)
         else:
-            all_scores = self.comm.all_gather_cat(scores, dim=1).contiguous()
-            tmp = torch.empty(S_total, 4, device=dev, dtype=torch.float32)
+            all_scores = self.comm.all_gather_cat(scores, dim=2).contiguous()
+            tmp = torch.empty(qn * S_total, 4, device=dev, dtype=torch.float32)
             ops.sel_vp_norm(all_scores, tmp, 0, IN_EPS)
             r0, _ = self.comm.shard_range(self.rfn_total)
-            feats[:, 512:516] = tmp[r0 * an:r0 * an + S]
-        x = ops.conv(feats.reshape(S, 1, 1, FEAT_PAD), p['sp0'], act=ops.ACT_RELU)
-        x = ops.conv(x, p['sp2']).reshape(rfn, an, 512)
+            feats.reshape(qn, S, FEAT_PAD)[:, :, 512:516] = tmp.reshape(qn, S_total, 4)[:, r0 * an:r0 * an + S]
+        x = ops.conv(feats.reshape(qn * S, 1, 1, FEAT_PAD), p['sp0'], act=ops.ACT_RELU)
+        x = ops.conv(x, p['sp2']).reshape(qn * rfn, an, 512)
         sf = ops.sel_max_angle_add(x, self.ref_pose_embed)
-        sf = self.comm.all_gather_cat(sf, dim=0).contiguous()
         rfn_local, rfn = rfn, self.rfn_total
+        if self.comm.world > 1:
+            sf = self.comm.all_gather_cat(sf.reshape(qn, rfn_local, 512), dim=1).reshape(qn * rfn, 512).contiguous()
         for att, (m0, m3) in zip(p['atts'], p['mlps']):
-            x4 = sf.reshape(rfn, 1, 1, 512)
-            qv = ops.conv(x4, att['conv_query']).reshape(rfn, 512)
-            kv = ops.conv(x4, att['conv_key']).reshape(rfn, 512)
-            vv = ops.conv(x4, att['conv_feats']).reshape(rfn, 512)
-            msg = ops.attention(qv, kv, vv, heads=8, head_major=True)
-            msg = ops.conv(msg.reshape(rfn, 1, 1, 512), att['conv_merge']).reshape(rfn, 512)
+            x4 = sf.reshape(qn * rfn, 1, 1, 512)
+            qv = ops.conv(x4, att['conv_query']).reshape(qn * rfn, 512)
+            kv = ops.conv(x4, att['conv_key']).reshape(qn * rfn, 512)
+            vv = ops.conv(x4, att['conv_feats']).reshape(qn * rfn, 512)
+            msg = ops.attention(qv, kv, vv, heads=8, head_major=True, groups=qn)
+            msg = ops.conv(msg.reshape(qn * rfn, 1, 1, 512), att['conv_merge']).reshape(qn * rfn, 512)
             msg = ops.layernorm(msg, att['ln_w'], att['ln_b'], 1e-5)
-            y = ops.conv(torch.cat([sf, msg], 1).reshape(rfn, 1, 1, 1024), m0)
+            y = ops.conv(torch.cat([sf, msg], 1).reshape(qn * rfn, 1, 1, 1024), m0)
             ps, pb = ops.instnorm_stats(y, rows_per_group=rfn, eps=IN_EPS)
             y = ops.conv(y, m3, prologue=ops.PRO_AFFINE_RELU, pro_scale=ps, pro_shift=pb, group_rows=rfn)
             ps, pb = ops.instnorm_stats(y, rows_per_group=rfn, eps=IN_EPS)
-            y = ops.affine_act(y.reshape(rfn, 512), ps, pb, rows_per_group=rfn, act=ops.ACT_RELU)
+            y = ops.affine_act(y.reshape(qn * rfn, 512), ps, pb, rows_per_group=rfn, act=ops.ACT_RELU)
             sf = ops.add(y, sf)
-        x = ops.conv(sf.reshape(rfn, 1, 1, 512), p['score_predict'][0], act=ops.ACT_RELU)
-        logits = ops.conv(x, p['score_predict'][1]).reshape(rfn)
-        x = feats.reshape(rfn_local, 1, 1, an * FEAT_PAD)
+        x = ops.conv(sf.reshape(qn * rfn, 1, 1, 512), p['score_predict'][0], act=ops.ACT_RELU)
+        logits = ops.conv(x, p['score_predict'][1]).reshape(qn, rfn)
+        x = feats.reshape(qn * rfn_local, 1, 1, an * FEAT_PAD)
         for i, pc in enumerate(p['angle_predict']):
             x = ops.conv(x, pc, act=ops.ACT_RELU if i < 2 else ops.ACT_NONE)
-        angles = self.comm.all_gather_cat(x.reshape(rfn_local), dim=0)
+        angles = self.comm.all_gather_cat(x.reshape(qn, rfn_local), dim=1)
         return logits, angles, scores
 
     def _select_nhwc(self, que_norm4):
         if self.ref_feats_cache is None:
             raise RuntimeError('ViewpointSelector: load_ref_imgs / extract_ref_feats must be called first')
-        feats = self._feats(que_norm4)
-        logits, angles, taps = [], [], []
-        for qi in range(que_norm4.shape[0]):
-            lg, ang, sc = self._select_one([f[qi] for f in feats])
-            logits.append(lg)
-            angles.append(ang)
-            taps.append(sc)
-        return torch.stack(logits, 0), torch.stack(angles, 0), torch.stack(taps, 0)
+        return self._select_batch(self._feats(que_norm4))
 
     def _select_u8(self, u8):
         logits, angles, _ = self._select_nhwc(ops.preprocess_u8(u8, out_c=4, imagenet_norm=True))
diff --git a/gen6d_b200/ops.py b/gen6d_b200/ops.py
--- a/gen6d_b200/ops.py
+++ b/gen6d_b200/ops.py
@@ -321,13 +321,16 @@
 
 
 def conv(x, pc, prologue=PRO_NONE, pro_scale=None, pro_shift=None, group_rows=1, act=ACT_NONE,
-         in_coff=0, out=None, out_coff=0, stats_rows=None):
+         in_coff=0, out=None, out_coff=0, stats_rows=None, batch=None):
     four = x.dim() == 4
     if four:
-        B, H, W, cs = x.shape
+        B_in, H, W, cs = x.shape
         D = 1
     else:
-        B, D, H, W, cs = x.shape
+        B_in, D, H, W, cs = x.shape
+    B = batch or B_in
+    if B % B_in:
+        raise ValueError(f'conv: batch {B} is not a multiple of the input items {B_in}')
     kd, kh, kw = pc.k
     pd, ph, pw = pc.pad
     s = pc.stride
@@ -337,7 +340,8 @@
         out = torch.empty(shape, device=x.device, dtype=torch.float32)
     d = _lib.ConvDesc(B=B, D=D, H=H, W=W, Cin=pc.cin, in_cstride=cs, in_coff=in_coff, Cout=pc.cout, kd=kd, kh=kh,
                       kw=kw, stride=s, pd=pd, ph=ph, pw=pw, Do=Do, Ho=Ho, Wo=Wo, out_cstride=out.shape[-1],
-                      out_coff=out_coff, prologue=prologue, group_rows=group_rows, act=act, max_chain_k=pc.max_chain_k)
+                      out_coff=out_coff, prologue=prologue, group_rows=group_rows, act=act, max_chain_k=pc.max_chain_k,
+                      in_items=B_in if B != B_in else 0)
     work = 2.0 * B * Do * Ho * Wo * pc.cout * kd * kh * kw * pc.cin
     M = B * Do * Ho * Wo
     stats = None
@@ -431,10 +435,10 @@
 
 
 def sel_corr_prologue(q, s1, s2, S, eps=1e-5):
-    Pn, Cc = q.shape
-    scale = torch.empty(Pn, Cc, device=q.device, dtype=torch.float32)
-    shift = torch.empty(Cc, device=q.device, dtype=torch.float32)
-    _call('g6d_sel_corr_prologue', _p(q), _p(s1, torch.float64), _p(s2, torch.float64), S, Pn, Cc, eps, _p(scale),
+    qn, Pn, Cc = (1,) + tuple(q.shape) if q.dim() == 2 else q.shape
+    scale = torch.empty(q.shape, device=q.device, dtype=torch.float32)
+    shift = torch.empty(q.shape[:-2] + (Cc,), device=q.device, dtype=torch.float32)
+    _call('g6d_sel_corr_prologue', _p(q), _p(s1, torch.float64), _p(s2, torch.float64), S, Pn, Cc, qn, eps, _p(scale),
           _p(shift), _stream())
     return scale, shift
 
@@ -451,29 +455,37 @@
 def sel_corr_score3(refs, qs, counters=None):
     S, Cc = refs[0].shape[0], refs[0].shape[2]
     Ps = [r.shape[1] for r in refs]
-    out = torch.empty(3, S, device=refs[0].device, dtype=torch.float32)
-    ws = torch.empty(_lib.lib().g6d_sel_corr_score3_workspace_bytes(S, *Ps) // 4, device=refs[0].device, dtype=torch.float32)
+    qn = 1 if qs[0].dim() == 2 else qs[0].shape[0]
+    out = torch.empty(qs[0].shape[:-2] + (3, S), device=refs[0].device, dtype=torch.float32)
+    ws = torch.empty(_lib.lib().g6d_sel_corr_score3_workspace_bytes(S, *Ps, qn) // 4, device=refs[0].device, dtype=torch.float32)
     _call('g6d_sel_corr_score3', _p(refs[0]), _p(refs[1]), _p(refs[2]), _p(qs[0]), _p(qs[1]), _p(qs[2]), S, Ps[0], Ps[1],
-          Ps[2], Cc, _p(out), _p(ws), _p(counters, torch.int32), _stream(), work=4.0 * (S * sum(Ps) * Cc + sum(Ps) * Cc + 3 * S))
+          Ps[2], Cc, qn, _p(out), _p(ws), _p(counters, torch.int32), _stream(),
+          work=4.0 * (S * sum(Ps) * Cc + qn * (sum(Ps) * Cc + 3 * S)))
     return out
 
 
 def sel_vp_norm(score, feats, coff, eps=1e-5):
-    Ln, n = score.shape
-    _call('g6d_sel_vp_norm', _p(score), Ln, n, eps, _p(feats), feats.shape[-1], coff, _stream())
+    groups, Ln, n = (1,) + tuple(score.shape) if score.dim() == 2 else score.shape
+    _call('g6d_sel_vp_norm', _p(score), groups, Ln, n, eps, _p(feats), feats.shape[-1], coff, _stream())
 
 
 def sel_max_angle_add(x, embed):
-    rfn, an, Cc = x.shape
-    out = torch.empty(rfn, Cc, device=x.device, dtype=torch.float32)
-    _call('g6d_sel_max_angle_add', _p(x), _p(embed), _p(out), rfn, an, Cc, _stream())
-    return out
-
-
-def attention(q, k, v, heads, head_major=False):
-    n, Cc = q.shape
+    rows, an, Cc = x.shape
+    rfn = embed.shape[0]
+    if rows % rfn:
+        raise ValueError(f'sel_max_angle_add: {rows} rows are not a whole number of {rfn}-reference groups')
+    out = torch.empty(rows, Cc, device=x.device, dtype=torch.float32)
+    _call('g6d_sel_max_angle_add', _p(x), _p(embed), _p(out), rows // rfn, rfn, an, Cc, _stream())
+    return out
+
+
+def attention(q, k, v, heads, head_major=False, groups=1):
+    rows, Cc = q.shape
+    if rows % groups:
+        raise ValueError(f'attention: {rows} tokens are not {groups} equal groups')
     out = torch.empty_like(q)
-    _call('g6d_attention_headmajor' if head_major else 'g6d_attention', _p(q), _p(k), _p(v), _p(out), n, Cc, heads, _stream())
+    _call('g6d_attention_headmajor' if head_major else 'g6d_attention', _p(q), _p(k), _p(v), _p(out), groups, rows // groups,
+          Cc, heads, _stream())
     return out
 
 
diff --git a/include/gen6d_b200.h b/include/gen6d_b200.h
--- a/include/gen6d_b200.h
+++ b/include/gen6d_b200.h
@@ -113,6 +113,7 @@
     long long group_rows;
     int act;
     int max_chain_k;
+    int in_items;
 } g6d_conv_desc;
 
 #define G6D_PRO_NONE 0
@@ -163,20 +164,21 @@
                   int pool_ratio, float* out, long long* out_idx, g6d_stream_t stream);
 
 int g6d_sel_ref_sums(const float* ref, int S, int P, int C, double* sum1, double* sum2, g6d_stream_t stream);
-int g6d_sel_corr_prologue(const float* q, const double* sum1, const double* sum2, int S, int P, int C, float eps,
+int g6d_sel_corr_prologue(const float* q, const double* sum1, const double* sum2, int S, int P, int C, int qn, float eps,
                           float* scale, float* shift, g6d_stream_t stream);
 int g6d_sel_corr_score(const float* ref, const float* q, int S, int P, int C, float* score, g6d_stream_t stream);
-long long g6d_sel_corr_score3_workspace_bytes(int S, int P0, int P1, int P2);
+long long g6d_sel_corr_score3_workspace_bytes(int S, int P0, int P1, int P2, int qn);
 int g6d_sel_corr_score3(const float* ref0, const float* ref1, const float* ref2, const float* q0, const float* q1,
-                        const float* q2, int S, int P0, int P1, int P2, int C, float* score, float* ws, int* counters,
+                        const float* q2, int S, int P0, int P1, int P2, int C, int qn, float* score, float* ws, int* counters,
                         g6d_stream_t stream);
-int g6d_sel_vp_norm(const float* score, int L, int n, float eps, float* feats, int cstride, int coff,
+int g6d_sel_vp_norm(const float* score, int groups, int L, int n, float eps, float* feats, int cstride, int coff,
                     g6d_stream_t stream);
-int g6d_sel_max_angle_add(const float* x, const float* embed, float* out, int rfn, int an, int C, g6d_stream_t stream);
-int g6d_attention(const float* q, const float* k, const float* v, float* out, int n, int C, int heads,
+int g6d_sel_max_angle_add(const float* x, const float* embed, float* out, int groups, int rfn, int an, int C,
+                          g6d_stream_t stream);
+int g6d_attention(const float* q, const float* k, const float* v, float* out, int groups, int n, int C, int heads,
                   g6d_stream_t stream);
-int g6d_attention_headmajor(const float* q, const float* k, const float* v, float* out, int n, int C, int heads,
-                            g6d_stream_t stream);
+int g6d_attention_headmajor(const float* q, const float* k, const float* v, float* out, int groups, int n, int C,
+                            int heads, g6d_stream_t stream);
 int g6d_layernorm(const float* x, const float* gamma, const float* beta, float* out, int rows, int C, float eps,
                   g6d_stream_t stream);
 int g6d_sel_parse(const float* logits, const float* angles, int qn, int rfn, long long* out_idx, float* out,
```

Result: faster. 183.7, median of 6 (+7.7%).
